# tpy001/VFMSeg

Hardware: AMD Instinct MI355X
Metric: train images/sec @512x512 DINOv2-L+LoRA (dg_lora_dinov2_ms_masked, 1024^2 sample = LR+HR 512^2 passes) (higher is better)
Workload: dtype bf16; 1 GPU; configs[1]: dg_lora_dinov2_ms_masked.py, synthetic 1024^2 19-class samples -> 2x512^2 passes, bs=2/GPU, full train step (fwd+bwd+allreduce+AdamW), LoRA dropout on; global_batch=2, parallelism=dp1

## Files before the change

include/vfmseg_hip.h:

```cpp
#ifndef VFMSEG_HIP_H
#define VFMSEG_HIP_H
#include <stdint.h>

#ifdef __cplusplus
extern "C" {
#endif

enum { VFM_F32 = 0, VFM_BF16 = 1, VFM_U8 = 2, VFM_I64 = 3,
       VFM_SPLIT3 = 4  };
enum { VFM_OK = 0, VFM_E_INVAL = -1, VFM_E_SHAPE = -2, VFM_E_ALIGN = -3, VFM_E_HIP = -4, VFM_E_UNSUPPORTED = -5 };
enum { VFM_EP_NONE = 0, VFM_EP_GELU = 1, VFM_EP_RELU = 2, VFM_EP_MUL_GELU_GRAD = 3, VFM_EP_MUL = 4,
       VFM_EP_QGELU = 5 , VFM_EP_MUL_QGELU_GRAD = 6,
       VFM_EP_GELU_DGELU = 7  };
enum { VFM_ACT_NONE = 0, VFM_ACT_GELU = 1, VFM_ACT_RELU = 2, VFM_ACT_QGELU = 3 };

const char* vfm_last_error(void);
int vfm_abi_version(void);
int vfm_half_kind(void);

int vfm_cast(const void* src, int src_dt, long ld_src, void* dst, int dst_dt, long ld_dst, long rows, long cols,
             const float* colscale, void* stream);
int vfm_split3(const float* src, long stride_r, long stride_c, void* dst, long ld_dst, long rows, long K, int pattern, void* stream);
int vfm_transpose(const void* src, int src_dt, long ld_src, void* dst, int dst_dt, long ld_dst, long rows, long cols,
                  long pad_rows, void* stream);
int vfm_strided_copy(const void* src, int src_dt, void* dst, int dst_dt, long n0, long n1, long n2, long n3, long s0,
                     long s1, long s2, long s3, long d0, long d1, long d2, long d3, int accumulate, void* stream);
typedef struct vfm_copy_job {
  const float* src; void* dst; long dst_dt; long accumulate;
  long n[4], s[4], d[4];
  long nsum, sum_stride;
} vfm_copy_job;
int vfm_strided_copy_batch(const vfm_copy_job* table_dev, int njobs, long max_elems, void* stream);
int vfm_axpby(const float* x, float a, float* y, float b, long n, void* stream);
int vfm_scale_by_device_scalar(float* y, const float* scalar, long n, void* stream);
int vfm_colsum(const void* x, int dt, long ld, long rows, long cols, float* out, int accumulate, float* ws, void* stream);
typedef struct vfm_lora_site {
  const float* A; const float* B;
  void* a; void* at; void* w; void* wt;
  long r, K, N, Kw, ld_a, ld_at, ld_w, ld_wt;
} vfm_lora_site;
int vfm_lora_pack(const vfm_lora_site* table_dev, int nsites, long max_elems, int dt, void* stream);
int vfm_slab_reduce(const float* slabs, int kch, long P, long Q, long rows_used, float alpha, float* dst, long sp, long sq,
                    int accumulate, void* stream);
int vfm_dropout_mask(void* out, int dt, long n, float p, uint64_t seed, uint64_t offset, void* stream);
int vfm_mul_mask(const void* src, int src_dt, long ld_src, const void* mask, int mask_dt, long mask_ld,
                 long rows_per_group, void* dst, int dst_dt, long ld_dst, long rows, long cols, void* stream);
int vfm_geglu_fwd(const void* h, int h_dt, long ld_h, void* out, int out_dt, long ld_out, long rows, long C, void* stream);
int vfm_geglu_bwd(const void* h, int h_dt, long ld_h, const void* dout, int do_dt, long ld_do, void* dh, int dh_dt,
                  long ld_dh, long rows, long C, void* stream);
int vfm_swiglu_fwd(const void* h, int h_dt, long ld_h, void* out, int out_dt, long ld_out, long rows, long C, void* stream);
int vfm_swiglu_bwd(const void* h, int h_dt, long ld_h, const void* dout, int do_dt, long ld_do, void* dh, int dh_dt,
                   long ld_dh, long rows, long C, void* stream);
int vfm_rope(void* x, int dt, long ld, long rows, int np, int ncols, int d, const float* cos_t, const float* sin_t,
             int inverse, void* stream);
int vfm_act_grad_mul(const void* dy, int dy_dt, long ld_dy, const void* pre, int pre_dt, long ld_pre, void* out, int out_dt,
                     long ld_out, long rows, long cols, int act, void* stream);
int vfm_mask_token_fwd(const float* x, const uint8_t* keep, const float* token, float* out, long rows, long C, void* stream);
int vfm_mask_token_bwd(const float* dout, const uint8_t* keep, float* dx, float* dtoken, float* ws ,
                       long rows, long C, void* stream);

int vfm_layernorm_fwd(const float* x, long ld_x, const float* w, const float* b, float eps, void* y, int y_dt, long ld_y,
                      float* stats, long rows, long C, void* stream);
int vfm_layernorm_fwd_split3(const float* x, long ld_x, const float* w, const float* b, float eps, float* y, long ld_y, void* y3, long ld3,
                             long plane, float* stats, long rows, long C, void* stream);
int vfm_layernorm_dropout_fwd(const float* x, long ld_x, const float* w, const float* b, float eps, void* y, long ld_y,
                              float* stats, void* y_drop, long ld_yd, void* mask, long ld_mask, float p, uint64_t seed,
                              uint64_t offset, long rows, long C, void* stream);
int vfm_layernorm_bwd_scaled(const void* dy, int dy_dt, long ld_dy, const float* x, long ld_x, const float* w,
                             const float* stats, float* dx, long ld_dx, int accumulate_dx, void* t_out, long ld_t,
                             const float* t_scale, long rows, long C, void* stream);
int vfm_layernorm_bwd(const void* dy, int dy_dt, long ld_dy, const float* x, long ld_x, const float* w,
                      const float* stats, float* dx, long ld_dx, int accumulate_dx, float* dw, float* db, float* ws,
                      long rows, long C, void* stream);
int vfm_groupnorm_fwd(const float* x, const float* w, const float* b, float eps, int G, int act, void* y, int y_dt,
                      float* stats, float* ws, long B, long P, long C, void* stream);
int vfm_groupnorm_bwd(const void* dy, int dy_dt, const float* x, const float* w, const float* b, const float* stats,
                      int G, int act, float* dx, float* dw, float* db, float* ws, long B, long P, long C, void* stream);
int vfm_groupnorm_tile_ok(long P, long C, int G);
int vfm_groupnorm_tile_fwd(const float* x, const float* w, const float* b, float eps, int G, int act, void* y, int y_dt,
                           float* stats, long B, long P, long C, void* stream);
int vfm_groupnorm_tile_bwd(const void* dy, int dy_dt, const float* x, const float* w, const float* b, const float* stats,
                           int G, int act, float* dx, float* dw, float* db, float* ws, long B, long P, long C, void* stream);
int vfm_bn_moments(const float* x, long rows, long C, float* sums, float* ws, void* stream);
int vfm_bn_finalize(const float* sums, float count, float* mean_var, float* running_mean, float* running_var,
                    float momentum, long C, void* stream);
int vfm_bn_apply(const float* x, const float* mean_var, const float* w, const float* b, float eps, int act, void* y,
                 int y_dt, long rows, long C, void* stream);
int vfm_bn_bwd_reduce(const void* dy, int dy_dt, const float* x, const float* mean_var, const float* w, const float* b,
                      float eps, int act, float* sums_dy, float* ws, long rows, long C, void* stream);
int vfm_bn_bwd_apply(const void* dy, int dy_dt, const float* x, const float* mean_var, const float* w, const float* b,
                     float eps, int act, const float* sums_dy, float total_rows, float* dx, long rows, long C,
                     void* stream);

typedef struct vfm_gemm_desc {
  const void* A; const void* B; void* C;
  int in_dt; int c_dt;
  long M, N, K;
  long sa_m, sa_k, sb_n, sb_k, ldc;
  float alpha;
  const float* bias; long bias_mod;
  const float* colscale;
  const void* residual; int r_dt; long ldr;
  int ep_mode; const void* aux; int aux_dt; long ld_aux;
  void* C2; int c2_dt; long ldc2;
  long batch, stride_a, stride_b, stride_c;
  long c_plane;
  long kb_rows;
} vfm_gemm_desc;
int vfm_gemm(const vfm_gemm_desc* d, void* stream);
int vfm_tune(const char* key, int value);

typedef struct vfm_attn_desc {
  const void* q; const void* k; const void* v; void* o;
  int dt; long ldq, ldk, ldv, ldo;
  int B, H, d;
  int nq_main, nq_extra, nk_main, nk_extra;
  float scale;
  float* lse;
  const void* dout; long ld_do;
  void* dq; void* dk; void* dv; long ld_dq, ld_dk, ld_dv;
  float* delta;
} vfm_attn_desc;
int vfm_attn_fwd(const vfm_attn_desc* d, void* stream);
int vfm_attn_bwd(const vfm_attn_desc* d, void* stream);
int vfm_attn_fwd_x3(const vfm_attn_desc* d, long lo_off, void* stream);
int vfm_attn_fwd_x3_split(const vfm_attn_desc* d, long lo_off, void* o3, long ld3, long plane, void* stream);
int vfm_attn_bwd_x3(const vfm_attn_desc* d, const void* q3, const void* k3, const void* v3, long ld3, long lo_off, const void* do3,
                    long ld_do3, long lo_off_do3, void* stream);

int vfm_sam_relpos_table(const float* rel_pos, int L, int d, int S, float* out, void* stream);
int vfm_sam_attn_prep(const void* qkv, int dt, long ld, const float* bias, const float* rh, const float* rw, void* q_aug,
                      void* k_aug, void* v_win, int nimg, int G, int S, int H, int d, int Dq, int NP,
                      int rows_per_batch , float scale, void* stream);
int vfm_softmax_rows(const float* scores, long ld_s, void* out, int out_dt, long ld_o, long rows, int n, int npad, void* stream);
int vfm_sam_attn_merge(const void* o_win, int dt, void* out, long ld, int nimg, int G, int S, int H, int d, int NP, void* stream);
int vfm_sam_attn_bwd_prep(const void* dao, long ld_dao, const void* qkv, long ld_qkv, const float* bias, int dt, void* dow,
                          void* dowT, void* vp, void* qsT, int nimg, int G, int S, int H, int d, int dp, int NP, float scale,
                          void* stream);
int vfm_softmax_rows_batched(const float* scores, long ld_s, void* out, int out_dt, long ld_o, long rows, int n, int npad,
                             int rows_per_batch, int valid_rows, void* stream);
int vfm_softmax_rows_bwd(const void* p, const float* dp, long ld_dp, void* ds, int dt, long ld_p, long rows, int n, int npad,
                         int rows_per_batch, int valid_rows, void* stream);
int vfm_sam_attn_bwd_merge(const void* dqa, const void* dkT, const void* dvT, int dt, const float* rh, const float* rw, void* dqkv,
                           long ld, int nimg, int G, int S, int H, int d, int dp, int NP, int Dq, float scale, void* stream);

int vfm_rein_mix_fwd(const float* x, long ld_x, const void* t, const void* vt, void* u, long ld_u, void* p, long ld_p, void* x16,
                     long ld_x16, long rows, int D, int m, float c, void* stream);
int vfm_rein_mix_bwd(const void* du, long ld_du, const void* p, long ld_p, const void* v, const void* tt, void* ds, long ld_ds,
                     float* dx, long ld_dx, long rows, int D, int m, float c, void* stream);

int vfm_sam_attn_flash_fwd(const void* qkv, long ld, const float* bias, const void* tbl_h, const void* tbl_w, void* out, long ldo,
                           int nimg, int G, int S, int H, int d, float scale, void* stream);
int vfm_sam_attn_flash_fwd_train(const void* qkv, long ld, const float* bias, const void* tbl_h, const void* tbl_w, void* out, long ldo,
                                 int nimg, int G, int S, int H, int d, float scale, float* lse, void* qext, void* stream);
long vfm_sam_attn_flash_stat_rows(int nimg, int G, int S, int H);
int vfm_sam_attn_flash_bwd(const void* qkv, long ld, const float* bias, const void* tbl_h, const void* tbl_w, const void* out,
                           const void* dout, long ldo, const float* lse, const void* qext, float* dsum, void* dqkv, long ldg,
                           int nimg, int G, int S, int H, int d, float scale, void* stream);

int vfm_patchify(const float* img, long stride_b, long stride_c, long stride_y, int y0, int x0, int h, int w, int P,
                 void* out, int out_dt, long ld_out, int B, void* stream);
int vfm_assemble_tokens(const float* patch_tok, const float* cls, const float* pos, float* x, int B, int np, int C,
                        void* stream);

int vfm_resize_bilinear(const void* in, int in_dt, int in_nchw, int B, int Hi, int Wi, int C, long in_ld_c, void* out,
                        int out_dt, int out_mode, long out_ld_c, int Hv, int Wv, int y0, int x0, int hc, int wc,
                        float scale_y, float scale_x, void* stream);
int vfm_resize_bicubic(const float* in, int Hi, int Wi, int C, float* out, int Ho, int Wo, double scale_y, double scale_x,
                       void* stream);
int vfm_label_resize(const int64_t* in, int B, int Hi, int Wi, int64_t* out, int Hv, int Wv, int y0, int x0, int hc,
                     int wc, void* stream);
int vfm_unblock(const float* x, float* y, int B, int H, int W, int C, int levels, int inverse, void* stream);
int vfm_upsample_ce(const float* logits_low, const int64_t* label, int B, int h, int w, int C, int H, int W,
                    int ignore_index, float* loss_parts, int32_t* counts, float* dlogits, void* stream);
int vfm_upsample_ce_w(const float* logits_low, const int64_t* label, const float* weight, int B, int h, int w, int C, int H, int W,
                      int ignore_index, float* loss_parts, int32_t* counts, float* dlogits, void* stream);
int vfm_pseudo_label(const float* logits_low, int B, int h, int w, int C, int H, int W, float thr, int64_t* pseudo_label,
                     float* pseudo_prob, int32_t* count, void* stream);
int vfm_class_presence(const int64_t* label, int B, long n, uint32_t* bits, void* stream);
int vfm_class_mix(const float* src_img, const float* tgt_img, const int64_t* src_label, const int64_t* pseudo_label,
                  const uint32_t* chosen, const int32_t* count, long total, int ignore_top, int ignore_bottom, int B, int H, int W,
                  float* mixed_img, int64_t* mixed_label, float* mix_weight, uint8_t* mask, void* stream);
int vfm_ce_finish(const float* loss_parts, long n, float scale, int32_t* counts, float eps, float* loss, float* acc, void* stream);
int vfm_hrda_fuse_fwd(const float* lr, const float* a, const float* hr, int B, int h, int w, int C, int ha, int wa, int hc, int wc,
                      int Y0, int X0, int my0, int my1, int mx0, int mx1, float* fused, float* att_out, float* lr_scaled_out,
                      void* stream);
int vfm_hrda_fuse_bwd(const float* d_fused, const float* lr, const float* a, const float* hr, const float* att, int B, int h, int w,
                      int C, int ha, int wa, int hc, int wc, int Y0, int X0, int my0, int my1, int mx0, int mx1, float* d_lr,
                      float* d_a, float* d_hr, float* d_att_ws, void* stream);
int vfm_reduce_sum(const float* x, long n, float scale, float* out, void* stream);

int vfm_preprocess_u8(const uint8_t* img, int H, int W, float* out, int Hp, int Wp, const float* mean3, const float* std3,
                      int bgr_to_rgb, float pad_val, void* stream);
int vfm_conf_gate(const float* logits, int B, int C, int H, int W, int y0, int x0, int hc, int wc, float thr,
                  int32_t* count, void* stream);
int vfm_slide_accumulate(const float* crop, int crop_nchw, int B, int h, int w, int C, float* preds, float* count,
                         int H, int W, int y0, int x0, int hc, int wc, void* stream);
typedef struct vfm_slide_win {
  const float* crop;
  int nchw, h, w;
  int y0, x0, hc, wc;
} vfm_slide_win;
int vfm_slide_gather(const vfm_slide_win* wins, int nwin, int B, int C, float* preds, int H, int W, void* stream);
int vfm_conf_gate_windows(const float* logits, int B, int C, int H, int W, const int* boxes, int nwin, float thr, int32_t* counts,
                          void* stream);
int vfm_slide_finalize(float* preds, const float* count, uint8_t* argmax, int B, int C, int H, int W, void* stream);

int vfm_confusion_hist(const uint8_t* pred, const void* label, int label_dt, long n, int num_classes, int ignore_index,
                       int64_t* hist, void* stream);

int vfm_adamw(float* p, float* g, float* m, float* v, long n, const long* seg_start, const float* seg_lr_mult,
              const float* seg_wd, int n_seg, float lr, float beta1, float beta2, float eps, int step, float grad_scale,
              int zero_grad, int vec4, void* stream);
int vfm_adamw_guarded(float* p, float* g, float* m, float* v, long n, const long* seg_start, const float* seg_lr_mult,
                      const float* seg_wd, int n_seg, float lr, float beta1, float beta2, float eps, int step, float grad_scale,
                      int zero_grad, int vec4, const int* skip, const float* amp_state, void* stream);
int vfm_amp_update(const int* flag, float* amp_state, float growth, float backoff, int interval, int dynamic, void* stream);

enum { VFM_OP_GEMM = 0, VFM_OP_LN_FWD = 1, VFM_OP_LN_DROPOUT_FWD = 2, VFM_OP_LN_BWD_SCALED = 3, VFM_OP_ATTN_FWD = 4, VFM_OP_ATTN_BWD = 5,
       VFM_OP_CAST = 6, VFM_OP_STRIDED_COPY = 7 };
enum { VFM_PROF_NONE = 0, VFM_PROF_GEMM = 1, VFM_PROF_GEMM_TN = 2, VFM_PROF_ATTN_FWD = 3, VFM_PROF_ATTN_BWD = 4 };
typedef struct vfm_plan_op {
  int kind;
  int prof_kind;
  double flops;
  union {
// ... 21 lines not shown
```

vfmseg_amd/csrc/elementwise.hip:

```cpp
#include "common.h"

thread_local char g_vfm_err[512] = {0};

extern "C" const char* vfm_last_error(void) { return g_vfm_err; }
extern "C" int vfm_abi_version(void) { return 6; }
extern "C" int vfm_half_kind(void) { return VFM_HALF_KIND; }

template <typename TI, typename TO>
__global__ void k_cast(const TI* __restrict__ src, long ld_src, TO* __restrict__ dst, long ld_dst, long rows, long cols,
                       const float* __restrict__ colscale) {
  const long cols4 = cols >> 2;
  const long total = rows * cols4;
  for (long i = blockIdx.x * (long)blockDim.x + threadIdx.x; i < total; i += (long)gridDim.x * blockDim.x) {
    const long r = i / cols4, c = (i - r * cols4) << 2;
    float v[4];
#pragma unroll
    for (int j = 0; j < 4; ++j) v[j] = ld_f32(src + r * ld_src + c + j);
    if (colscale) {
#pragma unroll
      for (int j = 0; j < 4; ++j) v[j] *= colscale[c + j];
    }
#pragma unroll
    for (int j = 0; j < 4; ++j) st_f32(dst + r * ld_dst + c + j, v[j]);
  }
  const long tail0 = cols4 << 2;
  const long ntail = cols - tail0;
  if (ntail) {
    for (long i = blockIdx.x * (long)blockDim.x + threadIdx.x; i < rows * ntail; i += (long)gridDim.x * blockDim.x) {
      const long r = i / ntail, c = tail0 + (i - r * ntail);
      float v = ld_f32(src + r * ld_src + c);
      if (colscale) v *= colscale[c];
      st_f32(dst + r * ld_dst + c, v);
    }
  }
}

extern "C" int vfm_cast(const void* src, int src_dt, long ld_src, void* dst, int dst_dt, long ld_dst, long rows, long cols,
                        const float* colscale, void* stream) {
  VFM_CHECK(rows >= 0 && cols >= 0 && ld_src >= cols && ld_dst >= cols, VFM_E_SHAPE, "vfm_cast: bad shape");
  if (rows == 0 || cols == 0) return VFM_OK;
  hipStream_t s = (hipStream_t)stream;
  const long total = rows * ((cols + 3) / 4);
  const int grid = (int)((total + 255) / 256 > 4096 ? 4096 : (total + 255) / 256);
#define L(TI, TO) hipLaunchKernelGGL((k_cast<TI, TO>), dim3(grid), dim3(256), 0, s, (const TI*)src, ld_src, (TO*)dst, ld_dst, rows, cols, colscale)
  if (src_dt == VFM_F32 && dst_dt == VFM_F32) L(float, float);
  else if (src_dt == VFM_F32 && dst_dt == VFM_BF16) L(float, bf16_t);
  else if (src_dt == VFM_BF16 && dst_dt == VFM_F32) L(bf16_t, float);
  else if (src_dt == VFM_BF16 && dst_dt == VFM_BF16) L(bf16_t, bf16_t);
  else VFM_FAIL(VFM_E_INVAL, "vfm_cast: dtype");
#undef L
  VFM_LAUNCH_CHECK();
  return VFM_OK;
}

__global__ void k_split3(const float* __restrict__ src, long sr, long sc, bf16_t* __restrict__ dst, long ld_dst, long rows, long K, long Kp,
                         int pattern) {
  const long per_row = Kp / 4;
  const long total = rows * per_row;
  for (long i = (long)blockIdx.x * blockDim.x + threadIdx.x; i < total; i += (long)gridDim.x * blockDim.x) {
    const long r = i / per_row, c = (i % per_row) * 4;
    float v[4];
    if (sc == 1 && c + 3 < K && ((reinterpret_cast<uintptr_t>(src + r * sr + c) & 15) == 0)) {
      const float4 f = *reinterpret_cast<const float4*>(src + r * sr + c);
      v[0] = f.x, v[1] = f.y, v[2] = f.z, v[3] = f.w;
    } else {
#pragma unroll
      for (int e = 0; e < 4; ++e) v[e] = (c + e < K) ? src[r * sr + (c + e) * sc] : 0.f;
    }
    ushort4 hi, lo;
    bf16_t* ph = &hi.x;
    bf16_t* pl = &lo.x;
#pragma unroll
    for (int e = 0; e < 4; ++e) {
      ph[e] = f32_to_bf16(v[e]);
      pl[e] = f32_to_bf16(v[e] - bf16_to_f32(ph[e]));
    }
    bf16_t* d = dst + r * ld_dst + c;
    *reinterpret_cast<ushort4*>(d) = hi;
    *reinterpret_cast<ushort4*>(d + Kp) = pattern == 0 ? hi : lo;
    *reinterpret_cast<ushort4*>(d + 2 * Kp) = pattern == 0 ? lo : hi;
  }
}

extern "C" int vfm_split3(const float* src, long stride_r, long stride_c, void* dst, long ld_dst, long rows, long K, int pattern, void* stream) {
  const long Kp = (K + 63) / 64 * 64;
  VFM_CHECK(rows >= 0 && K > 0 && ld_dst >= 3 * Kp && ld_dst % 4 == 0 && ((uintptr_t)dst % 8) == 0 && (pattern == 0 || pattern == 1), VFM_E_SHAPE,
            "vfm_split3: dst must hold rows x 3 ceil64(K) bf16 (ld %% 4 == 0, 8-byte aligned)");
  if (rows == 0) return VFM_OK;
  const long total = rows * (Kp / 4);
  const int grid = (int)((total + 255) / 256 > 8192 ? 8192 : (total + 255) / 256);
  hipLaunchKernelGGL(k_split3, dim3(grid), dim3(256), 0, (hipStream_t)stream, src, stride_r, stride_c, (bf16_t*)dst, ld_dst, rows, K, Kp, pattern);
  VFM_LAUNCH_CHECK();
  return VFM_OK;
}

template <typename TI, typename TO>
__global__ void k_transpose(const TI* __restrict__ src, long ld_src, TO* __restrict__ dst, long ld_dst, long rows, long cols,
                            long pad_rows) {
  __shared__ float tile[64][65];
  const long r0 = (long)blockIdx.y * 64, c0 = (long)blockIdx.x * 64;
  const int tx = threadIdx.x & 63, ty = threadIdx.x >> 6;
  for (int i = ty; i < 64; i += 4) {
    const long r = r0 + i, c = c0 + tx;
    tile[i][tx] = (r < rows && c < cols) ? ld_f32(src + r * ld_src + c) : 0.f;
  }
  __syncthreads();
  for (int i = ty; i < 64; i += 4) {
    const long c = c0 + i, r = r0 + tx;
    if (c < cols && r < pad_rows) st_f32(dst + c * ld_dst + r, tile[tx][i]);
  }
}

extern "C" int vfm_transpose(const void* src, int src_dt, long ld_src, void* dst, int dst_dt, long ld_dst, long rows, long cols,
                             long pad_rows, void* stream) {
  VFM_CHECK(pad_rows >= rows && ld_dst >= pad_rows && ld_src >= cols, VFM_E_SHAPE, "vfm_transpose: bad shape");
  if (cols == 0 || pad_rows == 0) return VFM_OK;
  hipStream_t s = (hipStream_t)stream;
  dim3 grid(cdiv(cols, 64), cdiv(pad_rows, 64));
#define L(TI, TO) hipLaunchKernelGGL((k_transpose<TI, TO>), grid, dim3(256), 0, s, (const TI*)src, ld_src, (TO*)dst, ld_dst, rows, cols, pad_rows)
  if (src_dt == VFM_F32 && dst_dt == VFM_F32) L(float, float);
  else if (src_dt == VFM_F32 && dst_dt == VFM_BF16) L(float, bf16_t);
  else if (src_dt == VFM_BF16 && dst_dt == VFM_F32) L(bf16_t, float);
  else if (src_dt == VFM_BF16 && dst_dt == VFM_BF16) L(bf16_t, bf16_t);
  else VFM_FAIL(VFM_E_INVAL, "vfm_transpose: dtype");
#undef L
  VFM_LAUNCH_CHECK();
  return VFM_OK;
}

template <typename TI, typename TO>
__global__ void k_strided_copy(const TI* __restrict__ src, TO* __restrict__ dst, long n0, long n1, long n2, long n3, long s0,
                               long s1, long s2, long s3, long d0, long d1, long d2, long d3, int accumulate) {
  const long total = n0 * n1 * n2 * n3;
  for (long i = blockIdx.x * (long)blockDim.x + threadIdx.x; i < total; i += (long)gridDim.x * blockDim.x) {
    long t = i;
    const long i3 = t % n3; t /= n3;
    const long i2 = t % n2; t /= n2;
    const long i1 = t % n1; t /= n1;
    const float v = ld_f32(src + t * s0 + i1 * s1 + i2 * s2 + i3 * s3);
    TO* q = dst + t * d0 + i1 * d1 + i2 * d2 + i3 * d3;
    st_f32(q, accumulate ? ld_f32(q) + v : v);
  }
}

extern "C" int vfm_strided_copy(const void* src, int src_dt, void* dst, int dst_dt, long n0, long n1, long n2, long n3,
                                long s0, long s1, long s2, long s3, long d0, long d1, long d2, long d3, int accumulate,
                                void* stream) {
  const long total = n0 * n1 * n2 * n3;
  if (total == 0) return VFM_OK;
  hipStream_t s = (hipStream_t)stream;
  const int grid = (int)((total + 255) / 256 > 4096 ? 4096 : (total + 255) / 256);
#define L(TI, TO) hipLaunchKernelGGL((k_strided_copy<TI, TO>), dim3(grid), dim3(256), 0, s, (const TI*)src, (TO*)dst, n0, n1, n2, n3, s0, s1, s2, s3, d0, d1, d2, d3, accumulate)
  if (src_dt == VFM_F32 && dst_dt == VFM_F32) L(float, float);
  else if (src_dt == VFM_F32 && dst_dt == VFM_BF16) L(float, bf16_t);
  else if (src_dt == VFM_BF16 && dst_dt == VFM_F32) L(bf16_t, float);
  else if (src_dt == VFM_BF16 && dst_dt == VFM_BF16) L(bf16_t, bf16_t);
  else VFM_FAIL(VFM_E_INVAL, "vfm_strided_copy: dtype");
#undef L
  VFM_LAUNCH_CHECK();
  return VFM_OK;
}

__global__ void k_axpby(const float* __restrict__ x, float a, float* __restrict__ y, float b, long n) {
  for (long i = blockIdx.x * (long)blockDim.x + threadIdx.x; i < n; i += (long)gridDim.x * blockDim.x)
    y[i] = (b == 0.f) ? a * x[i] : a * x[i] + b * y[i];
}
extern "C" int vfm_axpby(const float* x, float a, float* y, float b, long n, void* stream) {
  if (n == 0) return VFM_OK;
  const int grid = (int)((n + 255) / 256 > 4096 ? 4096 : (n + 255) / 256);
  hipLaunchKernelGGL(k_axpby, dim3(grid), dim3(256), 0, (hipStream_t)stream, x, a, y, b, n);
  VFM_LAUNCH_CHECK();
  return VFM_OK;
}
__global__ void k_scale_dev(float* __restrict__ y, const float* __restrict__ sc, long n) {
  const float s = *sc;
  for (long i = blockIdx.x * (long)blockDim.x + threadIdx.x; i < n; i += (long)gridDim.x * blockDim.x) y[i] *= s;
}
extern "C" int vfm_scale_by_device_scalar(float* y, const float* scalar, long n, void* stream) {
  if (n == 0) return VFM_OK;
  const int grid = (int)((n + 255) / 256 > 4096 ? 4096 : (n + 255) / 256);
  hipLaunchKernelGGL(k_scale_dev, dim3(grid), dim3(256), 0, (hipStream_t)stream, y, scalar, n);
  VFM_LAUNCH_CHECK();
  return VFM_OK;
}

template <typename T>
__global__ void k_colsum1(const T* __restrict__ x, long ld, long rows, long cols, float* __restrict__ ws, int CT) {
  __shared__ float sh[256];
  const int rl = 256 / CT;
  const int tx = threadIdx.x % CT, ty = threadIdx.x / CT;
  const long c = (long)blockIdx.x * CT + tx;
  float acc = 0.f;
  if (c < cols)
    for (long r = (long)blockIdx.y * rl + ty; r < rows; r += (long)gridDim.y * rl) acc += ld_f32(x + r * ld + c);
  sh[threadIdx.x] = acc;
  __syncthreads();
  if (ty == 0 && c < cols) {
    float a = 0.f;
    for (int k = 0; k < rl; ++k) a += sh[k * CT + tx];
    ws[(long)blockIdx.y * cols + c] = a;
  }
}
__global__ void __launch_bounds__(256) k_colsum2(const float* __restrict__ ws, long cols, int parts, float* __restrict__ out, int accumulate) {
  __shared__ float sh[4][64];
  const int tx = threadIdx.x & 63, g = threadIdx.x >> 6;
  const long c = blockIdx.x * 64L + tx;
  float a = 0.f;
  if (c < cols) {
    int p = g;
    for (; p + 12 < parts; p += 16) {
      const float v0 = ws[(long)p * cols + c], v1 = ws[(long)(p + 4) * cols + c], v2 = ws[(long)(p + 8) * cols + c], v3 = ws[(long)(p + 12) * cols + c];
      a += (v0 + v1) + (v2 + v3);
    }
    for (; p < parts; p += 4) a += ws[(long)p * cols + c];
  }
  sh[g][tx] = a;
  __syncthreads();
  if (g == 0 && c < cols) {
    const float t = (sh[0][tx] + sh[1][tx]) + (sh[2][tx] + sh[3][tx]);
    out[c] = accumulate ? out[c] + t : t;
  }
}
extern "C" int vfm_colsum(const void* x, int dt, long ld, long rows, long cols, float* out, int accumulate, float* ws,
                          void* stream) {
  VFM_CHECK(ld >= cols && ws, VFM_E_SHAPE, "vfm_colsum: bad args");
  if (cols == 0) return VFM_OK;
  hipStream_t s = (hipStream_t)stream;
  int CT = 64;
  while (CT > 8 && CT / 2 >= cols) CT /= 2;
  const int rl = 256 / CT;
  long parts = (rows + rl * 8 - 1) / (rl * 8);
  if (parts > 64) parts = 64;
  if (parts < 1) parts = 1;
  dim3 grid(cdiv(cols, CT), (unsigned)parts);
  if (dt == VFM_F32) hipLaunchKernelGGL(k_colsum1<float>, grid, dim3(256), 0, s, (const float*)x, ld, rows, cols, ws, CT);
  else if (dt == VFM_BF16) hipLaunchKernelGGL(k_colsum1<bf16_t>, grid, dim3(256), 0, s, (const bf16_t*)x, ld, rows, cols, ws, CT);
  else VFM_FAIL(VFM_E_INVAL, "vfm_colsum: dtype");
  hipLaunchKernelGGL(k_colsum2, dim3(cdiv(cols, 64)), dim3(256), 0, s, ws, cols, (int)parts, out, accumulate);
  VFM_LAUNCH_CHECK();
  return VFM_OK;
}

__global__ void k_slab_reduce(const float* __restrict__ slabs, int kch, long P, long Q, long rows_used, float alpha,
                              float* __restrict__ dst, long sp, long sq, int accumulate) {
  const long total = rows_used * Q;
  for (long i = blockIdx.x * (long)blockDim.x + threadIdx.x; i < total; i += (long)gridDim.x * blockDim.x) {
    const long p = i / Q, q = i - p * Q;
    float a = 0.f;
    for (int k = 0; k < kch; ++k) a += slabs[((long)k * P + p) * Q + q];
    a *= alpha;
    float* d = dst + p * sp + q * sq;
    *d = accumulate ? *d + a : a;
  }
}
extern "C" int vfm_slab_reduce(const float* slabs, int kch, long P, long Q, long rows_used, float alpha, float* dst, long sp,
                               long sq, int accumulate, void* stream) {
  VFM_CHECK(kch >= 1 && rows_used >= 0 && rows_used <= P, VFM_E_SHAPE, "vfm_slab_reduce: bad shape");
  const long total = rows_used * Q;
  if (total == 0) return VFM_OK;
  const int grid = (int)((total + 255) / 256 > 4096 ? 4096 : (total + 255) / 256);
  hipLaunchKernelGGL(k_slab_reduce, dim3(grid), dim3(256), 0, (hipStream_t)stream, slabs, kch, P, Q, rows_used, alpha, dst, sp, sq,
                     accumulate);
  VFM_LAUNCH_CHECK();
  return VFM_OK;
}

__global__ void __launch_bounds__(256) k_strided_copy_batch(const vfm_copy_job* __restrict__ tab) {
  const vfm_copy_job t = tab[blockIdx.y];
  const unsigned n1 = (unsigned)t.n[1], n2 = (unsigned)t.n[2], n3 = (unsigned)t.n[3];
  const unsigned total = (unsigned)t.n[0] * n1 * n2 * n3;
  for (unsigned i = blockIdx.x * 256u + threadIdx.x; i < total; i += gridDim.x * 256u) {
    unsigned r = i;
    const unsigned i3 = r % n3; r /= n3;
    const unsigned i2 = r % n2; r /= n2;
    const unsigned i1 = r % n1; r /= n1;
    const float* sp = t.src + ((long)r * t.s[0] + (long)i1 * t.s[1] + (long)i2 * t.s[2] + (long)i3 * t.s[3]);
    float v = sp[0];
    for (long c = 1; c < t.nsum; ++c) v += sp[c * t.sum_stride];
    const long o = (long)r * t.d[0] + (long)i1 * t.d[1] + (long)i2 * t.d[2] + (long)i3 * t.d[3];
    if (t.accumulate) ((float*)t.dst)[o] += v;
    else st_any(t.dst, o, (int)t.dst_dt, v);
  }
}
extern "C" int vfm_strided_copy_batch(const vfm_copy_job* table_dev, int njobs, long max_elems, void* stream) {
  VFM_CHECK(table_dev && njobs >= 0, VFM_E_INVAL, "vfm_strided_copy_batch: bad args");
  if (njobs == 0 || max_elems <= 0) return VFM_OK;
  VFM_CHECK(max_elems < (1l << 31), VFM_E_SHAPE, "vfm_strided_copy_batch: jobs are limited to 2^31 elements");
  int gx = (int)((max_elems + 2047) / 2048);
  if (gx > 2048) gx = 2048;
  if (gx < 1) gx = 1;
  hipLaunchKernelGGL(k_strided_copy_batch, dim3(gx, njobs), dim3(256), 0, (hipStream_t)stream, table_dev);
  VFM_LAUNCH_CHECK();
  return VFM_OK;
}

__global__ void k_lora_pack(const vfm_lora_site* __restrict__ tab, int dt) {
  const vfm_lora_site t = tab[blockIdx.y];
  const long na = t.r * t.K, nb = t.N * t.r;
  for (long i = blockIdx.x * (long)blockDim.x + threadIdx.x; i < na + nb; i += (long)gridDim.x * blockDim.x) {
    if (i < na) {
      const long rr = i / t.K, k = i - rr * t.K;
      const float v = t.A[i];
      st_any(t.a, rr * t.ld_a + k, dt, v);
      st_any(t.at, k * t.ld_at + rr, dt, v);
    } else {
      const long j = i - na;
      const long n = j / t.r, rr = j - n * t.r;
      const float v = t.B[j];
      st_any(t.w, n * t.ld_w + t.Kw + rr, dt, v);
      if (t.wt) st_any(t.wt, (t.Kw + rr) * t.ld_wt + n, dt, v);
    }
  }
}
extern "C" int vfm_lora_pack(const vfm_lora_site* table_dev, int nsites, long max_elems, int dt, void* stream) {
  VFM_CHECK(table_dev && nsites >= 0 && (dt == VFM_F32 || dt == VFM_BF16), VFM_E_INVAL, "vfm_lora_pack: bad args");
  if (nsites == 0) return VFM_OK;
  int gx = (int)((max_elems + 255) / 256);
  if (gx > 256) gx = 256;
  if (gx < 1) gx = 1;
  hipLaunchKernelGGL(k_lora_pack, dim3(gx, nsites), dim3(256), 0, (hipStream_t)stream, table_dev, dt);
  VFM_LAUNCH_CHECK();
  return VFM_OK;
}

struct F8 { float v[8]; };
__device__ __forceinline__ F8 ld8_bf16(const bf16_t* p) {
  const uint4 u = *reinterpret_cast<const uint4*>(p);
  F8 r;
  r.v[0] = h16_lo(u.x), r.v[1] = h16_hi(u.x);
  r.v[2] = h16_lo(u.y), r.v[3] = h16_hi(u.y);
  r.v[4] = h16_lo(u.z), r.v[5] = h16_hi(u.z);
  r.v[6] = h16_lo(u.w), r.v[7] = h16_hi(u.w);
  return r;
}
__device__ __forceinline__ void st8_bf16(bf16_t* p, const F8& r) {
  uint4 u;
  u.x = (uint32_t)f32_to_bf16(r.v[0]) | ((uint32_t)f32_to_bf16(r.v[1]) << 16);
  u.y = (uint32_t)f32_to_bf16(r.v[2]) | ((uint32_t)f32_to_bf16(r.v[3]) << 16);
  u.z = (uint32_t)f32_to_bf16(r.v[4]) | ((uint32_t)f32_to_bf16(r.v[5]) << 16);
  u.w = (uint32_t)f32_to_bf16(r.v[6]) | ((uint32_t)f32_to_bf16(r.v[7]) << 16);
  *reinterpret_cast<uint4*>(p) = u;
}
__device__ __forceinline__ F8 ld8_f32(const float* p) {
  const float4 a = *reinterpret_cast<const float4*>(p), b = *reinterpret_cast<const float4*>(p + 4);
  F8 r;
  r.v[0] = a.x, r.v[1] = a.y, r.v[2] = a.z, r.v[3] = a.w, r.v[4] = b.x, r.v[5] = b.y, r.v[6] = b.z, r.v[7] = b.w;
  return r;
}
__device__ __forceinline__ void st8_f32(float* p, const F8& r) {
  *reinterpret_cast<float4*>(p) = make_float4(r.v[0], r.v[1], r.v[2], r.v[3]);
  *reinterpret_cast<float4*>(p + 4) = make_float4(r.v[4], r.v[5], r.v[6], r.v[7]);
}
static inline bool al16(const void* p) { return ((uintptr_t)p & 15) == 0; }
static inline int grid8(long total8) { return (int)((total8 + 255) / 256 > 16384 ? 16384 : (total8 + 255) / 256); }

__global__ void k_dropout_mask_bf16x8(bf16_t* __restrict__ out, long n8, float p, float keep_scale, uint64_t seed, uint64_t offset) {
  for (long i = blockIdx.x * (long)blockDim.x + threadIdx.x; i < n8; i += (long)gridDim.x * blockDim.x) {
    F8 r;
#pragma unroll
    for (int e = 0; e < 8; ++e) {
      const float u = (hash_u32(seed, offset + (uint64_t)(i * 8 + e)) >> 8) * (1.0f / 16777216.0f);
      r.v[e] = u >= p ? keep_scale : 0.f;
    }
    st8_bf16(out + i * 8, r);
  }
}
__global__ void k_mul_mask_bf16x8(const bf16_t* __restrict__ src, long ld_src, const bf16_t* __restrict__ mask, long mask_ld, long rpg,
                                  bf16_t* __restrict__ dst, long ld_dst, long rows, int cols8) {
  const long total = rows * cols8;
  for (long i = blockIdx.x * (long)blockDim.x + threadIdx.x; i < total; i += (long)gridDim.x * blockDim.x) {
    const long r = i / cols8;
    const int c = (int)(i - r * cols8) * 8;
    F8 a = ld8_bf16(src + r * ld_src + c);
    const F8 m = ld8_bf16(mask + (r / rpg) * mask_ld + c);
#pragma unroll
    for (int e = 0; e < 8; ++e) a.v[e] *= m.v[e];
    st8_bf16(dst + r * ld_dst + c, a);
  }
}
__global__ void k_act_grad_mul_bf16x8(const bf16_t* __restrict__ dy, long ld_dy, const bf16_t* __restrict__ pre, long ld_pre,
                                      bf16_t* __restrict__ out, long ld_out, long rows, int cols8, int act) {
  const long total = rows * cols8;
  for (long i = blockIdx.x * (long)blockDim.x + threadIdx.x; i < total; i += (long)gridDim.x * blockDim.x) {
    const long r = i / cols8;
    const int c = (int)(i - r * cols8) * 8;
    F8 d = ld8_bf16(dy + r * ld_dy + c);
    const F8 p = ld8_bf16(pre + r * ld_pre + c);
#pragma unroll
    for (int e = 0; e < 8; ++e) {
      const float x = p.v[e];
      const float g = act == VFM_ACT_GELU ? gelu_grad_f(x) : (act == VFM_ACT_RELU ? (x > 0.f ? 1.f : 0.f) : (act == VFM_ACT_QGELU ? qgelu_grad_f(x) : 1.f));
      d.v[e] *= g;
    }
    st8_bf16(out + r * ld_out + c, d);
  }
// ... 57 lines not shown
}

__global__ void k_mul_mask(const void* __restrict__ src, int src_dt, long ld_src, const void* __restrict__ mask, int mask_dt,
                           long mask_ld, long rpg, void* __restrict__ dst, int dst_dt, long ld_dst, long rows, long cols) {
  const long total = rows * cols;
  for (long i = blockIdx.x * (long)blockDim.x + threadIdx.x; i < total; i += (long)gridDim.x * blockDim.x) {
    const long r = i / cols, c = i - r * cols;
    const float m = ld_any(mask, (r / rpg) * mask_ld + c, mask_dt);
    st_any(dst, r * ld_dst + c, dst_dt, ld_any(src, r * ld_src + c, src_dt) * m);
  }
}
template <typename TS, typename TM, typename TD>
__global__ void k_mul_mask_x8(const TS* __restrict__ src, long ld_src, const TM* __restrict__ mask, long mask_ld, long rpg, TD* __restrict__ dst,
                              long ld_dst, long rows, int cols8) {
  const long total = rows * cols8;
  for (long i = blockIdx.x * (long)blockDim.x + threadIdx.x; i < total; i += (long)gridDim.x * blockDim.x) {
    const long r = i / cols8;
    const int c = (int)(i - r * cols8) * 8;
    F8 a, m;
    if constexpr (sizeof(TS) == 2) a = ld8_bf16(src + r * ld_src + c); else a = ld8_f32(src + r * ld_src + c);
    if constexpr (sizeof(TM) == 2) m = ld8_bf16(mask + (r / rpg) * mask_ld + c); else m = ld8_f32(mask + (r / rpg) * mask_ld + c);
#pragma unroll
    for (int e = 0; e < 8; ++e) a.v[e] *= m.v[e];
    if constexpr (sizeof(TD) == 2) st8_bf16(dst + r * ld_dst + c, a); else st8_f32(dst + r * ld_dst + c, a);
  }
}
template <typename TS, typename TM, typename TD>
static void launch_mul_mask_x8(const void* src, long ld_src, const void* mask, long mask_ld, long rpg, void* dst, long ld_dst, long rows, long cols,
                               hipStream_t s) {
  hipLaunchKernelGGL((k_mul_mask_x8<TS, TM, TD>), dim3(grid8(rows * cols / 8)), dim3(256), 0, s, (const TS*)src, ld_src, (const TM*)mask, mask_ld, rpg,
                     (TD*)dst, ld_dst, rows, (int)(cols / 8));
}
extern "C" int vfm_mul_mask(const void* src, int src_dt, long ld_src, const void* mask, int mask_dt, long mask_ld,
                            long rows_per_group, void* dst, int dst_dt, long ld_dst, long rows, long cols, void* stream) {
  VFM_CHECK(rows_per_group >= 1, VFM_E_INVAL, "vfm_mul_mask: rows_per_group");
  const long total = rows * cols;
  if (total == 0) return VFM_OK;
  auto h16 = [](int dt) { return dt == VFM_BF16; };
  auto okdt = [](int dt) { return dt == VFM_BF16 || dt == VFM_F32; };
  if (okdt(src_dt) && okdt(mask_dt) && okdt(dst_dt) && !(h16(src_dt) && h16(mask_dt) && h16(dst_dt)) && cols % 8 == 0 && ld_src % 8 == 0 &&
      mask_ld % 8 == 0 && ld_dst % 8 == 0 && al16(src) && al16(mask) && al16(dst)) {
    hipStream_t s = (hipStream_t)stream;
    const int key = (h16(src_dt) ? 4 : 0) | (h16(mask_dt) ? 2 : 0) | (h16(dst_dt) ? 1 : 0);
#define MM(TS, TM, TD) launch_mul_mask_x8<TS, TM, TD>(src, ld_src, mask, mask_ld, rows_per_group, dst, ld_dst, rows, cols, s)
    switch (key) {
      case 0: MM(float, float, float); break;
      case 1: MM(float, float, bf16_t); break;
      case 2: MM(float, bf16_t, float); break;
      case 3: MM(float, bf16_t, bf16_t); break;
      case 4: MM(bf16_t, float, float); break;
      case 5: MM(bf16_t, float, bf16_t); break;
      default: MM(bf16_t, bf16_t, float); break;
    }
#undef MM
    VFM_LAUNCH_CHECK();
    return VFM_OK;
  }
  if (src_dt == VFM_BF16 && mask_dt == VFM_BF16 && dst_dt == VFM_BF16 && cols % 8 == 0 && ld_src % 8 == 0 && mask_ld % 8 == 0 && ld_dst % 8 == 0 &&
      al16(src) && al16(mask) && al16(dst)) {
    hipLaunchKernelGGL(k_mul_mask_bf16x8, dim3(grid8(total / 8)), dim3(256), 0, (hipStream_t)stream, (const bf16_t*)src, ld_src, (const bf16_t*)mask,
                       mask_ld, rows_per_group, (bf16_t*)dst, ld_dst, rows, (int)(cols / 8));
    VFM_LAUNCH_CHECK();
    return VFM_OK;
  }
  const int grid = (int)((total + 255) / 256 > 8192 ? 8192 : (total + 255) / 256);
  hipLaunchKernelGGL(k_mul_mask, dim3(grid), dim3(256), 0, (hipStream_t)stream, src, src_dt, ld_src, mask, mask_dt, mask_ld,
                     rows_per_group, dst, dst_dt, ld_dst, rows, cols);
  VFM_LAUNCH_CHECK();
  return VFM_OK;
}

__global__ void k_geglu_fwd(const void* __restrict__ h, int h_dt, long ld_h, void* __restrict__ out, int out_dt, long ld_out,
                            long rows, long C) {
  const long total = rows * C;
  for (long i = blockIdx.x * (long)blockDim.x + threadIdx.x; i < total; i += (long)gridDim.x * blockDim.x) {
    const long r = i / C, c = i - r * C;
    const float a = ld_any(h, r * ld_h + c, h_dt), g = ld_any(h, r * ld_h + C + c, h_dt);
    st_any(out, r * ld_out + c, out_dt, a * gelu_f(g));
  }
}
__global__ void k_geglu_bwd(const void* __restrict__ h, int h_dt, long ld_h, const void* __restrict__ dout, int do_dt,
                            long ld_do, void* __restrict__ dh, int dh_dt, long ld_dh, long rows, long C) {
  const long total = rows * C;
  for (long i = blockIdx.x * (long)blockDim.x + threadIdx.x; i < total; i += (long)gridDim.x * blockDim.x) {
    const long r = i / C, c = i - r * C;
    const float a = ld_any(h, r * ld_h + c, h_dt), g = ld_any(h, r * ld_h + C + c, h_dt);
    const float d = ld_any(dout, r * ld_do + c, do_dt);
    st_any(dh, r * ld_dh + c, dh_dt, d * gelu_f(g));
    st_any(dh, r * ld_dh + C + c, dh_dt, d * a * gelu_grad_f(g));
  }
}
__global__ void k_geglu_fwd_x8(const bf16_t* __restrict__ h, long ld_h, bf16_t* __restrict__ out, long ld_out, long rows, long C, int c8) {
  const long total = rows * c8;
  for (long i = blockIdx.x * (long)blockDim.x + threadIdx.x; i < total; i += (long)gridDim.x * blockDim.x) {
    const long r = i / c8;
    const int c = (int)(i - r * c8) * 8;
    F8 a = ld8_bf16(h + r * ld_h + c);
    const F8 g = ld8_bf16(h + r * ld_h + C + c);
#pragma unroll
    for (int e = 0; e < 8; ++e) a.v[e] *= gelu_f(g.v[e]);
    st8_bf16(out + r * ld_out + c, a);
  }
}
__global__ void k_geglu_bwd_x8(const bf16_t* __restrict__ h, long ld_h, const bf16_t* __restrict__ dout, long ld_do, bf16_t* __restrict__ dh,
                               long ld_dh, long rows, long C, int c8) {
  const long total = rows * c8;
  for (long i = blockIdx.x * (long)blockDim.x + threadIdx.x; i < total; i += (long)gridDim.x * blockDim.x) {
    const long r = i / c8;
    const int c = (int)(i - r * c8) * 8;
    const F8 a = ld8_bf16(h + r * ld_h + c), g = ld8_bf16(h + r * ld_h + C + c), d = ld8_bf16(dout + r * ld_do + c);
    F8 da, dg;
#pragma unroll
    for (int e = 0; e < 8; ++e) {
      da.v[e] = d.v[e] * gelu_f(g.v[e]);
      dg.v[e] = d.v[e] * a.v[e] * gelu_grad_f(g.v[e]);
    }
    st8_bf16(dh + r * ld_dh + c, da);
    st8_bf16(dh + r * ld_dh + C + c, dg);
  }
}
extern "C" int vfm_geglu_fwd(const void* h, int h_dt, long ld_h, void* out, int out_dt, long ld_out, long rows, long C,
                             void* stream) {
  const long total = rows * C;
  if (total == 0) return VFM_OK;
  if (h_dt == VFM_BF16 && out_dt == VFM_BF16 && C % 8 == 0 && ld_h % 8 == 0 && ld_out % 8 == 0 && al16(h) && al16(out)) {
    hipLaunchKernelGGL(k_geglu_fwd_x8, dim3(grid8(total / 8)), dim3(256), 0, (hipStream_t)stream, (const bf16_t*)h, ld_h, (bf16_t*)out, ld_out, rows, C,
                       (int)(C / 8));
    VFM_LAUNCH_CHECK();
    return VFM_OK;
  }
  const int grid = (int)((total + 255) / 256 > 8192 ? 8192 : (total + 255) / 256);
  hipLaunchKernelGGL(k_geglu_fwd, dim3(grid), dim3(256), 0, (hipStream_t)stream, h, h_dt, ld_h, out, out_dt, ld_out, rows, C);
  VFM_LAUNCH_CHECK();
  return VFM_OK;
}
extern "C" int vfm_geglu_bwd(const void* h, int h_dt, long ld_h, const void* dout, int do_dt, long ld_do, void* dh, int dh_dt,
                             long ld_dh, long rows, long C, void* stream) {
  const long total = rows * C;
  if (total == 0) return VFM_OK;
  if (h_dt == VFM_BF16 && do_dt == VFM_BF16 && dh_dt == VFM_BF16 && C % 8 == 0 && ld_h % 8 == 0 && ld_do % 8 == 0 && ld_dh % 8 == 0 && al16(h) &&
      al16(dout) && al16(dh)) {
    hipLaunchKernelGGL(k_geglu_bwd_x8, dim3(grid8(total / 8)), dim3(256), 0, (hipStream_t)stream, (const bf16_t*)h, ld_h, (const bf16_t*)dout, ld_do,
                       (bf16_t*)dh, ld_dh, rows, C, (int)(C / 8));
    VFM_LAUNCH_CHECK();
    return VFM_OK;
  }
  const int grid = (int)((total + 255) / 256 > 8192 ? 8192 : (total + 255) / 256);
  hipLaunchKernelGGL(k_geglu_bwd, dim3(grid), dim3(256), 0, (hipStream_t)stream, h, h_dt, ld_h, dout, do_dt, ld_do, dh, dh_dt,
                     ld_dh, rows, C);
  VFM_LAUNCH_CHECK();
  return VFM_OK;
}

__global__ void k_swiglu_fwd(const void* __restrict__ h, int h_dt, long ld_h, void* __restrict__ out, int out_dt, long ld_out,
                             long rows, long C) {
  const long total = rows * C;
  for (long i = blockIdx.x * (long)blockDim.x + threadIdx.x; i < total; i += (long)gridDim.x * blockDim.x) {
    const long r = i / C, c = i - r * C;
    const float a = ld_any(h, r * ld_h + c, h_dt), g = ld_any(h, r * ld_h + C + c, h_dt);
    st_any(out, r * ld_out + c, out_dt, a / (1.f + __expf(-a)) * g);
  }
}
__global__ void k_swiglu_bwd(const void* __restrict__ h, int h_dt, long ld_h, const void* __restrict__ dout, int do_dt,
                             long ld_do, void* __restrict__ dh, int dh_dt, long ld_dh, long rows, long C) {
  const long total = rows * C;
  for (long i = blockIdx.x * (long)blockDim.x + threadIdx.x; i < total; i += (long)gridDim.x * blockDim.x) {
    const long r = i / C, c = i - r * C;
    const float a = ld_any(h, r * ld_h + c, h_dt), g = ld_any(h, r * ld_h + C + c, h_dt);
    const float d = ld_any(dout, r * ld_do + c, do_dt);
    const float sg = 1.f / (1.f + __expf(-a));
    st_any(dh, r * ld_dh + c, dh_dt, d * g * sg * (1.f + a * (1.f - sg)));
    st_any(dh, r * ld_dh + C + c, dh_dt, d * a * sg);
  }
}
extern "C" int vfm_swiglu_fwd(const void* h, int h_dt, long ld_h, void* out, int out_dt, long ld_out, long rows, long C,
                              void* stream) {
  const long total = rows * C;
  if (total == 0) return VFM_OK;
  if (h_dt == VFM_BF16 && (out_dt == VFM_BF16 || out_dt == VFM_F32) && C % 8 == 0 && ld_h % 8 == 0 && ld_out % 8 == 0 && al16(h) && al16(out)) {
    if (out_dt == VFM_BF16)
      hipLaunchKernelGGL(k_swiglu_fwd_x8<true>, dim3(grid8(total / 8)), dim3(256), 0, (hipStream_t)stream, (const bf16_t*)h, ld_h, out, ld_out, rows, C, (int)(C / 8));
    else
      hipLaunchKernelGGL(k_swiglu_fwd_x8<false>, dim3(grid8(total / 8)), dim3(256), 0, (hipStream_t)stream, (const bf16_t*)h, ld_h, out, ld_out, rows, C, (int)(C / 8));
    VFM_LAUNCH_CHECK();
    return VFM_OK;
  }
  const int grid = (int)((total + 255) / 256 > 8192 ? 8192 : (total + 255) / 256);
  hipLaunchKernelGGL(k_swiglu_fwd, dim3(grid), dim3(256), 0, (hipStream_t)stream, h, h_dt, ld_h, out, out_dt, ld_out, rows, C);
  VFM_LAUNCH_CHECK();
  return VFM_OK;
}
extern "C" int vfm_swiglu_bwd(const void* h, int h_dt, long ld_h, const void* dout, int do_dt, long ld_do, void* dh, int dh_dt,
                              long ld_dh, long rows, long C, void* stream) {
  const long total = rows * C;
  if (total == 0) return VFM_OK;
  if (h_dt == VFM_BF16 && dh_dt == VFM_BF16 && (do_dt == VFM_BF16 || do_dt == VFM_F32) && C % 8 == 0 && ld_h % 8 == 0 && ld_do % 8 == 0 &&
      ld_dh % 8 == 0 && al16(h) && al16(dout) && al16(dh)) {
    if (do_dt == VFM_BF16)
      hipLaunchKernelGGL(k_swiglu_bwd_x8<true>, dim3(grid8(total / 8)), dim3(256), 0, (hipStream_t)stream, (const bf16_t*)h, ld_h, dout, ld_do, (bf16_t*)dh, ld_dh, rows, C, (int)(C / 8));
    else
      hipLaunchKernelGGL(k_swiglu_bwd_x8<false>, dim3(grid8(total / 8)), dim3(256), 0, (hipStream_t)stream, (const bf16_t*)h, ld_h, dout, ld_do, (bf16_t*)dh, ld_dh, rows, C, (int)(C / 8));
    VFM_LAUNCH_CHECK();
    return VFM_OK;
  }
  const int grid = (int)((total + 255) / 256 > 8192 ? 8192 : (total + 255) / 256);
  hipLaunchKernelGGL(k_swiglu_bwd, dim3(grid), dim3(256), 0, (hipStream_t)stream, h, h_dt, ld_h, dout, do_dt, ld_do, dh, dh_dt,
                     ld_dh, rows, C);
  VFM_LAUNCH_CHECK();
  return VFM_OK;
}

__device__ __forceinline__ void rope_pair(float x0, float x1, float c_0, float c_1, float s_0, float s_1, int inverse, float& y0, float& y1) {
  if (!inverse) {
    y0 = fmaf(x0, c_0, -(x1 * s_0));
    y1 = fmaf(x1, c_1, x0 * s_1);
  } else {
    y0 = fmaf(x0, c_0, x1 * s_1);
    y1 = fmaf(x1, c_1, -(x0 * s_0));
  }
}
__global__ void k_rope(void* __restrict__ x, int dt, long ld, long rows, int np, int ncols, int d, const float* __restrict__ cs,
                       const float* __restrict__ sn, int inverse) {
  const long half = ncols / 2;
  const long total = rows * half;
  for (long i = blockIdx.x * (long)blockDim.x + threadIdx.x; i < total; i += (long)gridDim.x * blockDim.x) {
    const long r = i / half;
    const int c0 = (int)(i - r * half) * 2;
    const int t = (int)(r % np), dc = c0 % d;
    const float x0 = ld_any(x, r * ld + c0, dt), x1 = ld_any(x, r * ld + c0 + 1, dt);
    const float c_0 = cs[(long)t * d + dc], c_1 = cs[(long)t * d + dc + 1];
    const float s_0 = sn[(long)t * d + dc], s_1 = sn[(long)t * d + dc + 1];
    float y0, y1;
    rope_pair(x0, x1, c_0, c_1, s_0, s_1, inverse, y0, y1);
    st_any(x, r * ld + c0, dt, y0);
    st_any(x, r * ld + c0 + 1, dt, y1);
  }
}
__global__ void k_rope_bf16x8(bf16_t* __restrict__ x, long ld, long rows, int np, int c8n, int d, const float* __restrict__ cs,
                              const float* __restrict__ sn, int inverse) {
  const long total = rows * c8n;
  for (long i = blockIdx.x * (long)blockDim.x + threadIdx.x; i < total; i += (long)gridDim.x * blockDim.x) {
    const long r = i / c8n;
    const int c0 = (int)(i - r * c8n) * 8;
    const int t = (int)(r % np), dc = c0 % d;
    F8 v = ld8_bf16(x + r * ld + c0);
    const F8 c = ld8_f32(cs + (long)t * d + dc), sv = ld8_f32(sn + (long)t * d + dc);
#pragma unroll
    for (int e = 0; e < 8; e += 2) rope_pair(v.v[e], v.v[e + 1], c.v[e], c.v[e + 1], sv.v[e], sv.v[e + 1], inverse, v.v[e], v.v[e + 1]);
    st8_bf16(x + r * ld + c0, v);
  }
}
extern "C" int vfm_rope(void* x, int dt, long ld, long rows, int np, int ncols, int d, const float* cos_t, const float* sin_t,
                        int inverse, void* stream) {
  VFM_CHECK(d % 2 == 0 && ncols % d == 0 && np > 0, VFM_E_SHAPE, "vfm_rope: shape");
  const long total = rows * (ncols / 2);
  if (total == 0) return VFM_OK;
  if (dt == VFM_BF16 && d % 8 == 0 && ld % 8 == 0 && al16(x) && al16(cos_t) && al16(sin_t)) {
    hipLaunchKernelGGL(k_rope_bf16x8, dim3(grid8(rows * (ncols / 8))), dim3(256), 0, (hipStream_t)stream, (bf16_t*)x, ld, rows, np, ncols / 8, d, cos_t,
                       sin_t, inverse);
    VFM_LAUNCH_CHECK();
    return VFM_OK;
  }
  const int grid = (int)((total + 255) / 256 > 8192 ? 8192 : (total + 255) / 256);
  hipLaunchKernelGGL(k_rope, dim3(grid), dim3(256), 0, (hipStream_t)stream, x, dt, ld, rows, np, ncols, d, cos_t, sin_t, inverse);
  VFM_LAUNCH_CHECK();
  return VFM_OK;
}

__global__ void k_act_grad_mul(const void* __restrict__ dy, int dy_dt, long ld_dy, const void* __restrict__ pre, int pre_dt,
                               long ld_pre, void* __restrict__ out, int out_dt, long ld_out, long rows, long cols, int act) {
  const long total = rows * cols;
  for (long i = blockIdx.x * (long)blockDim.x + threadIdx.x; i < total; i += (long)gridDim.x * blockDim.x) {
    const long r = i / cols, c = i - r * cols;
    const float p = ld_any(pre, r * ld_pre + c, pre_dt);
    const float g = act == VFM_ACT_GELU ? gelu_grad_f(p) : (act == VFM_ACT_RELU ? (p > 0.f ? 1.f : 0.f) : (act == VFM_ACT_QGELU ? qgelu_grad_f(p) : 1.f));
    st_any(out, r * ld_out + c, out_dt, ld_any(dy, r * ld_dy + c, dy_dt) * g);
  }
}
extern "C" int vfm_act_grad_mul(const void* dy, int dy_dt, long ld_dy, const void* pre, int pre_dt, long ld_pre, void* out,
                                int out_dt, long ld_out, long rows, long cols, int act, void* stream) {
  const long total = rows * cols;
  if (total == 0) return VFM_OK;
  if (dy_dt == VFM_BF16 && pre_dt == VFM_BF16 && out_dt == VFM_BF16 && cols % 8 == 0 && ld_dy % 8 == 0 && ld_pre % 8 == 0 && ld_out % 8 == 0 &&
      al16(dy) && al16(pre) && al16(out)) {
    hipLaunchKernelGGL(k_act_grad_mul_bf16x8, dim3(grid8(total / 8)), dim3(256), 0, (hipStream_t)stream, (const bf16_t*)dy, ld_dy, (const bf16_t*)pre,
                       ld_pre, (bf16_t*)out, ld_out, rows, (int)(cols / 8), act);
    VFM_LAUNCH_CHECK();
    return VFM_OK;
  }
  const int grid = (int)((total + 255) / 256 > 8192 ? 8192 : (total + 255) / 256);
  hipLaunchKernelGGL(k_act_grad_mul, dim3(grid), dim3(256), 0, (hipStream_t)stream, dy, dy_dt, ld_dy, pre, pre_dt, ld_pre, out,
                     out_dt, ld_out, rows, cols, act);
  VFM_LAUNCH_CHECK();
  return VFM_OK;
}

__global__ void k_mask_token_fwd(const float* __restrict__ x, const uint8_t* __restrict__ keep, const float* __restrict__ tok,
                                 float* __restrict__ out, long rows, long C) {
  const long total = rows * C;
  for (long i = blockIdx.x * (long)blockDim.x + threadIdx.x; i < total; i += (long)gridDim.x * blockDim.x) {
    const long r = i / C, c = i - r * C;
    out[i] = keep[r] ? x[i] : tok[c];
  }
}
__global__ void k_mask_token_bwd(const float* __restrict__ dout, const uint8_t* __restrict__ keep, float* __restrict__ dx,
                                 float* __restrict__ ws, long rows, long C, long rows_per_chunk) {
// ... 74 lines not shown
```

vfmseg_amd/csrc/norm.hip:

```cpp
#include "common.h"

__device__ __forceinline__ float act_f(float v, int act) {
  return act == VFM_ACT_GELU ? gelu_f(v) : (act == VFM_ACT_RELU ? fmaxf(v, 0.f) : v);
}
__device__ __forceinline__ float act_grad_f(float v, int act) {
  return act == VFM_ACT_GELU ? gelu_grad_f(v) : (act == VFM_ACT_RELU ? (v > 0.f ? 1.f : 0.f) : 1.f);
}

template <typename TO, int MAXPL>
__global__ void k_ln_fwd(const float* __restrict__ x, long ld_x, const float* __restrict__ w, const float* __restrict__ b,
                         float eps, TO* __restrict__ y, long ld_y, float* __restrict__ stats, long rows, int C) {
  const int lane = threadIdx.x & 63;
  const long row = (long)blockIdx.x * (blockDim.x >> 6) + (threadIdx.x >> 6);
  if (row >= rows) return;
  const float* xr = x + row * ld_x;
  float v[MAXPL];
  float s = 0.f;
#pragma unroll
  for (int i = 0; i < MAXPL; ++i) {
    const int c = i * 64 + lane;
    v[i] = c < C ? xr[c] : 0.f;
    s += v[i];
  }
  const float mean = wave_sum(s) / C;
// ... 466 lines not shown
#pragma unroll
  for (int i = 0; i < MAXP4; ++i) {
    const int c = (i * 64 + lane) * 4;
    if (c < C) {
      float o[4];
#pragma unroll
      for (int e = 0; e < 4; ++e) o[e] = rstd * (g[i][e] - s1 - xh[i][e] * s2);
      if (c + 4 <= C) {
        float4* pp = reinterpret_cast<float4*>(dx + row * ld_dx + c);
        if (accumulate_dx) {
          const float4 old = *pp;
          o[0] += old.x, o[1] += old.y, o[2] += old.z, o[3] += old.w;
        }
        *pp = make_float4(o[0], o[1], o[2], o[3]);
      } else {
#pragma unroll
        for (int e = 0; e < 4; ++e)
          if (c + e < C) dx[row * ld_dx + c + e] = accumulate_dx ? dx[row * ld_dx + c + e] + o[e] : o[e];
      }
    }
  }
}

static int ln_bwd_impl(const void* dy, int dy_dt, long ld_dy, const float* x, long ld_x, const float* w, const float* stats,
                       float* dx, long ld_dx, int accumulate_dx, float* dw, float* db, float* ws, long rows, long C, void* t_out,
                       long ld_t, const float* t_scale, void* stream);
extern "C" int vfm_layernorm_bwd(const void* dy, int dy_dt, long ld_dy, const float* x, long ld_x, const float* w,
                                 const float* stats, float* dx, long ld_dx, int accumulate_dx, float* dw, float* db,
                                 float* ws, long rows, long C, void* stream) {
  return ln_bwd_impl(dy, dy_dt, ld_dy, x, ld_x, w, stats, dx, ld_dx, accumulate_dx, dw, db, ws, rows, C, nullptr, 0, nullptr, stream);
}
extern "C" int vfm_layernorm_bwd_scaled(const void* dy, int dy_dt, long ld_dy, const float* x, long ld_x, const float* w,
                                        const float* stats, float* dx, long ld_dx, int accumulate_dx, void* t_out, long ld_t,
                                        const float* t_scale, long rows, long C, void* stream) {
  VFM_CHECK(t_out && t_scale && ld_t % 4 == 0 && (uintptr_t)t_out % 8 == 0 && (uintptr_t)t_scale % 16 == 0, VFM_E_INVAL,
            "vfm_layernorm_bwd_scaled: t_out / t_scale");
  return ln_bwd_impl(dy, dy_dt, ld_dy, x, ld_x, w, stats, dx, ld_dx, accumulate_dx, nullptr, nullptr, nullptr, rows, C, t_out, ld_t,
                     t_scale, stream);
}
template <typename TD, int MAXP2>
__global__ void k_ln_bwd_v2(const TD* __restrict__ dy, long ld_dy, const float* __restrict__ x, long ld_x, const float* __restrict__ w,
                            const float* __restrict__ stats, float* __restrict__ dx, long ld_dx, int accumulate_dx, long rows, int C) {
  const int lane = threadIdx.x & 63;
  const long row = (long)blockIdx.x * (blockDim.x >> 6) + (threadIdx.x >> 6);
  if (row >= rows) return;
  const float mean = stats[row * 2], rstd = stats[row * 2 + 1];
  float2 g[MAXP2], xh[MAXP2];
  float s1 = 0.f, s2 = 0.f;
#pragma unroll
  for (int i = 0; i < MAXP2; ++i) {
    const int c = (i * 64 + lane) * 2;
    g[i] = xh[i] = make_float2(0.f, 0.f);
    if (c < C) {
      float2 d;
      if constexpr (sizeof(TD) == 2) {
        const ushort2 pp = *reinterpret_cast<const ushort2*>(dy + row * ld_dy + c);
        d = make_float2(bf16_to_f32(pp.x), bf16_to_f32(pp.y));
      } else {
        d = *reinterpret_cast<const float2*>(dy + row * ld_dy + c);
      }
      const float2 xv = *reinterpret_cast<const float2*>(x + row * ld_x + c);
      const float2 ww = *reinterpret_cast<const float2*>(w + c);
      xh[i] = make_float2((xv.x - mean) * rstd, (xv.y - mean) * rstd);
      g[i] = make_float2(d.x * ww.x, d.y * ww.y);
      s1 += g[i].x + g[i].y;
      s2 += g[i].x * xh[i].x + g[i].y * xh[i].y;
    }
  }
  s1 = wave_sum(s1) / C;
  s2 = wave_sum(s2) / C;
#pragma unroll
  for (int i = 0; i < MAXP2; ++i) {
    const int c = (i * 64 + lane) * 2;
    if (c < C) {
      float2 o = make_float2(rstd * (g[i].x - s1 - xh[i].x * s2), rstd * (g[i].y - s1 - xh[i].y * s2));
      float2* pp = reinterpret_cast<float2*>(dx + row * ld_dx + c);
      if (accumulate_dx) {
        const float2 old = *pp;
        o.x += old.x, o.y += old.y;
      }
      *pp = o;
    }
  }
}

static int ln_bwd_impl(const void* dy, int dy_dt, long ld_dy, const float* x, long ld_x, const float* w, const float* stats,
                       float* dx, long ld_dx, int accumulate_dx, float* dw, float* db, float* ws, long rows, long C, void* t_out,
                       long ld_t, const float* t_scale, void* stream) {
  VFM_CHECK(C > 0 && (C <= 1024 || (C <= 3072 && !(dw || db))), VFM_E_SHAPE, "vfm_layernorm_bwd: C=%ld unsupported", C);
  VFM_CHECK(!(dw || db) || ws, VFM_E_INVAL, "vfm_layernorm_bwd: ws required for dw/db");
  if (rows == 0) return VFM_OK;
  hipStream_t s = (hipStream_t)stream;
  const bool need_w = (dw || db);
  const int nv = (int)(C / 256);
  const bool v4 = !need_w && (C % 256 == 0) && (nv == 1 || nv == 2 || nv == 4 || nv == 5) && (ld_x % 4 == 0) && (ld_dx % 4 == 0) &&
                  (ld_dy % 4 == 0) && ((uintptr_t)x % 16 == 0) && ((uintptr_t)dx % 16 == 0) && ((uintptr_t)dy % 8 == 0) &&
                  ((uintptr_t)w % 16 == 0);
  if (v4) {
    dim3 grid(cdiv(rows, 4)), blk(256);
#define LV(TD, NV) hipLaunchKernelGGL((k_ln_bwd_v4<TD, NV>), grid, blk, 0, s, (const TD*)dy, ld_dy, x, ld_x, w, stats, dx, ld_dx, accumulate_dx, rows, (int)C, (bf16_t*)t_out, ld_t, t_scale)
    if (dy_dt == VFM_BF16) { if (nv == 1) LV(bf16_t, 1); else if (nv == 2) LV(bf16_t, 2); else if (nv == 4) LV(bf16_t, 4); else LV(bf16_t, 5); }
    else if (dy_dt == VFM_F32) { if (nv == 1) LV(float, 1); else if (nv == 2) LV(float, 2); else if (nv == 4) LV(float, 4); else LV(float, 5); }
    else VFM_FAIL(VFM_E_INVAL, "vfm_layernorm_bwd: dtype");
#undef LV
    VFM_LAUNCH_CHECK();
    return VFM_OK;
  }
  VFM_CHECK(!t_out, VFM_E_UNSUPPORTED, "vfm_layernorm_bwd_scaled: needs the vectorised path (C %% 256 == 0, aligned operands, no dw/db)");
  {
    const long cp = (C + 3) / 4 * 4;
    if (!need_w && C > 1024 && C <= 2816 && ld_x % 4 == 0 && ld_dx % 4 == 0 && ld_dy % 4 == 0 && ld_x >= cp && ld_dx >= cp && ld_dy >= cp &&
        (uintptr_t)x % 16 == 0 && (uintptr_t)dx % 16 == 0 && (uintptr_t)dy % 16 == 0 && (uintptr_t)w % 16 == 0) {
      dim3 grid(cdiv(rows, 4)), blk(256);
      if (dy_dt == VFM_BF16)
        hipLaunchKernelGGL((k_ln_bwd_v4t<bf16_t, 11>), grid, blk, 0, s, (const bf16_t*)dy, ld_dy, x, ld_x, w, stats, dx, ld_dx, accumulate_dx, rows, (int)C);
      else if (dy_dt == VFM_F32)
        hipLaunchKernelGGL((k_ln_bwd_v4t<float, 11>), grid, blk, 0, s, (const float*)dy, ld_dy, x, ld_x, w, stats, dx, ld_dx, accumulate_dx, rows, (int)C);
      else VFM_FAIL(VFM_E_INVAL, "vfm_layernorm_bwd: dtype");
      VFM_LAUNCH_CHECK();
      return VFM_OK;
    }
  }
  if (!need_w && C > 1024 && C % 2 == 0 && ld_x % 2 == 0 && ld_dx % 2 == 0 && ld_dy % 2 == 0 && (uintptr_t)x % 8 == 0 &&
      (uintptr_t)dx % 8 == 0 && (uintptr_t)dy % 8 == 0 && (uintptr_t)w % 8 == 0) {
    dim3 grid(cdiv(rows, 4)), blk(256);
    if (dy_dt == VFM_BF16)
      hipLaunchKernelGGL((k_ln_bwd_v2<bf16_t, 24>), grid, blk, 0, s, (const bf16_t*)dy, ld_dy, x, ld_x, w, stats, dx, ld_dx, accumulate_dx, rows, (int)C);
    else if (dy_dt == VFM_F32)
      hipLaunchKernelGGL((k_ln_bwd_v2<float, 24>), grid, blk, 0, s, (const float*)dy, ld_dy, x, ld_x, w, stats, dx, ld_dx, accumulate_dx, rows, (int)C);
    else VFM_FAIL(VFM_E_INVAL, "vfm_layernorm_bwd: dtype");
    VFM_LAUNCH_CHECK();
    return VFM_OK;
  }
  const int parts = need_w ? 128 : cdiv(rows, 4);
  const size_t shm = need_w ? (size_t)4 * 2 * C * sizeof(float) : 0;
  float* wsp = need_w ? ws : nullptr;
#define L(TD, PL, NW) hipLaunchKernelGGL((k_ln_bwd<TD, PL, NW>), dim3(parts), dim3(256), shm, s, (const TD*)dy, ld_dy, x, ld_x, w, stats, dx, ld_dx, accumulate_dx, wsp, rows, (int)C)
  const int pl = (int)((C + 63) / 64);
  if (need_w) {
    if (dy_dt == VFM_BF16) { if (pl <= 4) L(bf16_t, 4, true); else L(bf16_t, 16, true); }
    else if (dy_dt == VFM_F32) { if (pl <= 4) L(float, 4, true); else L(float, 16, true); }
    else VFM_FAIL(VFM_E_INVAL, "vfm_layernorm_bwd: dtype");
  } else {
    if (dy_dt == VFM_BF16) { if (pl <= 4) L(bf16_t, 4, false); else if (pl <= 16) L(bf16_t, 16, false); else L(bf16_t, 48, false); }
    else if (dy_dt == VFM_F32) { if (pl <= 4) L(float, 4, false); else if (pl <= 16) L(float, 16, false); else L(float, 48, false); }
    else VFM_FAIL(VFM_E_INVAL, "vfm_layernorm_bwd: dtype");
  }
#undef L
  if (need_w) hipLaunchKernelGGL(k_ln_bwd_fin, dim3(cdiv(C, 64)), dim3(256), 0, s, ws, parts, (int)C, dw, db);
  VFM_LAUNCH_CHECK();
  return VFM_OK;
}

template <int MODE, typename TD>
__global__ void k_chan_moments(const float* __restrict__ x, const TD* __restrict__ dy, const float* __restrict__ w,
                               const float* __restrict__ bb, const float* __restrict__ stats, int G, float eps, int act,
                               float* __restrict__ ws, long P, int C, int rows_per_chunk) {
  __shared__ float sh[2][4][64];
  const int tx = threadIdx.x & 63, ty = threadIdx.x >> 6;
  const int c = blockIdx.x * 64 + tx;
  const long b = blockIdx.z;
  const long r0 = (long)blockIdx.y * rows_per_chunk;
  long r1 = r0 + rows_per_chunk;
  if (r1 > P) r1 = P;
  float a1 = 0.f, a2 = 0.f;
  if (c < C) {
    float mean = 0.f, rstd = 1.f, wc = 1.f, bc = 0.f;
    if (MODE == 1) {
      if (G > 0) {
        const int g = c / (C / G);
        mean = stats[(b * G + g) * 2];
        rstd = stats[(b * G + g) * 2 + 1];
      } else {
        mean = stats[c];
        rstd = rsqrtf(stats[C + c] + eps);
      }
      wc = w[c];
      bc = bb[c];
    }
    const float* xp = x + (b * P) * C + c;
    for (long r = r0 + ty; r < r1; r += 4) {
      const float xv = xp[r * C];
      if (MODE == 0) {
        a1 += xv;
        a2 += xv * xv;
      } else {
        const float xh = (xv - mean) * rstd;
        float d = ld_f32(dy + (b * P + r) * C + c);
        if (act != VFM_ACT_NONE) d *= act_grad_f(xh * wc + bc, act);
        a1 += d;
        a2 += d * xh;
      }
    }
  }
  sh[0][ty][tx] = a1;
  sh[1][ty][tx] = a2;
  __syncthreads();
  if (ty == 0 && c < C) {
    const long slot = b * gridDim.y + blockIdx.y;
    ws[(slot * 2 + 0) * C + c] = sh[0][0][tx] + sh[0][1][tx] + sh[0][2][tx] + sh[0][3][tx];
    ws[(slot * 2 + 1) * C + c] = sh[1][0][tx] + sh[1][1][tx] + sh[1][2][tx] + sh[1][3][tx];
  }
}

static inline int pick_chunks(long P) {
  int n = (int)((P + 63) / 64);
  if (n > 64) n = 64;
  if (n < 1) n = 1;
  return n;
}

__device__ __forceinline__ double wave_sum_f64(double v) {
#pragma unroll
  for (int o = 32; o > 0; o >>= 1) v += __shfl_xor(v, o, 64);
  return v;
}
__global__ void k_gn_fin_fwd(const float* __restrict__ ws, int nchunk, int C, int G, long P, float eps,
                             float* __restrict__ stats, int BG) {
  const int i = blockIdx.x * (blockDim.x >> 6) + (threadIdx.x >> 6), lane = threadIdx.x & 63;
  if (i >= BG) return;
  const int b = i / G, g = i - b * G, cg = C / G;
  double s = 0.0, q = 0.0;
  for (int e = lane; e < nchunk * cg; e += 64) {
    const int k = e / cg, j = e - k * cg;
    const long slot = (long)b * nchunk + k;
    s += ws[(slot * 2 + 0) * C + g * cg + j];
    q += ws[(slot * 2 + 1) * C + g * cg + j];
  }
  s = wave_sum_f64(s), q = wave_sum_f64(q);
  if (lane) return;
  const double n = (double)P * cg;
  const double mean = s / n;
  double var = q / n - mean * mean;
  if (var < 0) var = 0;
  stats[i * 2] = (float)mean;
  stats[i * 2 + 1] = (float)(1.0 / sqrt(var + (double)eps));
}
template <typename TO>
__global__ void k_gn_apply(const float* __restrict__ x, const float* __restrict__ w, const float* __restrict__ b,
                           const float* __restrict__ stats, int G, int act, TO* __restrict__ y, long B, long P, int C) {
  const long total = B * P * C;
  const int cg = C / G;
  for (long i = blockIdx.x * (long)blockDim.x + threadIdx.x; i < total; i += (long)gridDim.x * blockDim.x) {
    const int c = (int)(i % C);
    const long bi = i / ((long)P * C);
    const int g = c / cg;
    const float mean = stats[(bi * G + g) * 2], rstd = stats[(bi * G + g) * 2 + 1];
    st_f32(y + i, act_f((x[i] - mean) * rstd * w[c] + b[c], act));
  }
}
extern "C" int vfm_groupnorm_fwd(const float* x, const float* w, const float* b, float eps, int G, int act, void* y, int y_dt,
                                 float* stats, float* ws_in, long B, long P, long C, void* stream) {
  VFM_CHECK(G > 0 && C % G == 0 && ws_in, VFM_E_SHAPE, "vfm_groupnorm_fwd: C %% G / ws");
  if (B * P * C == 0) return VFM_OK;
  hipStream_t s = (hipStream_t)stream;
  const int nchunk = pick_chunks(P);
  const int rpc = (int)((P + nchunk - 1) / nchunk);
  float* ws = ws_in + B * G * 2;
  hipLaunchKernelGGL((k_chan_moments<0, float>), dim3(cdiv(C, 64), nchunk, (unsigned)B), dim3(256), 0, s, x, (const float*)nullptr,
                     (const float*)nullptr, (const float*)nullptr, (const float*)nullptr, 0, 0.f, 0, ws, P, (int)C, rpc);
  hipLaunchKernelGGL(k_gn_fin_fwd, dim3(cdiv(B * G, 4)), dim3(256), 0, s, ws, nchunk, (int)C, G, P, eps, stats, (int)(B * G));
  const long total = B * P * C;
  const int grid = (int)((total + 255) / 256 > 8192 ? 8192 : (total + 255) / 256);
  if (y_dt == VFM_BF16) hipLaunchKernelGGL(k_gn_apply<bf16_t>, dim3(grid), dim3(256), 0, s, x, w, b, stats, G, act, (bf16_t*)y, B, P, (int)C);
  else if (y_dt == VFM_F32) hipLaunchKernelGGL(k_gn_apply<float>, dim3(grid), dim3(256), 0, s, x, w, b, stats, G, act, (float*)y, B, P, (int)C);
  else VFM_FAIL(VFM_E_INVAL, "vfm_groupnorm_fwd: dtype");
  VFM_LAUNCH_CHECK();
  return VFM_OK;
}

__global__ void k_gn_fin_bwd(const float* __restrict__ ws, int nchunk, int C, int G, const float* __restrict__ w,
                             float* __restrict__ gs, int BG) {
  const int i = blockIdx.x * (blockDim.x >> 6) + (threadIdx.x >> 6), lane = threadIdx.x & 63;
  if (i >= BG) return;
  const int b = i / G, g = i - b * G, cg = C / G;
  double s1 = 0.0, s2 = 0.0;
  for (int e = lane; e < nchunk * cg; e += 64) {
    const int k = e / cg, j = e - k * cg;
    const long slot = (long)b * nchunk + k;
    const int c = g * cg + j;
    s1 += (double)w[c] * ws[(slot * 2 + 0) * C + c];
    s2 += (double)w[c] * ws[(slot * 2 + 1) * C + c];
  }
  s1 = wave_sum_f64(s1), s2 = wave_sum_f64(s2);
  if (lane) return;
  gs[i * 2] = (float)s1;
  gs[i * 2 + 1] = (float)s2;
}
__global__ void k_chan_fin_wb(const float* __restrict__ ws, int slots, int C, float* __restrict__ dw, float* __restrict__ db) {
  __shared__ float sh[2][4][64];
  const int tx = threadIdx.x & 63, ty = threadIdx.x >> 6;
  const int c = blockIdx.x * 64 + tx;
  float a = 0.f, b = 0.f;
  if (c < C) {
#pragma unroll 8
    for (int k = ty; k < slots; k += 4) {
      b += ws[((long)k * 2 + 0) * C + c];
      a += ws[((long)k * 2 + 1) * C + c];
    }
  }
  sh[0][ty][tx] = a, sh[1][ty][tx] = b;
  __syncthreads();
  if (ty == 0 && c < C) {
    if (dw) dw[c] += (sh[0][0][tx] + sh[0][1][tx]) + (sh[0][2][tx] + sh[0][3][tx]);
    if (db) db[c] += (sh[1][0][tx] + sh[1][1][tx]) + (sh[1][2][tx] + sh[1][3][tx]);
  }
// ... 330 lines not shown
```

vfmseg_amd/functional.py:

```python
import os

import torch

from .precision import is_half
from . import ops
from .precision import compute_dtype

_seed_state = {"seed": 0x5EED, "offset": 0}


def manual_seed(seed):
    _seed_state["seed"], _seed_state["offset"] = int(seed), 0


def _next_rng(n):
    off = _seed_state["offset"]
    _seed_state["offset"] += int(n)
    return _seed_state["seed"], off


def draw_seed(seed, n):
    if seed is None:
        return _next_rng(n)
    return int(seed), 0
# ... 201 lines not shown
            assert act is None
            mask = torch.empty(M, N, dtype=cd, device=x.device)
            seed, off = _next_rng(M * N)
            ops.dropout_mask(mask, drop_p, seed, off)
            ep, aux = ops.EP_MUL, mask
        bias_full = None
        if bias is not None:
            bias_full = bias.detach()
        ops.gemm(x, wp, y, bias=bias_full, bias_mod=(N // bias_tile if bias_tile > 1 else 0), residual=residual, ep_mode=ep,
                 aux=aux, c2=pre)
        ctx.save_for_backward(x, wp, pre if pre is not None else (y if act == "relu" else None), mask, *weights)
        ctx.opts, ctx.dims, ctx.has_res, ctx.has_bias = opts, dims, residual is not None, bias is not None
        ctx.bias_param = bias
        ctx.res_dtype = residual.dtype if residual is not None else None
        return y

    @staticmethod
    def backward(ctx, dy):
        x, wp, pre, mask, *weights = ctx.saved_tensors
        opts, dims = ctx.opts, ctx.dims
        layouts, act, bias_tile = opts["layouts"], opts.get("act"), opts.get("bias_tile", 1)
        cd = x.dtype
        M, Kp = x.shape
        N = wp.shape[0]
        dy = dy.contiguous()
        d_res = None
        if ctx.has_res and ctx.needs_input_grad[1]:
            d_res = dy if dy.dtype == ctx.res_dtype else _cast_new(dy, ctx.res_dtype)
        npad = _pad64(N) if is_half(cd) else N
        if mask is None and act is None and dy.dtype == cd and npad == N and dy.data_ptr() % 16 == 0:
            g = gv = dy
        else:
            g = torch.zeros(M, npad, dtype=cd, device=dy.device) if npad > N else torch.empty(M, N, dtype=cd, device=dy.device)
            gv = g[:, :N]
        if g is dy:
            pass
        elif mask is not None:
            ops.mul_mask(dy, mask, gv)
        elif act == "gelu":
            _mul_act_grad(dy, pre, gv, "gelu")
        elif act == "relu":
            _mul_act_grad(dy, pre, gv, "relu")
        else:
            ops.cast(dy, gv)
        dx = None
        if ctx.needs_input_grad[0]:
            dx = torch.empty(M, Kp, dtype=cd, device=dy.device)
            if is_half(cd):
                ops.gemm(g, wp, dx, trans_b=True, kb_rows=N)
            else:
                ops.gemm(gv, wp, dx, trans_b=True)
        side = None
        if is_half(cd) and dy.is_cuda and all(direct_grad_target(p_) is not None for p_ in
                                              ([ctx.bias_param] if (ctx.has_bias and ctx.needs_input_grad[2]) else []) +
                                              [w for i, w in enumerate(weights) if ctx.needs_input_grad[4 + i]]):
            side = wgrad_stream()
        if side is not None:
            side.wait_stream(torch.cuda.current_stream())
            g.record_stream(side), x.record_stream(side)
            if not _WG["used"]:
                torch.autograd.Variable._execution_engine.queue_callback(join_wgrad_stream)
            _WG["used"] = True
            with torch.cuda.stream(side):
                dbias, dws = LinearFn._param_grads(ctx, g, gv, x, weights, dims, layouts, bias_tile, cd, M, N, Kp, npad)
        else:
            dbias, dws = LinearFn._param_grads(ctx, g, gv, x, weights, dims, layouts, bias_tile, cd, M, N, Kp, npad)
        return (dx, d_res, dbias, None) + tuple(dws)


def _param_grads_impl(ctx, g, gv, x, weights, dims, layouts, bias_tile, cd, M, N, Kp, npad):
        dy = g
        dbias = None
        if ctx.has_bias and ctx.needs_input_grad[2]:
            btgt = direct_grad_target(ctx.bias_param) if ctx.bias_param is not None else None
            if bias_tile > 1:
                full = torch.empty(N, dtype=torch.float32, device=dy.device)
                ops.colsum(gv, full)
                if btgt is not None:
                    ops.colsum(full.view(bias_tile, N // bias_tile), btgt.view(-1), accumulate=True)
                else:
                    dbias = torch.empty(N // bias_tile, dtype=torch.float32, device=dy.device)
                    ops.colsum(full.view(bias_tile, N // bias_tile), dbias)
            elif btgt is not None:
                ops.colsum(gv, btgt.view(-1), accumulate=True)
            else:
                dbias = torch.empty(N, dtype=torch.float32, device=dy.device)
                ops.colsum(gv, dbias)
        dws = [None] * len(weights)
        if any(ctx.needs_input_grad[4:]):
            gw = torch.empty(npad if is_half(cd) else N, Kp, dtype=torch.float32, device=dy.device)
            if is_half(cd):
                mp = _pad64(M)
                tiles = ((N + 127) // 128) * ((Kp + 127) // 128)
                kch = 1
                while tiles * kch < 256 and (mp // (kch * 2)) % 64 == 0 and mp // (kch * 2) >= 256:
                    kch *= 2
                if kch > 1:
                    slabs = torch.empty(kch, npad, Kp, dtype=torch.float32, device=dy.device)
                    ops.gemm_splitk_tn(g, x, slabs, kch)
                    tgt = direct_grad_target(weights[0]) if len(weights) == 1 and ctx.needs_input_grad[4] else None
                    if tgt is not None and layouts[0] in ("linear", "conv1x1") and Kp == dims[0][1]:
                        ops.slab_reduce(slabs, N, tgt, Kp, 1, accumulate=True)
                        return dbias, dws
                    ops.colsum(slabs.view(kch, npad * Kp), gw.view(npad * Kp))
                else:
                    ops.gemm_splitk_tn(g, x, gw.view(1, npad, Kp), 1)
            else:
                ops.gemm(gv, x, gw, trans_a=True, trans_b=True)
            r0 = 0
            for i, (w, l, d) in enumerate(zip(weights, layouts, dims)):
                if ctx.needs_input_grad[4 + i]:
                    dws[i] = _unpack_grad(gw[r0:r0 + d[0]], l, w)
                r0 += d[0]
        return dbias, dws

LinearFn._param_grads = staticmethod(_param_grads_impl)


def _cast_new(t, dtype):
    out = torch.empty(t.shape, dtype=dtype, device=t.device)
    ops.cast(t.view(-1, t.shape[-1]), out.view(-1, t.shape[-1]))
    return out


def _mul_act_grad(dy, pre, out, kind):
    M, N = dy.shape
    if kind == "gelu":
        ops.act_grad_mul(dy, pre, out, ops.ACT_GELU)
    else:
        ops.act_grad_mul(dy, pre, out, ops.ACT_RELU)


def linear(x, weights, layouts, bias=None, residual=None, act=None, out_dtype=None, drop_p=0.0, bias_tile=1):
    if not isinstance(weights, (list, tuple)):
        weights, layouts = [weights], [layouts]
    opts = dict(layouts=list(layouts), act=act, out_dtype=out_dtype or x.dtype, drop_p=drop_p, bias_tile=bias_tile)
    return LinearFn.apply(x, residual, bias, opts, *weights)


def _norm_grad_slots(w, b, C, device):
    tw, tb = direct_grad_target(w), direct_grad_target(b)
    dw = tw.view(-1) if tw is not None else torch.zeros(C, dtype=torch.float32, device=device)
    db = tb.view(-1) if tb is not None else torch.zeros(C, dtype=torch.float32, device=device)
    return dw, db, (None if tw is not None else dw), (None if tb is not None else db)


class GroupNormActFn(torch.autograd.Function):
    @staticmethod
    def forward(ctx, x, w, b, B, P, groups, eps, act, out_dtype):
        x = x.contiguous()
        C = x.shape[1]
        y = torch.empty(B * P, C, dtype=out_dtype, device=x.device)
        stats = torch.empty(B, groups, 2, dtype=torch.float32, device=x.device)
        ops.groupnorm_fwd(x, w.detach(), b.detach(), eps, groups, act, y, stats, B, P)
        ctx.save_for_backward(x, w, b, stats)
        ctx.cfg = (B, P, groups, act)
        return y

    @staticmethod
    def backward(ctx, dy):
        x, w, b, stats = ctx.saved_tensors
        B, P, groups, act = ctx.cfg
        C = x.shape[1]
        dx = torch.empty_like(x)
        dw, db, ret_w, ret_b = _norm_grad_slots(w, b, C, x.device)
        ops.groupnorm_bwd(dy.contiguous(), x, w.detach(), b.detach(), stats, groups, act, dx, dw, db, B, P)
        return dx, ret_w, ret_b, None, None, None, None, None, None


def group_norm_act(x, w, b, B, P, groups=32, eps=1e-5, act=ops.ACT_NONE, out_dtype=None):
    return GroupNormActFn.apply(x, w, b, B, P, groups, eps, act, out_dtype or compute_dtype())


GN_TILE_BWD_MIN_BLOCKS = 64
GN_TILE_SLAB = 32


def gn_tile_selected(P, C, groups, B=None, backward=False):
    v = os.environ.get("VFMSEG_GN_TILE", "")
    if v == "0" or not ops.groupnorm_tile_ok(P, C, groups):
        return False
    if v == "1" or not backward:
        return True
    return B is None or B * (C // GN_TILE_SLAB) >= GN_TILE_BWD_MIN_BLOCKS


class NormParamPack:

    def __init__(self):
        self.key = self.buf = self.table = self.stamp = None
        self.gkey = self.gbuf = self.gtable = None

    def get(self, ws, bs):
        key = tuple(p.data_ptr() for p in ws + bs)
        if key != self.key:
            C, n = ws[0].numel(), len(ws)
            self.buf = torch.empty(2, n * C, dtype=torch.float32, device=ws[0].device)
            jobs = [(p.detach().view(-1), self.buf[j][i * C:(i + 1) * C], (C,), (1,), (1,))
                    for j, ps in enumerate((ws, bs)) for i, p in enumerate(ps)]
            self.table, self.key, self.stamp = ops.CopyBatch(jobs), key, None
        stamp = _PackCache._stamp(ws + bs)
        if stamp != self.stamp:
            self.table.run()
            self.stamp = stamp
        return self.buf[0], self.buf[1]

    def grad_buffer(self, C, device):
        if self.gbuf is None or self.gbuf.shape[1] != C or self.gbuf.device != device:
            self.gbuf, self.gkey = torch.empty(2, C, dtype=torch.float32, device=device), None
        return self.gbuf.zero_()

    def scatter(self, params, n):
        c = self.gbuf.shape[1] // n
        parts = [self.gbuf[j, i * c:(i + 1) * c] for j in range(2) for i in range(n)]
        tgts = [direct_grad_target(p) for p in params]
        if any(t is None for t in tgts):
            for part, t in zip(parts, tgts):
                if t is not None:
                    ops.axpby(part, 1.0, t.view(-1), 1.0)
            return tuple(None if t is not None else part.clone() for part, t in zip(parts, tgts))
        key = tuple(t.data_ptr() for t in tgts)
        if key != self.gkey:
            self.gtable = ops.CopyBatch([(part, t.view(-1), (c,), (1,), (1,), True) for part, t in zip(parts, tgts)])
            self.gkey = key
        self.gtable.run()
        return (None,) * len(params)


class GroupNormCatFn(torch.autograd.Function):

    @staticmethod
    def forward(ctx, x, B, P, groups, eps, act, out_dtype, pack, n, *wb):
        x = x.contiguous()
        C = x.shape[1]
        ws, bs = wb[:n], wb[n:]
        if n == 1:
            w, b = ws[0].detach(), bs[0].detach()
        else:
            w, b = pack.get(ws, bs)
        tile = gn_tile_selected(P, C, n * groups, B)
        y = torch.empty(B * P, C, dtype=out_dtype, device=x.device)
        stats = torch.empty(B, n * groups, 2, dtype=torch.float32, device=x.device)
        (ops.groupnorm_tile_fwd if tile else ops.groupnorm_fwd)(x, w, b, eps, n * groups, act, y, stats, B, P)
        ctx.save_for_backward(x, w, b, stats, *wb)
        ctx.cfg = (B, P, n * groups, act, n, gn_tile_selected(P, C, n * groups, B, backward=True))
        ctx.pack = pack
        return y

    @staticmethod
    def backward(ctx, dy):
        x, w, b, stats, *wb = ctx.saved_tensors
        B, P, G, act, n, tile = ctx.cfg
        C = x.shape[1]
        bwd = ops.groupnorm_tile_bwd if tile else ops.groupnorm_bwd
        if n == 1:
            dw, db, ret_w, ret_b = _norm_grad_slots(wb[0], wb[1], C, x.device)
            dx = bwd(dy.contiguous(), x, w, b, stats, G, act, torch.empty_like(x), dw, db, B, P)
            return (dx,) + (None,) * 8 + (ret_w, ret_b)
        pack = ctx.pack
        dwb = pack.grad_buffer(C, x.device)
        dx = bwd(dy.contiguous(), x, w, b, stats, G, act, torch.empty_like(x), dwb[0], dwb[1], B, P)
        return (dx,) + (None,) * 8 + pack.scatter(wb, n)


def group_norm_cat_act(x, ws, bs, B, P, groups, eps, act, out_dtype=None, pack=None):
    ws, bs = list(ws), list(bs)
    return GroupNormCatFn.apply(x, B, P, groups, eps, act, out_dtype or compute_dtype(), pack, len(ws), *ws, *bs)


class BranchLinearFn(torch.autograd.Function):

    @staticmethod
    def _views(x, n):
        M, K = x.shape[0], x.shape[1] // n
        return x.as_strided((n, M, K), (K, x.stride(0), 1), x.storage_offset())

    @staticmethod
    def forward(ctx, x, n, *weights):
        cd = x.dtype
        M, K = x.shape[0], x.shape[1] // n
        N = weights[0].shape[0]
        assert x.stride(1) == 1 and all(w.shape[0] == N and w[0].numel() == K for w in weights)
        if is_half(cd) and (N % 64 or K % 64):
            raise NotImplementedError(f"branch_linear: 16-bit operands need in / out channels in multiples of 64 (got {K} / {N})")
        wp = PACKS.get(weights, ["conv1x1"] * n, [(N, K)] * n, K, K, cd)
        y = torch.empty(M, n * N, dtype=torch.float32, device=x.device)
        ops.gemm(BranchLinearFn._views(x, n), wp.view(n, N, K), BranchLinearFn._views(y, n))
        ctx.save_for_backward(x, wp, *weights)
        ctx.n = n
        return y

    @staticmethod
    def backward(ctx, dy):
        x, wp, *weights = ctx.saved_tensors
        n, cd = ctx.n, x.dtype
        M, K = x.shape[0], x.shape[1] // n
        N = wp.shape[0] // n
        dy = dy.contiguous()
        g = dy if dy.dtype == cd else _cast_new(dy, cd)
        g3, x3 = BranchLinearFn._views(g, n), BranchLinearFn._views(x, n)
        dx = None
        if ctx.needs_input_grad[0]:
            dx = torch.empty(M, n * K, dtype=cd, device=x.device)
            ops.gemm(g3, wp.view(n, N, K), BranchLinearFn._views(dx, n), trans_b=True)
        dws = [None] * n
        if any(ctx.needs_input_grad[2:]):
            gw = torch.empty(n, N, K, dtype=torch.float32, device=x.device)
            if is_half(cd):
                ops.gemm_tn_batched(g3, x3, gw, M)
            else:
                ops.gemm(g3, x3, gw, trans_a=True, trans_b=True)
            for i, w_ in enumerate(weights):
                if ctx.needs_input_grad[2 + i]:
                    tgt = direct_grad_target(w_)
                    if tgt is not None:
                        ops.axpby(gw[i].view(-1), 1.0, tgt.view(-1), 1.0)
                    else:
                        dws[i] = gw[i].view(w_.shape)
        return (dx, None) + tuple(dws)


def branch_linear(x, weights):
    return BranchLinearFn.apply(x, len(weights), *weights)


class LayerNormFn(torch.autograd.Function):
    @staticmethod
    def forward(ctx, x, w, b, eps, out_dtype):
        x = x.contiguous()
        M, C = x.shape
        y = torch.empty(M, C, dtype=out_dtype, device=x.device)
        stats = torch.empty(M, 2, dtype=torch.float32, device=x.device)
        ops.layernorm_fwd(x, w.detach(), b.detach(), eps, y, stats)
        ctx.save_for_backward(x, w, b, stats)
        return y

    @staticmethod
    def backward(ctx, dy):
        x, w, b, stats = ctx.saved_tensors
        C = x.shape[1]
        dx = torch.empty_like(x)
        dw, db, ret_w, ret_b = _norm_grad_slots(w, b, C, x.device)
        ops.layernorm_bwd(dy.contiguous(), x, w.detach(), stats, dx, False, dw, db)
        return dx, ret_w, ret_b, None, None


def layer_norm(x, w, b, eps=1e-5, out_dtype=None):
    return LayerNormFn.apply(x, w, b, eps, out_dtype or compute_dtype())


class BatchNormActFn(torch.autograd.Function):

    @staticmethod
    def forward(ctx, x, w, b, running_mean, running_var, momentum, eps, act, out_dtype, sync, world):
        x = x.contiguous()
        rows, C = x.shape
        sums = torch.empty(2, C, dtype=torch.float32, device=x.device)
        ops.bn_moments(x, sums)
        total = rows * world
        if sync is not None:
            sync(sums)
        mv = torch.empty(2, C, dtype=torch.float32, device=x.device)
        ops.bn_finalize(sums, total, mv, running_mean, running_var, momentum)
        y = torch.empty(rows, C, dtype=out_dtype, device=x.device)
        ops.bn_apply(x, mv, w.detach(), b.detach(), eps, act, y)
        ctx.save_for_backward(x, w, b, mv)
        ctx.cfg = (eps, act, sync, total)
        return y

    @staticmethod
    def backward(ctx, dy):
        x, w, b, mv = ctx.saved_tensors
        eps, act, sync, total = ctx.cfg
        rows, C = x.shape
        dy = dy.contiguous()
        sd = torch.empty(2, C, dtype=torch.float32, device=x.device)
        ops.bn_bwd_reduce(dy, x, mv, w.detach(), b.detach(), eps, act, sd)
        tw, tb = direct_grad_target(w), direct_grad_target(b)
        if tw is not None and tb is not None:
            ops.axpby(sd[1], 1.0, tw.view(-1), 1.0)
            ops.axpby(sd[0], 1.0, tb.view(-1), 1.0)
            dw = db = None
        else:
            db, dw = sd[0].clone(), sd[1].clone()
        if sync is not None:
            sync(sd)
        dx = torch.empty_like(x)
        ops.bn_bwd_apply(dy, x, mv, w.detach(), b.detach(), eps, act, sd, total, dx)
        return dx, dw, db, None, None, None, None, None, None, None, None


def batch_norm_act_train(x, w, b, running_mean, running_var, momentum=0.1, eps=1e-5, act=ops.ACT_NONE, out_dtype=None,
                         sync=None, world=1):
    return BatchNormActFn.apply(x, w, b, running_mean, running_var, momentum, eps, act, out_dtype or compute_dtype(), sync, world)


def batch_norm_act_eval(x, w, b, running_mean, running_var, eps=1e-5, act=ops.ACT_NONE, out_dtype=None):
    mv = torch.stack([running_mean.detach().float(), running_var.detach().float()]).contiguous()
    y = torch.empty(x.shape, dtype=out_dtype or compute_dtype(), device=x.device)
    ops.bn_apply(x.contiguous(), mv, w.detach(), b.detach(), eps, act, y)
    return y


class SelfAttnFn(torch.autograd.Function):

    @staticmethod
    def forward(ctx, qkv, B, N, H, d):
        inner = H * d
        o = torch.empty(B * N, inner, dtype=qkv.dtype, device=qkv.device)
        lse = torch.empty(B, H, N, dtype=torch.float32, device=qkv.device)
        ops.attn_fwd(qkv[:, :inner], qkv[:, inner:2 * inner], qkv[:, 2 * inner:], o, lse, B, H, d, N, 0, N, 0, d ** -0.5,
                     keep_split=ctx.needs_input_grad[0])
        ctx.save_for_backward(qkv, o, lse)
        ctx.cfg = (B, N, H, d)
        return o

    @staticmethod
    def backward(ctx, do):
        qkv, o, lse = ctx.saved_tensors
        B, N, H, d = ctx.cfg
        inner = H * d
        dqkv = torch.empty_like(qkv)
        ops.attn_bwd(qkv[:, :inner], qkv[:, inner:2 * inner], qkv[:, 2 * inner:], o, lse, do.contiguous(), dqkv[:, :inner],
                     dqkv[:, inner:2 * inner], dqkv[:, 2 * inner:], B, H, d, N, 0, N, 0, d ** -0.5)
        return dqkv, None, None, None, None


class CrossAttnFn(torch.autograd.Function):

    @staticmethod
    def forward(ctx, q, kv, B, Nq, Nk, H, d):
        inner = H * d
        o = torch.empty(B * Nq, inner, dtype=q.dtype, device=q.device)
        lse = torch.empty(B, H, Nq, dtype=torch.float32, device=q.device)
        ops.attn_fwd(q, kv[:, :inner], kv[:, inner:], o, lse, B, H, d, Nq, 0, Nk, 0, d ** -0.5)
        ctx.save_for_backward(q, kv, o, lse)
        ctx.cfg = (B, Nq, Nk, H, d)
        return o

    @staticmethod
    def backward(ctx, do):
        q, kv, o, lse = ctx.saved_tensors
        B, Nq, Nk, H, d = ctx.cfg
        inner = H * d
        dq, dkv = torch.empty_like(q), torch.empty_like(kv)
        ops.attn_bwd(q, kv[:, :inner], kv[:, inner:], o, lse, do.contiguous(), dq, dkv[:, :inner], dkv[:, inner:], B, H, d, Nq,
                     0, Nk, 0, d ** -0.5)
        return dq, dkv, None, None, None, None, None


class GegluFn(torch.autograd.Function):
    @staticmethod
    def forward(ctx, h):
        M, c2 = h.shape
        out = torch.empty(M, c2 // 2, dtype=h.dtype, device=h.device)
        ops.geglu_fwd(h, out)
        ctx.save_for_backward(h)
        return out

    @staticmethod
    def backward(ctx, dout):
        (h,) = ctx.saved_tensors
        dh = torch.empty_like(h)
        ops.geglu_bwd(h, dout.contiguous(), dh)
        return dh


class DropoutFn(torch.autograd.Function):

    @staticmethod
    def forward(ctx, x, p, rows_per_group):
        M, C = x.shape
        g = (M + rows_per_group - 1) // rows_per_group
        mask = torch.empty(g, C, dtype=torch.float32, device=x.device)
        seed, off = _next_rng(g * C)
        ops.dropout_mask(mask, p, seed, off)
        y = torch.empty_like(x)
        ops.mul_mask(x, mask, y, rows_per_group)
        ctx.save_for_backward(mask)
        ctx.rpg = rows_per_group
        return y

    @staticmethod
    def backward(ctx, dy):
        (mask,) = ctx.saved_tensors
        dx = torch.empty_like(dy)
        ops.mul_mask(dy.contiguous(), mask, dx, ctx.rpg)
        return dx, None, None


def dropout(x, p, training, rows_per_group=1):
    if not training or p <= 0:
        return x
    return DropoutFn.apply(x, p, rows_per_group)


class MaskTokenFn(torch.autograd.Function):
    @staticmethod
    def forward(ctx, x, keep_u8, token):
        out = torch.empty_like(x)
        ops.mask_token_fwd(x.contiguous(), keep_u8, token.detach().reshape(-1).contiguous(), out)
        ctx.save_for_backward(keep_u8)
        ctx.tshape = token.shape
        return out

    @staticmethod
    def backward(ctx, dout):
        (keep,) = ctx.saved_tensors
        dx = torch.empty_like(dout)
        dt = torch.empty(dout.shape[1], dtype=torch.float32, device=dout.device)
        ops.mask_token_bwd(dout.contiguous(), keep, dx, dt)
        return dx, None, dt.view(ctx.tshape)


class UnblockFn(torch.autograd.Function):

    @staticmethod
    def forward(ctx, x, B, H, W, levels):
        C = x.shape[-1]
        y = torch.empty(B, H, W, C, dtype=torch.float32, device=x.device)
        ops.unblock(x.contiguous(), y, B, H, W, C, levels, False)
        ctx.cfg = (B, H, W, C, levels, x.shape)
        return y

    @staticmethod
    def backward(ctx, dy):
        B, H, W, C, levels, shp = ctx.cfg
        dx = torch.empty(shp, dtype=torch.float32, device=dy.device)
        ops.unblock(dy.contiguous(), dx, B, H, W, C, levels, True)
        return dx, None, None, None, None


class UpsampleCEFn(torch.autograd.Function):

    @staticmethod
    def forward(ctx, logits_low, label, ignore_index, loss_weight):
        loss, acc, dl = ops.upsample_ce_loss_acc(logits_low.contiguous(), label, ignore_index, need_grad=True)
        ctx.save_for_backward(dl)
        ctx.lw = loss_weight
        ctx.mark_non_differentiable(acc)
        if loss_weight != 1.0:
            ops.axpby(loss, loss_weight, loss, 0.0)
        return loss.view(()), acc

    @staticmethod
    def backward(ctx, dloss, _):
        (dl,) = ctx.saved_tensors
        g = dl.clone() if False else dl
        ops.scale_by_device_scalar(g, dloss.contiguous().view(1))
        if ctx.lw != 1.0:
            ops.axpby(g, ctx.lw, g, 0.0)
        return g, None, None, None


class UpsampleCEWeightedFn(torch.autograd.Function):

    @staticmethod
    def forward(ctx, logits_low, label, weight, ignore_index, loss_weight):
        loss, acc, dl = ops.upsample_ce_w_loss_acc(logits_low.contiguous(), label, weight, ignore_index, need_grad=True)
        ctx.save_for_backward(dl)
        ctx.lw = loss_weight
        ctx.mark_non_differentiable(acc)
        if loss_weight != 1.0:
            ops.axpby(loss, loss_weight, loss, 0.0)
        return loss.view(()), acc

    @staticmethod
    def backward(ctx, dloss, _):
        (g,) = ctx.saved_tensors
        ops.scale_by_device_scalar(g, dloss.contiguous().view(1))
        if ctx.lw != 1.0:
            ops.axpby(g, ctx.lw, g, 0.0)
        return g, None, None, None, None


class UpsampleCEAllFn(torch.autograd.Function):

    @staticmethod
    def forward(ctx, logits_low, label, ignore_index, loss_weight):
        loss, counts, dl = ops.upsample_ce(logits_low.contiguous(), label, ignore_index, need_grad=True)
        ctx.save_for_backward(dl)
        ctx.lw = loss_weight
        acc = counts[:1].to(torch.float32)
        ops.axpby(acc, 100.0 / label.numel(), acc, 0.0)
        ctx.mark_non_differentiable(acc)
        if loss_weight != 1.0:
            ops.axpby(loss, loss_weight, loss, 0.0)
        return loss.view(()), acc

    @staticmethod
    def backward(ctx, dloss, _):
        (g,) = ctx.saved_tensors
        ops.scale_by_device_scalar(g, dloss.contiguous().view(1))
        if ctx.lw != 1.0:
            ops.axpby(g, ctx.lw, g, 0.0)
        return g, None, None, None


class HrdaFuseFn(torch.autograd.Function):

    @staticmethod
    def forward(ctx, lr, a, hr, offset, mask_box):
        lr, a, hr = lr.contiguous(), a.contiguous(), hr.contiguous()
        B, h, w, C = lr.shape
        fused = torch.empty(B, 2 * h, 2 * w, C, dtype=torch.float32, device=lr.device)
        att = torch.empty_like(lr)
        lrs = torch.empty_like(lr)
        ops.hrda_fuse_fwd(lr, a, hr, offset, mask_box, fused, att, lrs)
        ctx.save_for_backward(lr, a, hr, att)
        ctx.geo = (tuple(offset), None if mask_box is None else tuple(mask_box))
        ctx.mark_non_differentiable(lrs)
        return fused, lrs

    @staticmethod
    def backward(ctx, d_fused, _):
        lr, a, hr, att = ctx.saved_tensors
        offset, mask_box = ctx.geo
        d_lr, d_a, d_hr = torch.empty_like(lr), torch.empty_like(a), torch.empty_like(hr)
        ops.hrda_fuse_bwd(d_fused.contiguous(), lr, a, hr, att, offset, mask_box, d_lr, d_a, d_hr)
        return d_lr, d_a, d_hr, None, None
```

vfmseg_amd/heads.py:

```python
import torch
import torch.nn as nn

from . import functional as Fh
from . import ops
from .precision import compute_dtype, is_half
from .registry import MODELS


class FeatPack:

    def __init__(self, xcat, B, hp, wp):
        self.xcat, self.B, self.hp, self.wp = xcat, B, hp, wp

    def taps_nchw(self):
        n = 4
        c = self.xcat.shape[1] // n
        v = self.xcat.view(self.B, self.hp, self.wp, n, c)
        return tuple(v[:, :, :, i].permute(0, 3, 1, 2) for i in range(n))


def as_featpack(inputs, in_index=(0, 1, 2, 3)):
    if isinstance(inputs, FeatPack):
        return inputs
    feats = [inputs[i] for i in in_index]
# ... 117 lines not shown

        class _ConvModule(nn.Module):
            def __init__(s):
                super().__init__()
                s.conv = nn.Conv2d(c * n, c, 1, bias=False)
                s.gn = nn.GroupNorm(self.norm_cfg.get("num_groups", 32), c)

        self.fusion_conv = _ConvModule()
        self.output_upscaling = nn.Sequential(
            nn.ConvTranspose2d(c, c // 2, kernel_size=2, stride=2),
            nn.BatchNorm2d(c // 2),
            nn.GELU(),
            nn.ConvTranspose2d(c // 2, c // 4, kernel_size=2, stride=2),
            nn.GELU(),
        )
        self.bn_sync = None
        self.bn_world = 1

    @_fp32_on_fp32_taps
    def forward_tokens(self, fp):
        cd = compute_dtype()
        B, P = fp.B, fp.hp * fp.wp
        fc, up = self.fusion_conv, self.output_upscaling
        y = Fh.linear(fp.xcat, fc.conv.weight, "conv1x1", out_dtype=torch.float32)
        y = Fh.group_norm_act(y, fc.gn.weight, fc.gn.bias, B, P, fc.gn.num_groups, fc.gn.eps, ops.ACT_RELU, cd)
        y = Fh.linear(y, up[0].weight, "convT2x2", bias=up[0].bias, bias_tile=4, out_dtype=torch.float32)
        y = y.view(4 * B * P, -1)
        bn = up[1]
        if self.training:
            y = Fh.batch_norm_act_train(y, bn.weight, bn.bias, bn.running_mean, bn.running_var, bn.momentum, bn.eps,
                                        ops.ACT_GELU, cd, self.bn_sync, self.bn_world)
            with torch.no_grad():
                bn.num_batches_tracked += 1
        else:
            y = Fh.batch_norm_act_eval(y, bn.weight, bn.bias, bn.running_mean, bn.running_var, bn.eps, ops.ACT_GELU, cd)
        y = Fh.linear(y, up[3].weight, "convT2x2", bias=up[3].bias, bias_tile=4, act="gelu", out_dtype=cd)
        y = y.view(16 * B * P, -1)
        y = Fh.dropout(y, self.dropout_ratio, self.training, rows_per_group=16 * P)
        lg = Fh.linear(y, self.conv_seg.weight, "conv1x1", bias=self.conv_seg.bias, out_dtype=torch.float32)
        return Fh.UnblockFn.apply(lg.view(B, 16 * P, -1), B, 4 * fp.hp, 4 * fp.wp, 2)

    def forward(self, inputs):
        return self.forward_tokens(as_featpack(inputs, self.in_index)).permute(0, 3, 1, 2)

    def loss(self, inputs, seg_label, return_logits=False):
        lg = self.forward_tokens(as_featpack(inputs, self.in_index))
        return self._loss_from_lowres(lg, seg_label, return_logits)

    def predict(self, inputs, batch_img_metas, test_cfg=None):
        return self.predict_by_feat(self.forward_tokens(as_featpack(inputs, self.in_index)), batch_img_metas)


@MODELS.register_module()
class SegformerHead(BaseDecodeHead):

    def __init__(self, interpolate_mode="bilinear", **kwargs):
        super().__init__(input_transform="multiple_select", **kwargs)
        if interpolate_mode != "bilinear":
            raise NotImplementedError(f"SegformerHead: interpolate_mode={interpolate_mode!r}: the taps of the reference configs share one size, "
                                      "only the (identity) bilinear resize is on the HIP path")
        if (self.norm_cfg or {}).get("type") != "GN":
            raise NotImplementedError("SegformerHead: only norm_cfg=dict(type='GN') (the reference configs) is on the HIP path")
        if (self.act_cfg or {}).get("type") != "ReLU":
            raise NotImplementedError("SegformerHead: only act_cfg=dict(type='ReLU') is on the HIP path")
        n = len(self.in_channels)
        assert n == len(self.in_index)
        if any(c != self.in_channels[0] for c in self.in_channels):
            raise NotImplementedError("SegformerHead: taps of differing width are not on the HIP path (one batched embedding GEMM)")
        ch, groups = self.channels, self.norm_cfg.get("num_groups", 32)

        class _ConvModule(nn.Module):
            def __init__(s, cin):
                super().__init__()
                s.conv = nn.Conv2d(cin, ch, 1, bias=False)
                s.gn = nn.GroupNorm(groups, ch)

        self.convs = nn.ModuleList([_ConvModule(c) for c in self.in_channels])
        self.fusion_conv = _ConvModule(ch * n)
        self._gn_pack = Fh.NormParamPack()

    @_fp32_on_fp32_taps
    def forward_tokens(self, fp):
        cd = compute_dtype()
        B, P = fp.B, fp.hp * fp.wp
        n, fc = len(self.convs), self.fusion_conv
        if fp.xcat.shape[1] != sum(self.in_channels):
            raise NotImplementedError("SegformerHead: the feature pack does not hold one tap per in_channels entry")
        gn0 = self.convs[0].gn
        y = Fh.branch_linear(fp.xcat, [m.conv.weight for m in self.convs])
        y = Fh.group_norm_cat_act(y, [m.gn.weight for m in self.convs], [m.gn.bias for m in self.convs], B, P, gn0.num_groups, gn0.eps,
                                  ops.ACT_RELU, cd, pack=self._gn_pack)
        y = Fh.linear(y, fc.conv.weight, "conv1x1", out_dtype=torch.float32)
        y = Fh.group_norm_cat_act(y, [fc.gn.weight], [fc.gn.bias], B, P, fc.gn.num_groups, fc.gn.eps, ops.ACT_RELU, cd)
        y = Fh.dropout(y, self.dropout_ratio, self.training, rows_per_group=P)
        lg = Fh.linear(y, self.conv_seg.weight, "conv1x1", bias=self.conv_seg.bias, out_dtype=torch.float32)
        return lg.view(B, fp.hp, fp.wp, -1)

    def _pack(self, inputs):
        if not isinstance(inputs, FeatPack):
            feats = [inputs[i] for i in self.in_index]
            if any(f.shape[2:] != feats[0].shape[2:] for f in feats):
                raise NotImplementedError("SegformerHead: taps of differing size (resize_feat / multi-resolution necks) are not on the HIP path")
        return as_featpack(inputs, self.in_index)

    def forward(self, inputs):
        return self.forward_tokens(self._pack(inputs)).permute(0, 3, 1, 2)

    def loss(self, inputs, seg_label, return_logits=False):
        return self._loss_from_lowres(self.forward_tokens(self._pack(inputs)), seg_label, return_logits)

    def predict(self, inputs, batch_img_metas, test_cfg=None):
        return self.predict_by_feat(self.forward_tokens(self._pack(inputs)), batch_img_metas)


class _CrossAttention(nn.Module):
    def __init__(self, query_dim, context_dim=None, heads=8, dim_head=64, dropout=0.0):
        super().__init__()
        inner = heads * dim_head
        context_dim = context_dim or query_dim
        self.heads, self.dim_head, self.p = heads, dim_head, dropout
        self.to_q = nn.Linear(query_dim, inner, bias=False)
        self.to_k = nn.Linear(context_dim, inner, bias=False)
        self.to_v = nn.Linear(context_dim, inner, bias=False)
        self.to_out = nn.Sequential(nn.Linear(inner, query_dim), nn.Dropout(dropout))


class _GEGLU(nn.Module):
    def __init__(self, dim_in, dim_out):
        super().__init__()
        self.proj = nn.Linear(dim_in, dim_out * 2)


class _FeedForward(nn.Module):
    def __init__(self, dim, mult=4, dropout=0.0):
        super().__init__()
        self.p = dropout
        self.net = nn.Sequential(_GEGLU(dim, dim * mult), nn.Dropout(dropout), nn.Linear(dim * mult, dim))


class BasicTransformerBlock(nn.Module):

    def __init__(self, query_dim, n_heads, d_head, dropout=0.0, context_dim=None):
        super().__init__()
        self.attn1 = _CrossAttention(query_dim, None, n_heads, d_head, dropout)
        self.ff = _FeedForward(query_dim, dropout=dropout)
        self.attn2 = _CrossAttention(query_dim, context_dim, n_heads, d_head, dropout)
        self.norm1, self.norm2, self.norm3 = nn.LayerNorm(query_dim), nn.LayerNorm(query_dim), nn.LayerNorm(query_dim)

    def run(self, x, ctx, B, N, Nk, training):
        cd = compute_dtype()
        a1, a2, ff = self.attn1, self.attn2, self.ff
        H, d = a1.heads, a1.dim_head
        lin = ["linear"]
        h = Fh.layer_norm(x, self.norm1.weight, self.norm1.bias, self.norm1.eps, cd)
        qkv = Fh.linear(h, [a1.to_q.weight, a1.to_k.weight, a1.to_v.weight], lin * 3, out_dtype=cd)
        o = Fh.SelfAttnFn.apply(qkv, B, N, H, d)
        x = Fh.linear(o, a1.to_out[0].weight, "linear", bias=a1.to_out[0].bias, residual=x, out_dtype=torch.float32,
                      drop_p=a1.p if training else 0.0)
        h = Fh.layer_norm(x, self.norm2.weight, self.norm2.bias, self.norm2.eps, cd)
        q = Fh.linear(h, a2.to_q.weight, "linear", out_dtype=cd)
        kv = Fh.linear(ctx, [a2.to_k.weight, a2.to_v.weight], lin * 2, out_dtype=cd)
        o = Fh.CrossAttnFn.apply(q, kv, B, N, Nk, H, d)
        x = Fh.linear(o, a2.to_out[0].weight, "linear", bias=a2.to_out[0].bias, residual=x, out_dtype=torch.float32,
                      drop_p=a2.p if training else 0.0)
        h = Fh.layer_norm(x, self.norm3.weight, self.norm3.bias, self.norm3.eps, cd)
        g = Fh.GegluFn.apply(Fh.linear(h, ff.net[0].proj.weight, "linear", bias=ff.net[0].proj.bias, out_dtype=cd))
        g = Fh.dropout(g, ff.p, training)
        return Fh.linear(g, ff.net[2].weight, "linear", bias=ff.net[2].bias, residual=x, out_dtype=torch.float32)


@MODELS.register_module()
class TransformerDecoder(nn.Module):

    def __init__(self, query_dim, img_feat_dim, n_heads, d_head, depth=1, dropout=0.0):
        super().__init__()
        self.in_channels = query_dim
        self.norm = nn.GroupNorm(32, query_dim, eps=1e-6)
        self.transformer_blocks = nn.ModuleList(
            [BasicTransformerBlock(query_dim, n_heads, d_head, dropout, img_feat_dim) for _ in range(depth)])

    def run_tokens(self, query_f32, ctx_cd, B, P, Pk):
        x = Fh.group_norm_act(query_f32, self.norm.weight, self.norm.bias, B, P, 32, self.norm.eps, ops.ACT_NONE, torch.float32)
        for blk in self.transformer_blocks:
            x = blk.run(x, ctx_cd, B, P, Pk, self.training)
        return x


@MODELS.register_module()
class MaskTransformerDecoder(TransformerDecoder):

    def __init__(self, mask_ratio, **kwargs):
        super().__init__(**kwargs)
        self.mask_ratio = mask_ratio
        self.mask_token = nn.Parameter(torch.randn(1, self.in_channels, 1, 1))
        self.mask_enable = True
        self.fixed_keep = None

    def draw_keep(self, B, P, device):
        if self.fixed_keep is not None:
            return self.fixed_keep.reshape(B * P).to(device=device, dtype=torch.uint8).contiguous()
        m = torch.empty(B * P, dtype=torch.float32, device=device)
        seed, off = Fh._next_rng(B * P)
        ops.dropout_mask(m, self.mask_ratio, seed, off)
        return (m > 0).to(torch.uint8)

    def run_tokens(self, query_f32, ctx_cd, B, P, Pk):
        if self.mask_enable:
            query_f32 = Fh.MaskTokenFn.apply(query_f32, self.draw_keep(B, P, query_f32.device), self.mask_token)
        return super().run_tokens(query_f32, ctx_cd, B, P, Pk)


class CastFn(torch.autograd.Function):
    @staticmethod
    def forward(ctx, x, dtype):
        ctx.src = x.dtype
        if x.dtype == dtype:
            return x
        out = torch.empty(x.shape, dtype=dtype, device=x.device)
        ops.cast(x, out)
        return out

    @staticmethod
    def backward(ctx, dy):
        if dy.dtype == ctx.src:
            return dy, None
        out = torch.empty(dy.shape, dtype=ctx.src, device=dy.device)
        ops.cast(dy.contiguous(), out)
        return out, None


@MODELS.register_module()
class VFMHead(BaseDecodeHead):
    def __init__(self, transformer, interpolate_mode="bilinear", **kwargs):
        super().__init__(input_transform="multiple_select", **kwargs)
        n = len(self.in_channels)
        assert n == len(self.in_index) == 4
        transformer = dict(transformer)
        transformer["img_feat_dim"] = self.channels
        self.query_dim = transformer["query_dim"]
        ch = self.channels
        self.fuse_conv = nn.Sequential(nn.Conv2d(self.in_channels[0] * n, ch, 1), nn.GroupNorm(32, ch), nn.GELU())
        self.seg_logits_embed = nn.Sequential(
            nn.Conv2d(19, ch // 4, kernel_size=2, stride=2), nn.GroupNorm(32, ch // 4), nn.GELU(),
            nn.Conv2d(ch // 4, ch // 2, kernel_size=2, stride=2), nn.GroupNorm(32, ch // 2), nn.GELU(),
            nn.Conv2d(ch // 2, ch, kernel_size=1), nn.GroupNorm(32, ch),
        )
        self.transformer_decoder = MODELS.build(transformer)

    @staticmethod
    def ctx_windows_ok(seg, boxes, hp, wp):
        H, W = seg.shape[2:]
        ok = True
        for (y1, y2, x1, x2) in boxes:
            hc, wc = y2 - y1, x2 - x1
            ok = ok and hc % (4 * hp) == 0 and wc % (4 * wp) == 0 and hc // (4 * hp) == wc // (4 * wp)
            if ok:
                s_ = hc // (4 * hp)
                ok = y1 % s_ == 0 and x1 % s_ == 0 and H % s_ == 0 and W % s_ == 0
        return ok and len(boxes) > 0

    @_fp32_on_fp32_taps
    def forward_tokens(self, fp, ctx_nchw, ctx_windows=None):
        cd = compute_dtype()
        B, hp, wp = fp.B, fp.hp, fp.wp
        P = hp * wp
        emb, fc = self.seg_logits_embed, self.fuse_conv
        if ctx_windows is not None:
            seg, boxes = ctx_windows
            seg = seg.detach()
            assert seg.is_contiguous() and seg.dtype == torch.float32 and len(boxes) * seg.shape[0] == B
            Bimg, Cc, H, W = seg.shape
            dev = seg.device
        else:
            ctx_nchw = ctx_nchw.detach().contiguous()
            Cc, Hc, Wc = ctx_nchw.shape[1:]
            dev = ctx_nchw.device
        kpad = 128 if 4 * Cc <= 128 else (4 * Cc + 63) // 64 * 64
        a1 = torch.zeros(B * 4 * P, kpad, dtype=cd, device=dev)
        if ctx_windows is not None:
            for j, (y1, y2, x1, x2) in enumerate(boxes):
                s_ = (y2 - y1) // (4 * hp)
                ops.resize_bilinear(seg, True, Bimg, H, W, Cc, a1[j * Bimg * 4 * P:(j + 1) * Bimg * 4 * P], 2, (H // s_, W // s_),
                                    window=(y1 // s_, x1 // s_, 4 * hp, 4 * wp), out_ld=kpad)
        else:
            ops.resize_bilinear(ctx_nchw, True, B, Hc, Wc, Cc, a1, 2, (4 * hp, 4 * wp), out_ld=kpad)
        e = Fh.linear(a1, emb[0].weight, "conv2x2s2", bias=emb[0].bias, out_dtype=torch.float32)
        e = Fh.group_norm_act(e, emb[1].weight, emb[1].bias, B, 4 * P, 32, emb[1].eps, ops.ACT_GELU, cd)
        e = Fh.linear(e.view(B * P, -1), emb[3].weight, "conv2x2s2", bias=emb[3].bias, out_dtype=torch.float32)
        e = Fh.group_norm_act(e, emb[4].weight, emb[4].bias, B, P, 32, emb[4].eps, ops.ACT_GELU, cd)
        e = Fh.linear(e, emb[6].weight, "conv1x1", bias=emb[6].bias, out_dtype=torch.float32)
        e = Fh.group_norm_act(e, emb[7].weight, emb[7].bias, B, P, 32, emb[7].eps, ops.ACT_NONE, cd)
        f = Fh.linear(fp.xcat, fc[0].weight, "conv1x1", bias=fc[0].bias, out_dtype=torch.float32)
        f = Fh.group_norm_act(f, fc[1].weight, fc[1].bias, B, P, 32, fc[1].eps, ops.ACT_GELU, torch.float32)
        x = self.transformer_decoder.run_tokens(f, e, B, P, P)
        x = CastFn.apply(x, cd)
        x = Fh.dropout(x, self.dropout_ratio, self.training, rows_per_group=P)
        lg = Fh.linear(x, self.conv_seg.weight, "conv1x1", bias=self.conv_seg.bias, out_dtype=torch.float32)
        return lg.view(B, hp, wp, -1)

    def forward(self, inputs, seg_logits, query=None):
        return self.forward_tokens(as_featpack(inputs, self.in_index), seg_logits).permute(0, 3, 1, 2)

    def loss(self, inputs, seg_logits_embed, seg_label, query=None, return_logits=False):
        lg = self.forward_tokens(as_featpack(inputs, self.in_index), seg_logits_embed)
        return self._loss_from_lowres(lg, seg_label, return_logits)


@MODELS.register_module()
class AttentionHead(BaseDecodeHead):

    def __init__(self, interpolate_mode="bilinear", **kwargs):
        super().__init__(input_transform="multiple_select", **kwargs)
        n = len(self.in_channels)
        assert n == len(self.in_index) == 4
        if (self.norm_cfg or {}).get("type") != "GN":
            raise NotImplementedError("AttentionHead: only norm_cfg=dict(type='GN') (the reference config) is on the HIP path")
        cin, ch, groups = self.in_channels[0] * n, self.channels, self.norm_cfg.get("num_groups", 32)

        class _ConvModule(nn.Module):
            def __init__(s):
# ... 153 lines not shown
```

vfmseg_amd/lib.py:

```python
import ctypes as C
import os

import torch

_HERE = os.path.dirname(os.path.abspath(__file__))
LIB_PATH = os.path.join(_HERE, "csrc", "libvfmseg_hip.so")
LIB_PATH_F16 = os.path.join(_HERE, "csrc", "libvfmseg_hip_f16.so")

F32, BF16, U8, I64, SPLIT3 = 0, 1, 2, 3, 4
ABI_VERSION = 6
EP_NONE, EP_GELU, EP_RELU, EP_MUL_GELU_GRAD, EP_MUL, EP_QGELU, EP_MUL_QGELU_GRAD, EP_GELU_DGELU = 0, 1, 2, 3, 4, 5, 6, 7
ACT_NONE, ACT_GELU, ACT_RELU, ACT_QGELU = 0, 1, 2, 3

vp, ci, cl, cf, u64 = C.c_void_p, C.c_int, C.c_long, C.c_float, C.c_uint64


class GemmDesc(C.Structure):
    _fields_ = [
        ("A", vp), ("B", vp), ("C", vp),
        ("in_dt", ci), ("c_dt", ci),
        ("M", cl), ("N", cl), ("K", cl),
        ("sa_m", cl), ("sa_k", cl), ("sb_n", cl), ("sb_k", cl), ("ldc", cl),
        ("alpha", cf),
        ("bias", vp), ("bias_mod", cl),
        ("colscale", vp),
        ("residual", vp), ("r_dt", ci), ("ldr", cl),
        ("ep_mode", ci), ("aux", vp), ("aux_dt", ci), ("ld_aux", cl),
        ("C2", vp), ("c2_dt", ci), ("ldc2", cl),
        ("batch", cl), ("stride_a", cl), ("stride_b", cl), ("stride_c", cl),
        ("c_plane", cl),
        ("kb_rows", cl),
    ]


class AttnDesc(C.Structure):
    _fields_ = [
        ("q", vp), ("k", vp), ("v", vp), ("o", vp),
        ("dt", ci), ("ldq", cl), ("ldk", cl), ("ldv", cl), ("ldo", cl),
        ("B", ci), ("H", ci), ("d", ci),
        ("nq_main", ci), ("nq_extra", ci), ("nk_main", ci), ("nk_extra", ci),
        ("scale", cf),
        ("lse", vp),
        ("dout", vp), ("ld_do", cl),
        ("dq", vp), ("dk", vp), ("dv", vp), ("ld_dq", cl), ("ld_dk", cl), ("ld_dv", cl),
        ("delta", vp),
    ]


class _LnFwd(C.Structure):
    _fields_ = [("x", vp), ("ld_x", cl), ("w", vp), ("b", vp), ("eps", cf), ("y", vp), ("y_dt", ci), ("ld_y", cl), ("stats", vp),
                ("rows", cl), ("C", cl)]


class _LnDrop(C.Structure):
    _fields_ = [("x", vp), ("ld_x", cl), ("w", vp), ("b", vp), ("eps", cf), ("y", vp), ("ld_y", cl), ("stats", vp), ("y_drop", vp),
                ("ld_yd", cl), ("mask", vp), ("ld_mask", cl), ("p", cf), ("offset", u64), ("rows", cl), ("C", cl)]


class _LnBwd(C.Structure):
    _fields_ = [("dy", vp), ("dy_dt", ci), ("ld_dy", cl), ("x", vp), ("ld_x", cl), ("w", vp), ("stats", vp), ("dx", vp), ("ld_dx", cl),
                ("accumulate_dx", ci), ("t_out", vp), ("ld_t", cl), ("t_scale", vp), ("rows", cl), ("C", cl)]


class _CastOp(C.Structure):
    _fields_ = [("src", vp), ("src_dt", ci), ("ld_src", cl), ("dst", vp), ("dst_dt", ci), ("ld_dst", cl), ("rows", cl), ("cols", cl),
                ("colscale", vp)]


class _CopyOp(C.Structure):
    _fields_ = [("src", vp), ("src_dt", ci), ("dst", vp), ("dst_dt", ci), ("n", cl * 4), ("ss", cl * 4), ("ds", cl * 4), ("accumulate", ci)]


class _PlanU(C.Union):
    _fields_ = [("gemm", GemmDesc), ("attn", AttnDesc), ("ln_fwd", _LnFwd), ("ln_drop", _LnDrop), ("ln_bwd", _LnBwd), ("cast", _CastOp),
                ("copy", _CopyOp)]


class PlanOp(C.Structure):
    _fields_ = [("kind", ci), ("prof_kind", ci), ("flops", C.c_double), ("u", _PlanU)]


OP_GEMM, OP_LN_FWD, OP_LN_DROPOUT_FWD, OP_LN_BWD_SCALED, OP_ATTN_FWD, OP_ATTN_BWD, OP_CAST, OP_STRIDED_COPY = range(8)
PROF_NONE, PROF_GEMM, PROF_GEMM_TN, PROF_ATTN_FWD, PROF_ATTN_BWD = range(5)
PROF_NAMES = {PROF_GEMM: "gemm", PROF_GEMM_TN: "gemm_tn", PROF_ATTN_FWD: "attn_fwd", PROF_ATTN_BWD: "attn_bwd"}


class SlideWin(C.Structure):
    _fields_ = [("crop", vp), ("nchw", ci), ("h", ci), ("w", ci), ("y0", ci), ("x0", ci), ("hc", ci), ("wc", ci)]


SIGNATURES = {
    "vfm_cast": [vp, ci, cl, vp, ci, cl, cl, cl, vp, vp],
    "vfm_split3": [vp, cl, cl, vp, cl, cl, cl, ci, vp],
    "vfm_transpose": [vp, ci, cl, vp, ci, cl, cl, cl, cl, vp],
    "vfm_strided_copy": [vp, ci, vp, ci] + [cl] * 12 + [ci, vp],
    "vfm_strided_copy_batch": [vp, ci, cl, vp],
    "vfm_axpby": [vp, cf, vp, cf, cl, vp],
    "vfm_scale_by_device_scalar": [vp, vp, cl, vp],
    "vfm_colsum": [vp, ci, cl, cl, cl, vp, ci, vp, vp],
    "vfm_preprocess_u8": [vp, ci, ci, vp, ci, ci, C.POINTER(C.c_float), C.POINTER(C.c_float), ci, cf, vp],
    "vfm_lora_pack": [vp, ci, cl, ci, vp],
    "vfm_slab_reduce": [vp, ci, cl, cl, cl, cf, vp, cl, cl, ci, vp],
    "vfm_dropout_mask": [vp, ci, cl, cf, u64, u64, vp],
    "vfm_mul_mask": [vp, ci, cl, vp, ci, cl, cl, vp, ci, cl, cl, cl, vp],
    "vfm_geglu_fwd": [vp, ci, cl, vp, ci, cl, cl, cl, vp],
    "vfm_geglu_bwd": [vp, ci, cl, vp, ci, cl, vp, ci, cl, cl, cl, vp],
    "vfm_swiglu_fwd": [vp, ci, cl, vp, ci, cl, cl, cl, vp],
    "vfm_swiglu_bwd": [vp, ci, cl, vp, ci, cl, vp, ci, cl, cl, cl, vp],
    "vfm_rope": [vp, ci, cl, cl, ci, ci, ci, vp, vp, ci, vp],
    "vfm_act_grad_mul": [vp, ci, cl, vp, ci, cl, vp, ci, cl, cl, cl, ci, vp],
    "vfm_mask_token_fwd": [vp, vp, vp, vp, cl, cl, vp],
    "vfm_mask_token_bwd": [vp, vp, vp, vp, vp, cl, cl, vp],
    "vfm_layernorm_fwd": [vp, cl, vp, vp, cf, vp, ci, cl, vp, cl, cl, vp],
    "vfm_layernorm_fwd_split3": [vp, cl, vp, vp, cf, vp, cl, vp, cl, cl, vp, cl, cl, vp],
    "vfm_layernorm_dropout_fwd": [vp, cl, vp, vp, cf, vp, cl, vp, vp, cl, vp, cl, cf, u64, u64, cl, cl, vp],
    "vfm_layernorm_bwd_scaled": [vp, ci, cl, vp, cl, vp, vp, vp, cl, ci, vp, cl, vp, cl, cl, vp],
    "vfm_layernorm_bwd": [vp, ci, cl, vp, cl, vp, vp, vp, cl, ci, vp, vp, vp, cl, cl, vp],
    "vfm_groupnorm_fwd": [vp, vp, vp, cf, ci, ci, vp, ci, vp, vp, cl, cl, cl, vp],
    "vfm_groupnorm_bwd": [vp, ci, vp, vp, vp, vp, ci, ci, vp, vp, vp, vp, cl, cl, cl, vp],
    "vfm_groupnorm_tile_ok": [cl, cl, ci],
    "vfm_groupnorm_tile_fwd": [vp, vp, vp, cf, ci, ci, vp, ci, vp, cl, cl, cl, vp],
    "vfm_groupnorm_tile_bwd": [vp, ci, vp, vp, vp, vp, ci, ci, vp, vp, vp, vp, cl, cl, cl, vp],
    "vfm_bn_moments": [vp, cl, cl, vp, vp, vp],
    "vfm_bn_finalize": [vp, cf, vp, vp, vp, cf, cl, vp],
    "vfm_bn_apply": [vp, vp, vp, vp, cf, ci, vp, ci, cl, cl, vp],
    "vfm_bn_bwd_reduce": [vp, ci, vp, vp, vp, vp, cf, ci, vp, vp, cl, cl, vp],
    "vfm_bn_bwd_apply": [vp, ci, vp, vp, vp, vp, cf, ci, vp, cf, vp, cl, cl, vp],
    "vfm_gemm": [C.POINTER(GemmDesc), vp],
    "vfm_tune": [C.c_char_p, ci],
    "vfm_attn_fwd": [C.POINTER(AttnDesc), vp],
    "vfm_attn_fwd_x3": [C.POINTER(AttnDesc), cl, vp],
    "vfm_attn_fwd_x3_split": [C.POINTER(AttnDesc), cl, vp, cl, cl, vp],
    "vfm_attn_bwd": [C.POINTER(AttnDesc), vp],
    "vfm_attn_bwd_x3": [C.POINTER(AttnDesc), vp, vp, vp, cl, cl, vp, cl, cl, vp],
    "vfm_sam_relpos_table": [vp, ci, ci, ci, vp, vp],
    "vfm_sam_attn_prep": [vp, ci, cl, vp, vp, vp, vp, vp, vp, ci, ci, ci, ci, ci, ci, ci, ci, cf, vp],
    "vfm_softmax_rows": [vp, cl, vp, ci, cl, cl, ci, ci, vp],
    "vfm_sam_attn_merge": [vp, ci, vp, cl, ci, ci, ci, ci, ci, ci, vp],
    "vfm_sam_attn_bwd_prep": [vp, cl, vp, cl, vp, ci, vp, vp, vp, vp, ci, ci, ci, ci, ci, ci, ci, cf, vp],
    "vfm_softmax_rows_batched": [vp, cl, vp, ci, cl, cl, ci, ci, ci, ci, vp],
    "vfm_softmax_rows_bwd": [vp, vp, cl, vp, ci, cl, cl, ci, ci, ci, ci, vp],
    "vfm_rein_mix_fwd": [vp, cl, vp, vp, vp, cl, vp, cl, vp, cl, cl, ci, ci, cf, vp],
    "vfm_rein_mix_bwd": [vp, cl, vp, cl, vp, vp, vp, cl, vp, cl, cl, ci, ci, cf, vp],
    "vfm_sam_attn_bwd_merge": [vp, vp, vp, ci, vp, vp, vp, cl, ci, ci, ci, ci, ci, ci, ci, ci, cf, vp],
    "vfm_sam_attn_flash_fwd": [vp, cl, vp, vp, vp, vp, cl, ci, ci, ci, ci, ci, cf, vp],
    "vfm_sam_attn_flash_fwd_train": [vp, cl, vp, vp, vp, vp, cl, ci, ci, ci, ci, ci, cf, vp, vp, vp],
    "vfm_sam_attn_flash_bwd": [vp, cl, vp, vp, vp, vp, vp, cl, vp, vp, vp, vp, cl, ci, ci, ci, ci, ci, cf, vp],
    "vfm_patchify": [vp, cl, cl, cl, ci, ci, ci, ci, ci, vp, ci, cl, ci, vp],
    "vfm_assemble_tokens": [vp, vp, vp, vp, ci, ci, ci, vp],
    "vfm_resize_bilinear": [vp, ci, ci, ci, ci, ci, ci, cl, vp, ci, ci, cl, ci, ci, ci, ci, ci, ci, cf, cf, vp],
    "vfm_resize_bicubic": [vp, ci, ci, ci, vp, ci, ci, C.c_double, C.c_double, vp],
    "vfm_label_resize": [vp, ci, ci, ci, vp, ci, ci, ci, ci, ci, ci, vp],
    "vfm_unblock": [vp, vp, ci, ci, ci, ci, ci, ci, vp],
    "vfm_upsample_ce": [vp, vp, ci, ci, ci, ci, ci, ci, ci, vp, vp, vp, vp],
    "vfm_upsample_ce_w": [vp, vp, vp, ci, ci, ci, ci, ci, ci, ci, vp, vp, vp, vp],
    "vfm_pseudo_label": [vp, ci, ci, ci, ci, ci, ci, cf, vp, vp, vp, vp],
    "vfm_class_presence": [vp, ci, cl, vp, vp],
    "vfm_class_mix": [vp, vp, vp, vp, vp, vp, cl, ci, ci, ci, ci, ci, vp, vp, vp, vp, vp],
    "vfm_hrda_fuse_fwd": [vp, vp, vp] + [ci] * 14 + [vp, vp, vp, vp],
    "vfm_hrda_fuse_bwd": [vp, vp, vp, vp, vp] + [ci] * 14 + [vp, vp, vp, vp, vp],
    "vfm_reduce_sum": [vp, cl, cf, vp, vp],
    "vfm_ce_finish": [vp, cl, cf, vp, cf, vp, vp, vp],
    "vfm_conf_gate": [vp, ci, ci, ci, ci, ci, ci, ci, ci, cf, vp, vp],
    "vfm_slide_accumulate": [vp, ci, ci, ci, ci, ci, vp, vp, ci, ci, ci, ci, ci, ci, vp],
    "vfm_slide_finalize": [vp, vp, vp, ci, ci, ci, ci, vp],
    "vfm_slide_gather": [vp, ci, ci, ci, vp, ci, ci, vp],
    "vfm_conf_gate_windows": [vp, ci, ci, ci, ci, vp, ci, cf, vp, vp],
    "vfm_confusion_hist": [vp, vp, ci, cl, ci, ci, vp, vp],
    "vfm_adamw": [vp, vp, vp, vp, cl, vp, vp, vp, ci, cf, cf, cf, cf, ci, cf, ci, ci, vp],
    "vfm_adamw_guarded": [vp, vp, vp, vp, cl, vp, vp, vp, ci, cf, cf, cf, cf, ci, cf, ci, ci, vp, vp, vp],
    "vfm_amp_update": [vp, vp, cf, cf, ci, ci, vp],
    "vfm_run_plan": [C.POINTER(PlanOp), ci, u64, u64, vp],
    "vfm_prof_config": [ci],
    "vfm_prof_read": [C.POINTER(C.c_double), ci],
}

_lib = None
_libs = {}
_half = 0
HALF_DTYPES = (torch.bfloat16, torch.float16)


class HipLibraryMissing(RuntimeError):
    pass


def _open(kind):
    path = LIB_PATH_F16 if kind else LIB_PATH
    if not os.path.exists(path):
        raise HipLibraryMissing(
            f"{path} not found: build it with `python -m vfmseg_amd.csrc.build` (hipcc --offload-arch=gfx950)")
    lib = C.CDLL(path)
    lib.vfm_last_error.restype = C.c_char_p
    lib.vfm_abi_version.restype = ci
    lib.vfm_half_kind.restype = ci
    if lib.vfm_abi_version() < ABI_VERSION:
        raise HipLibraryMissing(f"{path} has ABI version {lib.vfm_abi_version()}, this binding needs {ABI_VERSION}: rebuild (python -m vfmseg_amd.csrc.build)")
    if lib.vfm_half_kind() != kind:
        raise HipLibraryMissing(f"{path} reports half kind {lib.vfm_half_kind()}, expected {kind}: stale build")
    for name, args in SIGNATURES.items():
        fn = getattr(lib, name)
        fn.argtypes = args
        fn.restype = ci
    return lib


def load():
    global _lib
    if _lib is not None:
        return _lib
    if _half not in _libs:
        _libs[_half] = _open(_half)
    _lib = _libs[_half]
    return _lib


def set_half(kind):
    global _half, _lib
    kind = {torch.bfloat16: 0, torch.float16: 1, "bf16": 0, "fp16": 1, "f16": 1}.get(kind, kind)
    assert kind in (0, 1)
    if kind != _half:
        _half, _lib = kind, None


def half_dtype():
    return torch.float16 if _half else torch.bfloat16


class HipError(RuntimeError):
    pass


def check(rc, name):
    if rc != 0:
        raise HipError(f"{name} failed ({rc}): {load().vfm_last_error().decode()}")


_raw_stream = getattr(torch._C, "_cuda_getCurrentRawStream", None)
_dev_index = None


def stream():
    global _dev_index
    if _raw_stream is not None:
        if _dev_index is None:
            _dev_index = torch.cuda.current_device()
        return _raw_stream(_dev_index)
    return torch.cuda.current_stream().cuda_stream


def set_device_index(i):
    global _dev_index
    _dev_index = i


def dt_of(t):
    if t.dtype == torch.float32:
        return F32
    if t.dtype == torch.bfloat16 or t.dtype == torch.float16:
        if (t.dtype == torch.float16) != bool(_half):
            raise TypeError(f"{t.dtype} tensor handed to the {'fp16' if _half else 'bf16'} library (precision mode and tensors disagree)")
        return BF16
    if t.dtype == torch.uint8 or t.dtype == torch.bool:
        return U8
    if t.dtype == torch.int64:
        return I64
    raise TypeError(f"unsupported dtype {t.dtype}")


def torch_dt(code):
# ... 10 lines not shown
```

vfmseg_amd/ops.py:

```python
import ctypes as C
import os

import torch

from .precision import is_half
from . import lib as L
from .lib import (ACT_GELU, ACT_NONE, ACT_QGELU, ACT_RELU, BF16, EP_GELU, EP_GELU_DGELU, EP_MUL, EP_MUL_GELU_GRAD,
                  EP_MUL_QGELU_GRAD, EP_NONE, EP_QGELU, EP_RELU, F32)

_ws_cache = {}

PROFILE = None
REGION = ["heads"]


class region:
    def __init__(self, name):
        self.name = name

    def __enter__(self):
        REGION.append(self.name)

    def __exit__(self, *a):
        REGION.pop()


def workspace(nfloats, device, tag="default"):
    key = (str(device), tag, L.stream())
    t = _ws_cache.get(key)
    if t is None or t.numel() < nfloats:
        t = torch.empty(max(int(nfloats), 1 << 16), dtype=torch.float32, device=device)
        _ws_cache[key] = t
    return t


def ld_pad(cols, dtype):
    esz = torch.empty(0, dtype=dtype).element_size()
    return (256 // esz) if (cols * esz) % 8192 == 0 else 0


def empty_ld(rows, cols, dtype, device, zero=False):
    pad = ld_pad(cols, dtype)
    make = torch.zeros if zero else torch.empty
    if pad == 0:
        return make(rows, cols, dtype=dtype, device=device)
    return make(rows, cols + pad, dtype=dtype, device=device)[:, :cols]


def _ld(t):
    assert t.dim() == 2 and t.stride(1) == 1, "expected a row-major 2-D view"
    return t.stride(0)


def cast(src, dst, colscale=None):
    lib = L.load()
    L.check(lib.vfm_cast(L.ptr(src), L.dt_of(src), _ld(src), L.ptr(dst), L.dt_of(dst), _ld(dst), src.shape[0], src.shape[1],
                         L.ptr(colscale), L.stream()), "vfm_cast")
    return dst


def transpose(src, dst, pad_rows=None):
    lib = L.load()
    rows, cols = src.shape
    pad_rows = rows if pad_rows is None else pad_rows
    L.check(lib.vfm_transpose(L.ptr(src), L.dt_of(src), _ld(src), L.ptr(dst), L.dt_of(dst), _ld(dst), rows, cols, pad_rows,
                              L.stream()), "vfm_transpose")
    return dst


def strided_copy(src, dst, shape, sstr, dstr, accumulate=False):
    lib = L.load()
    n = list(shape) + [1] * (4 - len(shape))
    s = list(sstr) + [0] * (4 - len(sstr))
    d = list(dstr) + [0] * (4 - len(dstr))
    k = 4 - len(shape)
    n = [1] * k + list(shape)
    s = [0] * k + list(sstr)
    d = [0] * k + list(dstr)
    L.check(lib.vfm_strided_copy(L.ptr(src), L.dt_of(src), L.ptr(dst), L.dt_of(dst), *n, *s, *d, int(accumulate), L.stream()),
            "vfm_strided_copy")
    return dst


class CopyBatch:

    def __init__(self, jobs):
        import struct
        buf = bytearray()
        self.keep, self.max_elems, self.n = [], 0, len(jobs)
        for job in jobs:
            src, dst, shape, sstr, dstr = job[:5]
            acc = int(bool(job[5])) if len(job) > 5 else 0
            nsum, sstride = (int(job[6]), int(job[7])) if len(job) > 7 else (1, 0)
            assert src.dtype == torch.float32 and src.is_cuda and dst.is_cuda and (not acc or dst.dtype == torch.float32)
            k = 4 - len(shape)
            n, s_, d_ = [1] * k + list(shape), [0] * k + list(sstr), [0] * k + list(dstr)
            buf += struct.pack("2Q16q", src.data_ptr(), dst.data_ptr(), L.dt_of(dst), acc, *n, *s_, *d_, nsum, sstride)
            self.keep += [src, dst]
            e = 1
            for v in shape:
                e *= v
            self.max_elems = max(self.max_elems, e)
        self.table = torch.frombuffer(buf, dtype=torch.uint8).clone().to(jobs[0][1].device) if jobs else None

    def run(self):
        if self.n:
            lib = L.load()
            L.check(lib.vfm_strided_copy_batch(L.ptr(self.table), self.n, self.max_elems, L.stream()), "vfm_strided_copy_batch")


def permute_copy(src, perm, dst):
    v = src.permute(*perm)
    strided_copy(src, dst, list(v.shape), list(v.stride()), list(torch.empty(v.shape, device="meta").stride()))
    return dst


def axpby(x, a, y, b):
    lib = L.load()
    assert x.is_contiguous() and y.is_contiguous() and x.dtype == y.dtype == torch.float32 and x.numel() == y.numel()
    L.check(lib.vfm_axpby(L.ptr(x), float(a), L.ptr(y), float(b), x.numel(), L.stream()), "vfm_axpby")
    return y


def scale_by_device_scalar(y, scalar):
    lib = L.load()
    assert y.is_contiguous() and y.dtype == torch.float32
    L.check(lib.vfm_scale_by_device_scalar(L.ptr(y), L.ptr(scalar), y.numel(), L.stream()), "vfm_scale_by_device_scalar")
    return y


def colsum(x, out, accumulate=False):
    lib = L.load()
    rows, cols = x.shape
    ws = workspace(64 * cols, x.device)
    L.check(lib.vfm_colsum(L.ptr(x), L.dt_of(x), _ld(x), rows, cols, L.ptr(out), int(accumulate), L.ptr(ws), L.stream()),
            "vfm_colsum")
    return out


def dropout_mask(out, p, seed, offset=0):
    lib = L.load()
    assert out.is_contiguous()
    L.check(lib.vfm_dropout_mask(L.ptr(out), L.dt_of(out), out.numel(), float(p), int(seed), int(offset), L.stream()),
            "vfm_dropout_mask")
    return out


def mul_mask(src, mask, dst, rows_per_group=1):
    lib = L.load()
    L.check(lib.vfm_mul_mask(L.ptr(src), L.dt_of(src), _ld(src), L.ptr(mask), L.dt_of(mask), _ld(mask), rows_per_group,
                             L.ptr(dst), L.dt_of(dst), _ld(dst), src.shape[0], src.shape[1], L.stream()), "vfm_mul_mask")
    return dst


def geglu_fwd(h, out):
    lib = L.load()
    rows, c2 = h.shape
    L.check(lib.vfm_geglu_fwd(L.ptr(h), L.dt_of(h), _ld(h), L.ptr(out), L.dt_of(out), _ld(out), rows, c2 // 2, L.stream()),
            "vfm_geglu_fwd")
    return out


def geglu_bwd(h, dout, dh):
    lib = L.load()
    rows, c2 = h.shape
    L.check(lib.vfm_geglu_bwd(L.ptr(h), L.dt_of(h), _ld(h), L.ptr(dout), L.dt_of(dout), _ld(dout), L.ptr(dh), L.dt_of(dh),
                              _ld(dh), rows, c2 // 2, L.stream()), "vfm_geglu_bwd")
    return dh


def swiglu_fwd(h, out, C_):
    lib = L.load()
    L.check(lib.vfm_swiglu_fwd(L.ptr(h), L.dt_of(h), _ld(h), L.ptr(out), L.dt_of(out), _ld(out), h.shape[0], C_, L.stream()),
            "vfm_swiglu_fwd")
    return out


def swiglu_bwd(h, dout, dh, C_):
    lib = L.load()
    L.check(lib.vfm_swiglu_bwd(L.ptr(h), L.dt_of(h), _ld(h), L.ptr(dout), L.dt_of(dout), _ld(dout), L.ptr(dh), L.dt_of(dh),
                               _ld(dh), h.shape[0], C_, L.stream()), "vfm_swiglu_bwd")
    return dh


def rope(x, rows, np_, ncols, d, cos_t, sin_t, inverse=False):
    lib = L.load()
    L.check(lib.vfm_rope(L.ptr(x), L.dt_of(x), _ld(x), rows, np_, ncols, d, L.ptr(cos_t), L.ptr(sin_t), int(inverse), L.stream()),
            "vfm_rope")
    return x


def act_grad_mul(dy, pre, out, act):
    lib = L.load()
    L.check(lib.vfm_act_grad_mul(L.ptr(dy), L.dt_of(dy), _ld(dy), L.ptr(pre), L.dt_of(pre), _ld(pre), L.ptr(out),
                                 L.dt_of(out), _ld(out), dy.shape[0], dy.shape[1], act, L.stream()), "vfm_act_grad_mul")
    return out


def mask_token_fwd(x, keep, token, out):
    lib = L.load()
    L.check(lib.vfm_mask_token_fwd(L.ptr(x), L.ptr(keep), L.ptr(token), L.ptr(out), x.shape[0], x.shape[1], L.stream()),
            "vfm_mask_token_fwd")
    return out


def mask_token_bwd(dout, keep, dx, dtoken):
    lib = L.load()
    ws = workspace(64 * dout.shape[1], dout.device)
    L.check(lib.vfm_mask_token_bwd(L.ptr(dout), L.ptr(keep), L.ptr(dx), L.ptr(dtoken), L.ptr(ws), dout.shape[0], dout.shape[1],
                                   L.stream()), "vfm_mask_token_bwd")


def _split_key(t):
    return (t.data_ptr(), tuple(t.shape), tuple(t.stride()), t._version)


def _register_split_out(t, t3):
    try:
        t._vfm_split3_out = (_split_key(t), t3)
    except AttributeError:
        pass


def layernorm_fwd(x, w, b, eps, y, stats=None, split_out=None):
    lib = L.load()
    rows, c = x.shape
    if split_out and _split3_on() and y.dtype == torch.float32 and c % 256 == 0 and c // 256 in (1, 2, 4, 5, 8) and y.shape[1] == c:
        kp = (c + 63) // 64 * 64
        y3 = torch.empty(rows, 3 * kp, dtype=L.half_dtype(), device=x.device)
        L.check(lib.vfm_layernorm_fwd_split3(L.ptr(x), _ld(x), L.ptr(w), L.ptr(b), float(eps), None if split_out == "only" else L.ptr(y), _ld(y),
                                             L.ptr(y3), y3.stride(0), kp, L.ptr(stats), rows, c, L.stream()), "vfm_layernorm_fwd_split3")
        _register_split_out(y, y3)
        return y
    L.check(lib.vfm_layernorm_fwd(L.ptr(x), _ld(x), L.ptr(w), L.ptr(b), float(eps), L.ptr(y), L.dt_of(y), _ld(y),
                                  L.ptr(stats), rows, c, L.stream()), "vfm_layernorm_fwd")
    return y


def layernorm_dropout_fwd(x, w, b, eps, y, stats, y_drop, mask, p, seed, offset=0):
    lib = L.load()
    rows, c = x.shape
    assert is_half(y.dtype) and is_half(y_drop.dtype) and is_half(mask.dtype)
    L.check(lib.vfm_layernorm_dropout_fwd(L.ptr(x), _ld(x), L.ptr(w), L.ptr(b), float(eps), L.ptr(y), _ld(y), L.ptr(stats),
                                          L.ptr(y_drop), _ld(y_drop), L.ptr(mask), _ld(mask), float(p), int(seed), int(offset),
                                          rows, c, L.stream()), "vfm_layernorm_dropout_fwd")
    return y


def layernorm_bwd_scaled(dy, x, w, stats, dx, t_out, t_scale, accumulate_dx=False):
    lib = L.load()
    rows, c = x.shape
    assert is_half(t_out.dtype) and t_scale.dtype == torch.float32
    L.check(lib.vfm_layernorm_bwd_scaled(L.ptr(dy), L.dt_of(dy), _ld(dy), L.ptr(x), _ld(x), L.ptr(w), L.ptr(stats), L.ptr(dx),
                                         _ld(dx), int(accumulate_dx), L.ptr(t_out), _ld(t_out), L.ptr(t_scale), rows, c,
                                         L.stream()), "vfm_layernorm_bwd_scaled")
    return dx


def layernorm_bwd(dy, x, w, stats, dx, accumulate_dx=False, dw=None, db=None):
    lib = L.load()
    rows, c = x.shape
    ws = workspace(2 * 128 * c, x.device) if (dw is not None or db is not None) else None
    L.check(lib.vfm_layernorm_bwd(L.ptr(dy), L.dt_of(dy), _ld(dy), L.ptr(x), _ld(x), L.ptr(w), L.ptr(stats), L.ptr(dx),
                                  _ld(dx), int(accumulate_dx), L.ptr(dw), L.ptr(db), L.ptr(ws), rows, c, L.stream()),
            "vfm_layernorm_bwd")
    return dx


def groupnorm_fwd(x, w, b, eps, groups, act, y, stats, B, P):
    lib = L.load()
    c = x.shape[1]
    ws = workspace(B * groups * 2 + B * 64 * 2 * c, x.device)
    L.check(lib.vfm_groupnorm_fwd(L.ptr(x), L.ptr(w), L.ptr(b), float(eps), groups, act, L.ptr(y), L.dt_of(y), L.ptr(stats),
                                  L.ptr(ws), B, P, c, L.stream()), "vfm_groupnorm_fwd")
    return y


def groupnorm_bwd(dy, x, w, b, stats, groups, act, dx, dw, db, B, P):
    lib = L.load()
    c = x.shape[1]
    ws = workspace(B * groups * 2 + B * 64 * 2 * c, x.device)
    L.check(lib.vfm_groupnorm_bwd(L.ptr(dy), L.dt_of(dy), L.ptr(x), L.ptr(w), L.ptr(b), L.ptr(stats), groups, act, L.ptr(dx),
                                  L.ptr(dw), L.ptr(db), L.ptr(ws), B, P, c, L.stream()), "vfm_groupnorm_bwd")
    return dx


def groupnorm_tile_ok(P, C, groups):
    return bool(L.load().vfm_groupnorm_tile_ok(int(P), int(C), int(groups)))


def groupnorm_tile_fwd(x, w, b, eps, groups, act, y, stats, B, P):
    lib = L.load()
    L.check(lib.vfm_groupnorm_tile_fwd(L.ptr(x), L.ptr(w), L.ptr(b), float(eps), groups, act, L.ptr(y), L.dt_of(y), L.ptr(stats),
                                       B, P, x.shape[1], L.stream()), "vfm_groupnorm_tile_fwd")
    return y


def groupnorm_tile_bwd(dy, x, w, b, stats, groups, act, dx, dw, db, B, P):
    lib = L.load()
    c = x.shape[1]
    ws = workspace(B * 2 * c, x.device)
    L.check(lib.vfm_groupnorm_tile_bwd(L.ptr(dy), L.dt_of(dy), L.ptr(x), L.ptr(w), L.ptr(b), L.ptr(stats), groups, act, L.ptr(dx),
                                       L.ptr(dw), L.ptr(db), L.ptr(ws), B, P, c, L.stream()), "vfm_groupnorm_tile_bwd")
    return dx


def bn_moments(x, sums):
    lib = L.load()
    rows, c = x.shape
    ws = workspace(64 * 2 * c, x.device)
    L.check(lib.vfm_bn_moments(L.ptr(x), rows, c, L.ptr(sums), L.ptr(ws), L.stream()), "vfm_bn_moments")
    return sums


def bn_finalize(sums, count, mean_var, running_mean=None, running_var=None, momentum=0.1):
    lib = L.load()
    L.check(lib.vfm_bn_finalize(L.ptr(sums), float(count), L.ptr(mean_var), L.ptr(running_mean), L.ptr(running_var),
                                float(momentum), sums.shape[1], L.stream()), "vfm_bn_finalize")
    return mean_var


def bn_apply(x, mean_var, w, b, eps, act, y):
    lib = L.load()
    rows, c = x.shape
    L.check(lib.vfm_bn_apply(L.ptr(x), L.ptr(mean_var), L.ptr(w), L.ptr(b), float(eps), act, L.ptr(y), L.dt_of(y), rows, c,
                             L.stream()), "vfm_bn_apply")
    return y


def bn_bwd_reduce(dy, x, mean_var, w, b, eps, act, sums_dy):
    lib = L.load()
    rows, c = x.shape
    ws = workspace(64 * 2 * c, x.device)
    L.check(lib.vfm_bn_bwd_reduce(L.ptr(dy), L.dt_of(dy), L.ptr(x), L.ptr(mean_var), L.ptr(w), L.ptr(b), float(eps), act,
                                  L.ptr(sums_dy), L.ptr(ws), rows, c, L.stream()), "vfm_bn_bwd_reduce")
    return sums_dy


def bn_bwd_apply(dy, x, mean_var, w, b, eps, act, sums_dy, total_rows, dx):
    lib = L.load()
    rows, c = x.shape
    L.check(lib.vfm_bn_bwd_apply(L.ptr(dy), L.dt_of(dy), L.ptr(x), L.ptr(mean_var), L.ptr(w), L.ptr(b), float(eps), act,
                                 L.ptr(sums_dy), float(total_rows), L.ptr(dx), rows, c, L.stream()), "vfm_bn_bwd_apply")
    return dx


def split3(x, pattern, trans=False, cache=False):
    if pattern == 0 and not trans:
        hit = getattr(x, "_vfm_split3_out", None)
        if hit is not None and hit[0] == _split_key(x):
            return hit[1]
    if cache:
        from .optim import PARAM_EPOCH
        key = (PARAM_EPOCH[0], x._version, x.data_ptr(), pattern, trans, tuple(x.shape), tuple(x.stride()))
        hit = getattr(x, "_vfm_split3", None)
        if hit is not None and hit[0] == key:
            return hit[1]
    rows, K = (x.shape[1], x.shape[0]) if trans else (x.shape[0], x.shape[1])
    sr, sc = (x.stride(1), x.stride(0)) if trans else (x.stride(0), x.stride(1))
    kp = (K + 63) // 64 * 64
    out = torch.empty(rows, 3 * kp, dtype=L.half_dtype(), device=x.device)
    L.check(L.load().vfm_split3(L.ptr(x), sr, sc, L.ptr(out), out.stride(0), rows, K, pattern, L.stream()), "vfm_split3")
    if cache:
        try:
            x._vfm_split3 = (key, out)
        except AttributeError:
            pass
    return out


def gemm(a, b, c, *, alpha=1.0, bias=None, bias_mod=0, colscale=None, residual=None, ep_mode=EP_NONE, aux=None, c2=None,
         trans_a=False, trans_b=False, kb_rows=0, c_split=None):
    if a.dtype == torch.float32 and b.dtype == torch.float32 and a.dim() == 2 and not kb_rows and _split3_on():
        a3 = split3(a, 0, trans=trans_a)
        b3 = split3(b, 1, trans=trans_b, cache=not b.requires_grad)
        c3 = None
        if (c_split == "only" and c.dtype == torch.float32 and c.dim() == 2 and c.shape[1] % 64 == 0 and residual is None and c2 is None
                and ep_mode in (EP_NONE, EP_GELU)):
            c3 = torch.empty(c.shape[0], 3 * c.shape[1], dtype=L.half_dtype(), device=c.device)
        gemm(a3, b3, c, alpha=alpha, bias=bias, bias_mod=bias_mod, colscale=colscale, residual=residual, ep_mode=ep_mode, aux=aux, c2=c2, c_split=c3)
        if c3 is not None:
            _register_split_out(c, c3)
        return c
    lib = L.load()
    d = gemm_desc(a, b, c, alpha=alpha, bias=bias, bias_mod=bias_mod, colscale=colscale, residual=residual, ep_mode=ep_mode, aux=aux, c2=c2,
                  trans_a=trans_a, trans_b=trans_b, kb_rows=kb_rows)
    if torch.is_tensor(c_split):
        d.C, d.c_dt, d.ldc, d.c_plane = L.ptr(c_split), L.SPLIT3, c_split.stride(0), c.shape[1]
    fin = PROFILE("gemm", 2.0 * d.M * d.N * d.K * d.batch, REGION[-1]) if (PROFILE is not None and is_half(a.dtype)) else None
    L.check(lib.vfm_gemm(C.byref(d), L.stream()), "vfm_gemm")
    if fin is not None:
        fin()
    return c


def gemm_desc(a, b, c, *, alpha=1.0, bias=None, bias_mod=0, colscale=None, residual=None, ep_mode=EP_NONE, aux=None, c2=None,
              trans_a=False, trans_b=False, kb_rows=0, d=None):
    d = L.GemmDesc() if d is None else d
    batched = a.dim() == 3
    a2 = a[0] if batched else a
    b2 = b[0] if batched else b
    c2d = c[0] if batched else c
    if trans_a:
        K, M = a2.shape
        d.sa_m, d.sa_k = a2.stride(1), a2.stride(0)
    else:
        M, K = a2.shape
        d.sa_m, d.sa_k = a2.stride(0), a2.stride(1)
    if trans_b:
        Kb, N = b2.shape
        d.sb_n, d.sb_k = b2.stride(1), b2.stride(0)
    else:
        N, Kb = b2.shape
        d.sb_n, d.sb_k = b2.stride(0), b2.stride(1)
    if kb_rows:
        assert trans_b and Kb == kb_rows and K >= Kb, "kb_rows: b holds the first kb_rows of the K (token) dimension"
        d.kb_rows = int(kb_rows)
    else:
# ... 788 lines not shown
```

Before: 130.1 images/s.

## Fuse dropout, GEGLU+dropout, LayerNorm backward and colsum reductions in heads

Adds fused kernels that generate the dropout mask and apply it in one pass, combine GEGLU with dropout in forward and backward, and fold the LayerNorm backward dw/db reduction plus a residual gradient add into one kernel. A last-block ticket pattern finishes the cross-block reduction inside the same launch. The aim is fewer launches and less memory traffic in the decoder head blocks. The cost is extra complexity, atomic ticket counters that must be zero-initialised, and possible small numeric differences from the new rounding order.

New measurement: 130.2 images/s (median of 3 runs). Within noise of the previous version (+0.1%).

```diff
diff --git a/include/vfmseg_hip.h b/include/vfmseg_hip.h
--- a/include/vfmseg_hip.h
+++ b/include/vfmseg_hip.h
@@ -34,6 +34,8 @@
 int vfm_axpby(const float* x, float a, float* y, float b, long n, void* stream);
 int vfm_scale_by_device_scalar(float* y, const float* scalar, long n, void* stream);
 int vfm_colsum(const void* x, int dt, long ld, long rows, long cols, float* out, int accumulate, float* ws, void* stream);
+int vfm_colsum_fused(const void* x, int dt, long ld, long rows, long cols, float* out, int accumulate, float* ws, unsigned* counters,
+                     long n_counters, void* stream);
 typedef struct vfm_lora_site {
   const float* A; const float* B;
   void* a; void* at; void* w; void* wt;
@@ -48,6 +50,12 @@
 int vfm_geglu_fwd(const void* h, int h_dt, long ld_h, void* out, int out_dt, long ld_out, long rows, long C, void* stream);
 int vfm_geglu_bwd(const void* h, int h_dt, long ld_h, const void* dout, int do_dt, long ld_do, void* dh, int dh_dt,
                   long ld_dh, long rows, long C, void* stream);
+int vfm_dropout_apply(const void* src, int src_dt, long ld_src, void* mask, int mask_dt, long mask_ld, long rows_per_group, void* dst,
+                      int dst_dt, long ld_dst, long rows, long cols, float p, uint64_t seed, uint64_t offset, void* stream);
+int vfm_geglu_dropout_fwd(const void* h, int h_dt, long ld_h, void* out, int out_dt, long ld_out, void* mask, int mask_dt, long mask_ld,
+                          long rows, long C, float p, uint64_t seed, uint64_t offset, void* stream);
+int vfm_geglu_dropout_bwd(const void* h, int h_dt, long ld_h, const void* dout, int do_dt, long ld_do, const void* mask, int mask_dt,
+                          long mask_ld, void* dh, int dh_dt, long ld_dh, long rows, long C, void* stream);
 int vfm_swiglu_fwd(const void* h, int h_dt, long ld_h, void* out, int out_dt, long ld_out, long rows, long C, void* stream);
 int vfm_swiglu_bwd(const void* h, int h_dt, long ld_h, const void* dout, int do_dt, long ld_do, void* dh, int dh_dt,
                    long ld_dh, long rows, long C, void* stream);
@@ -72,6 +80,10 @@
 int vfm_layernorm_bwd(const void* dy, int dy_dt, long ld_dy, const float* x, long ld_x, const float* w,
                       const float* stats, float* dx, long ld_dx, int accumulate_dx, float* dw, float* db, float* ws,
                       long rows, long C, void* stream);
+int vfm_layernorm_bwd_fused_ok(long C);
+int vfm_layernorm_bwd_fused(const void* dy, int dy_dt, long ld_dy, const float* x, long ld_x, const float* w, const float* stats,
+                            const float* dx_add, long ld_add, float* dx, long ld_dx, float* dw, float* db, float* ws,
+                            unsigned* counter, long rows, long C, void* stream);
 int vfm_groupnorm_fwd(const float* x, const float* w, const float* b, float eps, int G, int act, void* y, int y_dt,
                       float* stats, float* ws, long B, long P, long C, void* stream);
 int vfm_groupnorm_bwd(const void* dy, int dy_dt, const float* x, const float* w, const float* b, const float* stats,
diff --git a/vfmseg_amd/csrc/elementwise.hip b/vfmseg_amd/csrc/elementwise.hip
--- a/vfmseg_amd/csrc/elementwise.hip
+++ b/vfmseg_amd/csrc/elementwise.hip
@@ -3,7 +3,7 @@
 thread_local char g_vfm_err[512] = {0};
 
 extern "C" const char* vfm_last_error(void) { return g_vfm_err; }
-extern "C" int vfm_abi_version(void) { return 6; }
+extern "C" int vfm_abi_version(void) { return 7; }
 extern "C" int vfm_half_kind(void) { return VFM_HALF_KIND; }
 
 template <typename TI, typename TO>
@@ -241,6 +241,83 @@
   return VFM_OK;
 }
 
+template <typename T>
+__global__ void __launch_bounds__(256) k_colsum_tk(const T* __restrict__ x, long ld, long rows, long cols, float* __restrict__ ws,
+                                                   unsigned* __restrict__ counters, float* __restrict__ out, int accumulate, int CT) {
+  __shared__ float sh[257];
+  const int rl = 256 / CT;
+  const int tx = threadIdx.x % CT, ty = threadIdx.x / CT;
+  const long c = (long)blockIdx.x * CT + tx;
+  const int parts = gridDim.y;
+  float acc = 0.f;
+  if (c < cols)
+    for (long r = (long)blockIdx.y * rl + ty; r < rows; r += (long)gridDim.y * rl) acc += ld_f32(x + r * ld + c);
+  sh[threadIdx.x] = acc;
+  __syncthreads();
+  if (ty == 0 && c < cols) {
+    float a = 0.f;
+    for (int k = 0; k < rl; ++k) a += sh[k * CT + tx];
+    if (parts == 1) {
+      const float t = ((0.f + a) + 0.f) + (0.f + 0.f);
+      out[c] = accumulate ? out[c] + t : t;
+    } else {
+      __hip_atomic_store(&ws[(long)blockIdx.y * cols + c], a, __ATOMIC_RELAXED, __HIP_MEMORY_SCOPE_AGENT);
+    }
+  }
+  if (parts == 1) return;
+  asm volatile("s_waitcnt vmcnt(0)" ::: "memory");
+  __syncthreads();
+  if (threadIdx.x == 0) {
+    const unsigned t = __hip_atomic_fetch_add(&counters[blockIdx.x], 1u, __ATOMIC_RELAXED, __HIP_MEMORY_SCOPE_AGENT);
+    const bool last = t == (unsigned)(parts - 1);
+    if (last) {
+      __builtin_amdgcn_fence(__ATOMIC_ACQUIRE, "agent");
+      asm volatile("s_waitcnt vmcnt(0)" ::: "memory");
+      __hip_atomic_store(&counters[blockIdx.x], 0u, __ATOMIC_RELAXED, __HIP_MEMORY_SCOPE_AGENT);
+    }
+    sh[256] = last ? 1.f : 0.f;
+  }
+  __syncthreads();
+  if (sh[256] == 0.f) return;
+  const int lx = threadIdx.x & 63, g = threadIdx.x >> 6;
+  const long cc = (long)blockIdx.x * CT + lx;
+  const bool live = lx < CT && cc < cols;
+  float a = 0.f;
+  if (live) {
+    int p = g;
+    for (; p + 12 < parts; p += 16) {
+      const float v0 = ws[(long)p * cols + cc], v1 = ws[(long)(p + 4) * cols + cc], v2 = ws[(long)(p + 8) * cols + cc], v3 = ws[(long)(p + 12) * cols + cc];
+      a += (v0 + v1) + (v2 + v3);
+    }
+    for (; p < parts; p += 4) a += ws[(long)p * cols + cc];
+  }
+  sh[g * 64 + lx] = a;
+  __syncthreads();
+  if (g == 0 && live) {
+    const float t = (sh[lx] + sh[64 + lx]) + (sh[128 + lx] + sh[192 + lx]);
+    out[cc] = accumulate ? out[cc] + t : t;
+  }
+}
+extern "C" int vfm_colsum_fused(const void* x, int dt, long ld, long rows, long cols, float* out, int accumulate, float* ws,
+                                unsigned* counters, long n_counters, void* stream) {
+  VFM_CHECK(ld >= cols && ws && counters, VFM_E_SHAPE, "vfm_colsum_fused: bad args");
+  if (cols == 0) return VFM_OK;
+  hipStream_t s = (hipStream_t)stream;
+  int CT = 64;
+  while (CT > 8 && CT / 2 >= cols) CT /= 2;
+  const int rl = 256 / CT;
+  long parts = (rows + rl * 8 - 1) / (rl * 8);
+  if (parts > 64) parts = 64;
+  if (parts < 1) parts = 1;
+  dim3 grid(cdiv(cols, CT), (unsigned)parts);
+  VFM_CHECK(parts == 1 || (long)grid.x <= n_counters, VFM_E_SHAPE, "vfm_colsum_fused: %u column strips, %ld counters", grid.x, n_counters);
+  if (dt == VFM_F32) hipLaunchKernelGGL(k_colsum_tk<float>, grid, dim3(256), 0, s, (const float*)x, ld, rows, cols, ws, counters, out, accumulate, CT);
+  else if (dt == VFM_BF16) hipLaunchKernelGGL(k_colsum_tk<bf16_t>, grid, dim3(256), 0, s, (const bf16_t*)x, ld, rows, cols, ws, counters, out, accumulate, CT);
+  else VFM_FAIL(VFM_E_INVAL, "vfm_colsum_fused: dtype");
+  VFM_LAUNCH_CHECK();
+  return VFM_OK;
+}
+
 __global__ void k_slab_reduce(const float* __restrict__ slabs, int kch, long P, long Q, long rows_used, float alpha,
                               float* __restrict__ dst, long sp, long sq, int accumulate) {
   const long total = rows_used * Q;
@@ -604,6 +681,209 @@
   return VFM_OK;
 }
 
+__device__ __forceinline__ float drop_mult(uint64_t seed, uint64_t ctr, float p, float keep_scale) {
+  const float u = (hash_u32(seed, ctr) >> 8) * (1.0f / 16777216.0f);
+  return u >= p ? keep_scale : 0.f;
+}
+__device__ __forceinline__ float round_h16(float v) { return bf16_to_f32(f32_to_bf16(v)); }
+__device__ __forceinline__ float round_dt(float v, int dt) { return dt == VFM_BF16 ? round_h16(v) : v; }
+template <typename T>
+__device__ __forceinline__ F8 ld8(const T* p) {
+  if constexpr (sizeof(T) == 2) return ld8_bf16(p); else return ld8_f32(p);
+}
+template <typename T>
+__device__ __forceinline__ void st8(T* p, const F8& r) {
+  if constexpr (sizeof(T) == 2) st8_bf16(p, r); else st8_f32(p, r);
+}
+template <typename T>
+__device__ __forceinline__ F8 drop_mult8(uint64_t seed, uint64_t ctr, float p, float keep_scale) {
+  F8 m;
+#pragma unroll
+  for (int e = 0; e < 8; ++e) {
+    m.v[e] = drop_mult(seed, ctr + (uint64_t)e, p, keep_scale);
+    if constexpr (sizeof(T) == 2) m.v[e] = round_h16(m.v[e]);
+  }
+  return m;
+}
+
+template <typename TS, typename TM, typename TD>
+__global__ void k_dropout_apply_x8(const TS* __restrict__ src, long ld_src, TM* __restrict__ mask, long mask_ld, long rpg, TD* __restrict__ dst,
+                                   long ld_dst, long rows, int cols8, float p, float keep_scale, uint64_t seed, uint64_t offset) {
+  const long total = rows * cols8;
+  for (long i = blockIdx.x * (long)blockDim.x + threadIdx.x; i < total; i += (long)gridDim.x * blockDim.x) {
+    const long r = i / cols8;
+    const int c = (int)(i - r * cols8) * 8;
+    const long gr = r / rpg;
+    const F8 m = drop_mult8<TM>(seed, offset + (uint64_t)(gr * ((long)cols8 * 8) + c), p, keep_scale);
+    if (r == gr * rpg) st8(mask + gr * mask_ld + c, m);
+    F8 a = ld8(src + r * ld_src + c);
+#pragma unroll
+    for (int e = 0; e < 8; ++e) a.v[e] *= m.v[e];
+    st8(dst + r * ld_dst + c, a);
+  }
+}
+__global__ void k_dropout_apply(const void* __restrict__ src, int src_dt, long ld_src, void* __restrict__ mask, int mask_dt, long mask_ld, long rpg,
+                                void* __restrict__ dst, int dst_dt, long ld_dst, long rows, long cols, float p, float keep_scale, uint64_t seed,
+                                uint64_t offset) {
+  const long total = rows * cols;
+  for (long i = blockIdx.x * (long)blockDim.x + threadIdx.x; i < total; i += (long)gridDim.x * blockDim.x) {
+    const long r = i / cols, c = i - r * cols, gr = r / rpg;
+    const float m = round_dt(drop_mult(seed, offset + (uint64_t)(gr * cols + c), p, keep_scale), mask_dt);
+    if (r == gr * rpg) st_any(mask, gr * mask_ld + c, mask_dt, m);
+    st_any(dst, r * ld_dst + c, dst_dt, ld_any(src, r * ld_src + c, src_dt) * m);
+  }
+}
+template <typename TS, typename TM, typename TD>
+static void launch_dropout_apply_x8(const void* src, long ld_src, void* mask, long mask_ld, long rpg, void* dst, long ld_dst, long rows, long cols, float p,
+                                    uint64_t seed, uint64_t offset, hipStream_t s) {
+  hipLaunchKernelGGL((k_dropout_apply_x8<TS, TM, TD>), dim3(grid8(rows * cols / 8)), dim3(256), 0, s, (const TS*)src, ld_src, (TM*)mask, mask_ld, rpg,
+                     (TD*)dst, ld_dst, rows, (int)(cols / 8), p, 1.0f / (1.0f - p), seed, offset);
+}
+extern "C" int vfm_dropout_apply(const void* src, int src_dt, long ld_src, void* mask, int mask_dt, long mask_ld, long rows_per_group, void* dst,
+                                 int dst_dt, long ld_dst, long rows, long cols, float p, uint64_t seed, uint64_t offset, void* stream) {
+  VFM_CHECK(p >= 0.f && p < 1.f, VFM_E_INVAL, "vfm_dropout_apply: p");
+  VFM_CHECK(rows_per_group >= 1 && mask_ld >= cols, VFM_E_INVAL, "vfm_dropout_apply: rows_per_group / mask_ld");
+  auto okdt = [](int dt) { return dt == VFM_BF16 || dt == VFM_F32; };
+  VFM_CHECK(okdt(src_dt) && okdt(mask_dt) && okdt(dst_dt), VFM_E_INVAL, "vfm_dropout_apply: dtype");
+  const long total = rows * cols;
+  if (total == 0) return VFM_OK;
+  hipStream_t s = (hipStream_t)stream;
+  if (cols % 8 == 0 && ld_src % 8 == 0 && mask_ld % 8 == 0 && ld_dst % 8 == 0 && al16(src) && al16(mask) && al16(dst)) {
+    const int key = (src_dt == VFM_BF16 ? 4 : 0) | (mask_dt == VFM_BF16 ? 2 : 0) | (dst_dt == VFM_BF16 ? 1 : 0);
+#define DA(TS, TM, TD) launch_dropout_apply_x8<TS, TM, TD>(src, ld_src, mask, mask_ld, rows_per_group, dst, ld_dst, rows, cols, p, seed, offset, s)
+    switch (key) {
+      case 0: DA(float, float, float); break;
+      case 1: DA(float, float, bf16_t); break;
+      case 2: DA(float, bf16_t, float); break;
+      case 3: DA(float, bf16_t, bf16_t); break;
+      case 4: DA(bf16_t, float, float); break;
+      case 5: DA(bf16_t, float, bf16_t); break;
+      case 6: DA(bf16_t, bf16_t, float); break;
+      default: DA(bf16_t, bf16_t, bf16_t); break;
+    }
+#undef DA
+    VFM_LAUNCH_CHECK();
+    return VFM_OK;
+  }
+  const int grid = (int)((total + 255) / 256 > 8192 ? 8192 : (total + 255) / 256);
+  hipLaunchKernelGGL(k_dropout_apply, dim3(grid), dim3(256), 0, s, src, src_dt, ld_src, mask, mask_dt, mask_ld, rows_per_group, dst, dst_dt, ld_dst, rows,
+                     cols, p, 1.0f / (1.0f - p), seed, offset);
+  VFM_LAUNCH_CHECK();
+  return VFM_OK;
+}
+
+template <typename TM>
+__global__ void k_geglu_dropout_fwd_x8(const bf16_t* __restrict__ h, long ld_h, bf16_t* __restrict__ out, long ld_out, TM* __restrict__ mask, long mask_ld,
+                                       long rows, long C, int c8, float p, float keep_scale, uint64_t seed, uint64_t offset) {
+  const long total = rows * c8;
+  for (long i = blockIdx.x * (long)blockDim.x + threadIdx.x; i < total; i += (long)gridDim.x * blockDim.x) {
+    const long r = i / c8;
+    const int c = (int)(i - r * c8) * 8;
+    const F8 m = drop_mult8<TM>(seed, offset + (uint64_t)(r * C + c), p, keep_scale);
+    st8(mask + r * mask_ld + c, m);
+    F8 a = ld8_bf16(h + r * ld_h + c);
+    const F8 g = ld8_bf16(h + r * ld_h + C + c);
+#pragma unroll
+    for (int e = 0; e < 8; ++e) {
+      a.v[e] *= gelu_f(g.v[e]);
+      a.v[e] = round_h16(a.v[e]) * m.v[e];
+    }
+    st8_bf16(out + r * ld_out + c, a);
+  }
+}
+__global__ void k_geglu_dropout_fwd(const void* __restrict__ h, int h_dt, long ld_h, void* __restrict__ out, int out_dt, long ld_out,
+                                    void* __restrict__ mask, int mask_dt, long mask_ld, long rows, long C, float p, float keep_scale, uint64_t seed,
+                                    uint64_t offset) {
+  const long total = rows * C;
+  for (long i = blockIdx.x * (long)blockDim.x + threadIdx.x; i < total; i += (long)gridDim.x * blockDim.x) {
+    const long r = i / C, c = i - r * C;
+    const float m = round_dt(drop_mult(seed, offset + (uint64_t)i, p, keep_scale), mask_dt);
+    st_any(mask, r * mask_ld + c, mask_dt, m);
+    const float a = ld_any(h, r * ld_h + c, h_dt), g = ld_any(h, r * ld_h + C + c, h_dt);
+    st_any(out, r * ld_out + c, out_dt, round_dt(a * gelu_f(g), out_dt) * m);
+  }
+}
+extern "C" int vfm_geglu_dropout_fwd(const void* h, int h_dt, long ld_h, void* out, int out_dt, long ld_out, void* mask, int mask_dt, long mask_ld,
+                                     long rows, long C, float p, uint64_t seed, uint64_t offset, void* stream) {
+  VFM_CHECK(p >= 0.f && p < 1.f && mask_ld >= C, VFM_E_INVAL, "vfm_geglu_dropout_fwd: p / mask_ld");
+  auto okdt = [](int dt) { return dt == VFM_BF16 || dt == VFM_F32; };
+  VFM_CHECK(okdt(h_dt) && okdt(out_dt) && okdt(mask_dt), VFM_E_INVAL, "vfm_geglu_dropout_fwd: dtype");
+  const long total = rows * C;
+  if (total == 0) return VFM_OK;
+  hipStream_t s = (hipStream_t)stream;
+  const float ks = 1.0f / (1.0f - p);
+  if (h_dt == VFM_BF16 && out_dt == VFM_BF16 && C % 8 == 0 && ld_h % 8 == 0 && ld_out % 8 == 0 && mask_ld % 8 == 0 && al16(h) && al16(out) && al16(mask)) {
+    if (mask_dt == VFM_BF16)
+      hipLaunchKernelGGL(k_geglu_dropout_fwd_x8<bf16_t>, dim3(grid8(total / 8)), dim3(256), 0, s, (const bf16_t*)h, ld_h, (bf16_t*)out, ld_out, (bf16_t*)mask,
+                         mask_ld, rows, C, (int)(C / 8), p, ks, seed, offset);
+    else
+      hipLaunchKernelGGL(k_geglu_dropout_fwd_x8<float>, dim3(grid8(total / 8)), dim3(256), 0, s, (const bf16_t*)h, ld_h, (bf16_t*)out, ld_out, (float*)mask,
+                         mask_ld, rows, C, (int)(C / 8), p, ks, seed, offset);
+    VFM_LAUNCH_CHECK();
+    return VFM_OK;
+  }
+  const int grid = (int)((total + 255) / 256 > 8192 ? 8192 : (total + 255) / 256);
+  hipLaunchKernelGGL(k_geglu_dropout_fwd, dim3(grid), dim3(256), 0, s, h, h_dt, ld_h, out, out_dt, ld_out, mask, mask_dt, mask_ld, rows, C, p, ks, seed, offset);
+  VFM_LAUNCH_CHECK();
+  return VFM_OK;
+}
+
+template <typename TM>
+__global__ void k_geglu_dropout_bwd_x8(const bf16_t* __restrict__ h, long ld_h, const bf16_t* __restrict__ dout, long ld_do, const TM* __restrict__ mask,
+                                       long mask_ld, bf16_t* __restrict__ dh, long ld_dh, long rows, long C, int c8) {
+  const long total = rows * c8;
+  for (long i = blockIdx.x * (long)blockDim.x + threadIdx.x; i < total; i += (long)gridDim.x * blockDim.x) {
+    const long r = i / c8;
+    const int c = (int)(i - r * c8) * 8;
+    const F8 a = ld8_bf16(h + r * ld_h + c), g = ld8_bf16(h + r * ld_h + C + c), m = ld8(mask + r * mask_ld + c);
+    F8 d = ld8_bf16(dout + r * ld_do + c);
+    F8 da, dg;
+#pragma unroll
+    for (int e = 0; e < 8; ++e) {
+      d.v[e] = round_h16(d.v[e] * m.v[e]);
+      da.v[e] = d.v[e] * gelu_f(g.v[e]);
+      dg.v[e] = d.v[e] * a.v[e] * gelu_grad_f(g.v[e]);
+    }
+    st8_bf16(dh + r * ld_dh + c, da);
+    st8_bf16(dh + r * ld_dh + C + c, dg);
+  }
+}
+__global__ void k_geglu_dropout_bwd(const void* __restrict__ h, int h_dt, long ld_h, const void* __restrict__ dout, int do_dt, long ld_do,
+                                    const void* __restrict__ mask, int mask_dt, long mask_ld, void* __restrict__ dh, int dh_dt, long ld_dh, long rows,
+                                    long C) {
+  const long total = rows * C;
+  for (long i = blockIdx.x * (long)blockDim.x + threadIdx.x; i < total; i += (long)gridDim.x * blockDim.x) {
+    const long r = i / C, c = i - r * C;
+    const float a = ld_any(h, r * ld_h + c, h_dt), g = ld_any(h, r * ld_h + C + c, h_dt);
+    const float d = round_dt(ld_any(dout, r * ld_do + c, do_dt) * ld_any(mask, r * mask_ld + c, mask_dt), do_dt);
+    st_any(dh, r * ld_dh + c, dh_dt, d * gelu_f(g));
+    st_any(dh, r * ld_dh + C + c, dh_dt, d * a * gelu_grad_f(g));
+  }
+}
+extern "C" int vfm_geglu_dropout_bwd(const void* h, int h_dt, long ld_h, const void* dout, int do_dt, long ld_do, const void* mask, int mask_dt,
+                                     long mask_ld, void* dh, int dh_dt, long ld_dh, long rows, long C, void* stream) {
+  auto okdt = [](int dt) { return dt == VFM_BF16 || dt == VFM_F32; };
+  VFM_CHECK(okdt(h_dt) && okdt(do_dt) && okdt(mask_dt) && okdt(dh_dt) && mask_ld >= C, VFM_E_INVAL, "vfm_geglu_dropout_bwd: dtype / mask_ld");
+  const long total = rows * C;
+  if (total == 0) return VFM_OK;
+  hipStream_t s = (hipStream_t)stream;
+  if (h_dt == VFM_BF16 && do_dt == VFM_BF16 && dh_dt == VFM_BF16 && C % 8 == 0 && ld_h % 8 == 0 && ld_do % 8 == 0 && ld_dh % 8 == 0 && mask_ld % 8 == 0 &&
+      al16(h) && al16(dout) && al16(dh) && al16(mask)) {
+    if (mask_dt == VFM_BF16)
+      hipLaunchKernelGGL(k_geglu_dropout_bwd_x8<bf16_t>, dim3(grid8(total / 8)), dim3(256), 0, s, (const bf16_t*)h, ld_h, (const bf16_t*)dout, ld_do,
+                         (const bf16_t*)mask, mask_ld, (bf16_t*)dh, ld_dh, rows, C, (int)(C / 8));
+    else
+      hipLaunchKernelGGL(k_geglu_dropout_bwd_x8<float>, dim3(grid8(total / 8)), dim3(256), 0, s, (const bf16_t*)h, ld_h, (const bf16_t*)dout, ld_do,
+                         (const float*)mask, mask_ld, (bf16_t*)dh, ld_dh, rows, C, (int)(C / 8));
+    VFM_LAUNCH_CHECK();
+    return VFM_OK;
+  }
+  const int grid = (int)((total + 255) / 256 > 8192 ? 8192 : (total + 255) / 256);
+  hipLaunchKernelGGL(k_geglu_dropout_bwd, dim3(grid), dim3(256), 0, s, h, h_dt, ld_h, dout, do_dt, ld_do, mask, mask_dt, mask_ld, dh, dh_dt, ld_dh, rows, C);
+  VFM_LAUNCH_CHECK();
+  return VFM_OK;
+}
+
 __global__ void k_swiglu_fwd(const void* __restrict__ h, int h_dt, long ld_h, void* __restrict__ out, int out_dt, long ld_out,
                              long rows, long C) {
   const long total = rows * C;
diff --git a/vfmseg_amd/csrc/norm.hip b/vfmseg_amd/csrc/norm.hip
--- a/vfmseg_amd/csrc/norm.hip
+++ b/vfmseg_amd/csrc/norm.hip
@@ -642,6 +642,130 @@
   return VFM_OK;
 }
 
+#define LNTK_THREADS 1024
+#define LNTK_MAX_PARTS 64
+template <typename TD>
+__global__ void __launch_bounds__(LNTK_THREADS) k_ln_bwd_tk(const TD* __restrict__ dy, long ld_dy, const float* __restrict__ x, long ld_x,
+                                                            const float* __restrict__ w, const float* __restrict__ stats,
+                                                            const float* __restrict__ dx_add, long ld_add, float* __restrict__ dx, long ld_dx,
+                                                            float* __restrict__ ws, unsigned* __restrict__ counter, float* __restrict__ dw,
+                                                            float* __restrict__ db, long rows, int C) {
+  constexpr int MAXPL = 4, NW = LNTK_THREADS / 64;
+  extern __shared__ float sh[];
+  const int lane = threadIdx.x & 63, wv = threadIdx.x >> 6;
+  const int C2 = 2 * C, parts = gridDim.x;
+  float pdw[MAXPL], pdb[MAXPL];
+#pragma unroll
+  for (int i = 0; i < MAXPL; ++i) pdw[i] = pdb[i] = 0.f;
+  for (long row = (long)blockIdx.x * NW + wv; row < rows; row += (long)gridDim.x * NW) {
+    const float mean = stats[row * 2], rstd = stats[row * 2 + 1];
+    float g[MAXPL], xh[MAXPL];
+    float s1 = 0.f, s2 = 0.f;
+#pragma unroll
+    for (int i = 0; i < MAXPL; ++i) {
+      const int c = i * 64 + lane;
+      if (c < C) {
+        const float d = ld_f32(dy + row * ld_dy + c);
+        xh[i] = (x[row * ld_x + c] - mean) * rstd;
+        g[i] = d * w[c];
+        s1 += g[i];
+        s2 += g[i] * xh[i];
+        pdw[i] += d * xh[i];
+        pdb[i] += d;
+      } else {
+        g[i] = xh[i] = 0.f;
+      }
+    }
+    s1 = wave_sum(s1) / C;
+    s2 = wave_sum(s2) / C;
+#pragma unroll
+    for (int i = 0; i < MAXPL; ++i) {
+      const int c = i * 64 + lane;
+      if (c < C) {
+        float v = rstd * (g[i] - s1 - xh[i] * s2);
+        asm volatile("" : "+v"(v));
+        dx[row * ld_dx + c] = dx_add ? dx_add[row * ld_add + c] + v : v;
+      }
+    }
+  }
+#pragma unroll
+  for (int i = 0; i < MAXPL; ++i) {
+    const int c = i * 64 + lane;
+    if (c < C) {
+      sh[(wv * 2 + 0) * C + c] = pdw[i];
+      sh[(wv * 2 + 1) * C + c] = pdb[i];
+    }
+  }
+  __syncthreads();
+  if ((int)threadIdx.x < C2) {
+    float a = 0.f;
+#pragma unroll
+    for (int k = 0; k < NW; ++k) a += sh[k * C2 + threadIdx.x];
+    __hip_atomic_store(&ws[(long)blockIdx.x * C2 + threadIdx.x], a, __ATOMIC_RELAXED, __HIP_MEMORY_SCOPE_AGENT);
+  }
+  asm volatile("s_waitcnt vmcnt(0)" ::: "memory");
+  __syncthreads();
+  if (threadIdx.x == 0) {
+    const unsigned t = __hip_atomic_fetch_add(counter, 1u, __ATOMIC_RELAXED, __HIP_MEMORY_SCOPE_AGENT);
+    const bool last = t == (unsigned)(parts - 1);
+    if (last) {
+      __builtin_amdgcn_fence(__ATOMIC_ACQUIRE, "agent");
+      asm volatile("s_waitcnt vmcnt(0)" ::: "memory");
+      __hip_atomic_store(counter, 0u, __ATOMIC_RELAXED, __HIP_MEMORY_SCOPE_AGENT);
+    }
+    sh[NW * C2] = last ? 1.f : 0.f;
+  }
+  __syncthreads();
+  if (sh[NW * C2] == 0.f) return;
+  float acc[2 * MAXPL];
+#pragma unroll
+  for (int s = 0; s < 2 * MAXPL; ++s) {
+    const int col = s * 64 + lane;
+    float v[LNTK_MAX_PARTS / NW];
+#pragma unroll
+    for (int j = 0; j < LNTK_MAX_PARTS / NW; ++j) {
+      const int p = wv + j * NW;
+      v[j] = (col < C2 && p < parts) ? ws[(long)p * C2 + col] : 0.f;
+    }
+    acc[s] = (v[0] + v[1]) + (v[2] + v[3]);
+  }
+#pragma unroll
+  for (int s = 0; s < 2 * MAXPL; ++s) {
+    const int col = s * 64 + lane;
+    if (col < C2) sh[wv * C2 + col] = acc[s];
+  }
+  __syncthreads();
+  if ((int)threadIdx.x < C2) {
+    float a = 0.f;
+#pragma unroll
+    for (int k = 0; k < NW; ++k) a += sh[k * C2 + threadIdx.x];
+    if ((int)threadIdx.x < C) dw[threadIdx.x] += a;
+    else db[threadIdx.x - C] += a;
+  }
+}
+extern "C" int vfm_layernorm_bwd_fused_ok(long C) { return (C > 0 && C <= 256) ? 1 : 0; }
+extern "C" int vfm_layernorm_bwd_fused(const void* dy, int dy_dt, long ld_dy, const float* x, long ld_x, const float* w, const float* stats,
+                                       const float* dx_add, long ld_add, float* dx, long ld_dx, float* dw, float* db, float* ws,
+                                       unsigned* counter, long rows, long C, void* stream) {
+  VFM_CHECK(C > 0 && C <= 256, VFM_E_SHAPE, "vfm_layernorm_bwd_fused: C=%ld is outside the one-launch kernel's coverage (C <= 256)", C);
+  VFM_CHECK(dw && db && ws && counter, VFM_E_INVAL, "vfm_layernorm_bwd_fused: dw, db, ws and counter are required");
+  VFM_CHECK(ld_dy >= C && ld_x >= C && ld_dx >= C && (!dx_add || ld_add >= C), VFM_E_SHAPE, "vfm_layernorm_bwd_fused: leading dimensions");
+  if (rows == 0) return VFM_OK;
+  hipStream_t s = (hipStream_t)stream;
+  int parts = cdiv(rows, 2 * (LNTK_THREADS / 64));
+  if (parts > LNTK_MAX_PARTS) parts = LNTK_MAX_PARTS;
+  const size_t shm = ((size_t)(LNTK_THREADS / 64) * 2 * C + 1) * sizeof(float);
+  if (dy_dt == VFM_BF16)
+    hipLaunchKernelGGL(k_ln_bwd_tk<bf16_t>, dim3(parts), dim3(LNTK_THREADS), shm, s, (const bf16_t*)dy, ld_dy, x, ld_x, w, stats, dx_add, ld_add, dx, ld_dx,
+                       ws, counter, dw, db, rows, (int)C);
+  else if (dy_dt == VFM_F32)
+    hipLaunchKernelGGL(k_ln_bwd_tk<float>, dim3(parts), dim3(LNTK_THREADS), shm, s, (const float*)dy, ld_dy, x, ld_x, w, stats, dx_add, ld_add, dx, ld_dx, ws,
+                       counter, dw, db, rows, (int)C);
+  else VFM_FAIL(VFM_E_INVAL, "vfm_layernorm_bwd_fused: dtype");
+  VFM_LAUNCH_CHECK();
+  return VFM_OK;
+}
+
 template <int MODE, typename TD>
 __global__ void k_chan_moments(const float* __restrict__ x, const TD* __restrict__ dy, const float* __restrict__ w,
                                const float* __restrict__ bb, const float* __restrict__ stats, int G, float eps, int act,
diff --git a/vfmseg_amd/functional.py b/vfmseg_amd/functional.py
--- a/vfmseg_amd/functional.py
+++ b/vfmseg_amd/functional.py
@@ -377,19 +377,21 @@
         C = x.shape[1]
         y = torch.empty(B * P, C, dtype=out_dtype, device=x.device)
         stats = torch.empty(B, groups, 2, dtype=torch.float32, device=x.device)
-        ops.groupnorm_fwd(x, w.detach(), b.detach(), eps, groups, act, y, stats, B, P)
+        fused = ops.heads_fused() and act in (ops.ACT_NONE, ops.ACT_RELU)
+        tile = fused and gn_tile_selected(P, C, groups, B)
+        (ops.groupnorm_tile_fwd if tile else ops.groupnorm_fwd)(x, w.detach(), b.detach(), eps, groups, act, y, stats, B, P)
         ctx.save_for_backward(x, w, b, stats)
-        ctx.cfg = (B, P, groups, act)
+        ctx.cfg = (B, P, groups, act, fused and gn_tile_selected(P, C, groups, B, backward=True))
         return y
 
     @staticmethod
     def backward(ctx, dy):
         x, w, b, stats = ctx.saved_tensors
-        B, P, groups, act = ctx.cfg
+        B, P, groups, act, tile = ctx.cfg
         C = x.shape[1]
         dx = torch.empty_like(x)
         dw, db, ret_w, ret_b = _norm_grad_slots(w, b, C, x.device)
-        ops.groupnorm_bwd(dy.contiguous(), x, w.detach(), b.detach(), stats, groups, act, dx, dw, db, B, P)
+        (ops.groupnorm_tile_bwd if tile else ops.groupnorm_bwd)(dy.contiguous(), x, w.detach(), b.detach(), stats, groups, act, dx, dw, db, B, P)
         return dx, ret_w, ret_b, None, None, None, None, None, None
 
 
@@ -574,6 +576,40 @@
     return LayerNormFn.apply(x, w, b, eps, out_dtype or compute_dtype())
 
 
+class LayerNormResFn(torch.autograd.Function):
+
+    @staticmethod
+    def forward(ctx, x, w, b, eps, out_dtype):
+        x = x.contiguous()
+        M, C = x.shape
+        y = torch.empty(M, C, dtype=out_dtype, device=x.device)
+        stats = torch.empty(M, 2, dtype=torch.float32, device=x.device)
+        ops.layernorm_fwd(x, w.detach(), b.detach(), eps, y, stats)
+        ctx.save_for_backward(x, w, b, stats)
+        ctx.set_materialize_grads(False)
+        return x.view_as(x), y
+
+    @staticmethod
+    def backward(ctx, gx, gy):
+        x, w, b, stats = ctx.saved_tensors
+        if gy is None:
+            return gx, None, None, None, None
+        C = x.shape[1]
+        dx = torch.empty_like(x)
+        dw, db, ret_w, ret_b = _norm_grad_slots(w, b, C, x.device)
+        if gx is not None:
+            assert gx.dtype == torch.float32 and gx.shape == x.shape
+            gx = gx.contiguous()
+        ops.layernorm_bwd_fused(gy.contiguous(), x, w.detach(), stats, dx, dw, db, dx_add=gx)
+        return dx, ret_w, ret_b, None, None
+
+
+def layer_norm_res(x, w, b, eps=1e-5, out_dtype=None):
+    if x.is_cuda and x.dtype == torch.float32 and ops.heads_fused() and ops.layernorm_bwd_fused_ok(x.shape[1]):
+        return LayerNormResFn.apply(x, w, b, eps, out_dtype or compute_dtype())
+    return x, layer_norm(x, w, b, eps, out_dtype)
+
+
 class BatchNormActFn(torch.autograd.Function):
 
     @staticmethod
@@ -691,6 +727,32 @@
         return dh
 
 
+class GegluDropoutFn(torch.autograd.Function):
+
+    @staticmethod
+    def forward(ctx, h, p):
+        M, c2 = h.shape
+        out = torch.empty(M, c2 // 2, dtype=h.dtype, device=h.device)
+        mask = torch.empty(M, c2 // 2, dtype=torch.float32, device=h.device)
+        seed, off = _next_rng(M * (c2 // 2))
+        ops.geglu_dropout_fwd(h, out, mask, p, seed, off)
+        ctx.save_for_backward(h, mask)
+        return out
+
+    @staticmethod
+    def backward(ctx, dout):
+        h, mask = ctx.saved_tensors
+        dh = torch.empty_like(h)
+        ops.geglu_dropout_bwd(h, dout.contiguous(), mask, dh)
+        return dh, None
+
+
+def geglu_dropout(h, p, training):
+    if training and p > 0 and ops.heads_fused():
+        return GegluDropoutFn.apply(h, p)
+    return dropout(GegluFn.apply(h), p, training)
+
+
 class DropoutFn(torch.autograd.Function):
 
     @staticmethod
@@ -699,9 +761,12 @@
         g = (M + rows_per_group - 1) // rows_per_group
         mask = torch.empty(g, C, dtype=torch.float32, device=x.device)
         seed, off = _next_rng(g * C)
-        ops.dropout_mask(mask, p, seed, off)
         y = torch.empty_like(x)
-        ops.mul_mask(x, mask, y, rows_per_group)
+        if rows_per_group == 1 and ops.heads_fused():
+            ops.dropout_apply(x, mask, y, p, seed, off)
+        else:
+            ops.dropout_mask(mask, p, seed, off)
+            ops.mul_mask(x, mask, y, rows_per_group)
         ctx.save_for_backward(mask)
         ctx.rpg = rows_per_group
         return y
diff --git a/vfmseg_amd/heads.py b/vfmseg_amd/heads.py
--- a/vfmseg_amd/heads.py
+++ b/vfmseg_amd/heads.py
@@ -293,20 +293,19 @@
         a1, a2, ff = self.attn1, self.attn2, self.ff
         H, d = a1.heads, a1.dim_head
         lin = ["linear"]
-        h = Fh.layer_norm(x, self.norm1.weight, self.norm1.bias, self.norm1.eps, cd)
+        x, h = Fh.layer_norm_res(x, self.norm1.weight, self.norm1.bias, self.norm1.eps, cd)
         qkv = Fh.linear(h, [a1.to_q.weight, a1.to_k.weight, a1.to_v.weight], lin * 3, out_dtype=cd)
         o = Fh.SelfAttnFn.apply(qkv, B, N, H, d)
         x = Fh.linear(o, a1.to_out[0].weight, "linear", bias=a1.to_out[0].bias, residual=x, out_dtype=torch.float32,
                       drop_p=a1.p if training else 0.0)
-        h = Fh.layer_norm(x, self.norm2.weight, self.norm2.bias, self.norm2.eps, cd)
+        x, h = Fh.layer_norm_res(x, self.norm2.weight, self.norm2.bias, self.norm2.eps, cd)
         q = Fh.linear(h, a2.to_q.weight, "linear", out_dtype=cd)
         kv = Fh.linear(ctx, [a2.to_k.weight, a2.to_v.weight], lin * 2, out_dtype=cd)
         o = Fh.CrossAttnFn.apply(q, kv, B, N, Nk, H, d)
         x = Fh.linear(o, a2.to_out[0].weight, "linear", bias=a2.to_out[0].bias, residual=x, out_dtype=torch.float32,
                       drop_p=a2.p if training else 0.0)
-        h = Fh.layer_norm(x, self.norm3.weight, self.norm3.bias, self.norm3.eps, cd)
-        g = Fh.GegluFn.apply(Fh.linear(h, ff.net[0].proj.weight, "linear", bias=ff.net[0].proj.bias, out_dtype=cd))
-        g = Fh.dropout(g, ff.p, training)
+        x, h = Fh.layer_norm_res(x, self.norm3.weight, self.norm3.bias, self.norm3.eps, cd)
+        g = Fh.geglu_dropout(Fh.linear(h, ff.net[0].proj.weight, "linear", bias=ff.net[0].proj.bias, out_dtype=cd), ff.p, training)
         return Fh.linear(g, ff.net[2].weight, "linear", bias=ff.net[2].bias, residual=x, out_dtype=torch.float32)
 
 
diff --git a/vfmseg_amd/lib.py b/vfmseg_amd/lib.py
--- a/vfmseg_amd/lib.py
+++ b/vfmseg_amd/lib.py
@@ -8,7 +8,7 @@
 LIB_PATH_F16 = os.path.join(_HERE, "csrc", "libvfmseg_hip_f16.so")
 
 F32, BF16, U8, I64, SPLIT3 = 0, 1, 2, 3, 4
-ABI_VERSION = 6
+ABI_VERSION = 7
 EP_NONE, EP_GELU, EP_RELU, EP_MUL_GELU_GRAD, EP_MUL, EP_QGELU, EP_MUL_QGELU_GRAD, EP_GELU_DGELU = 0, 1, 2, 3, 4, 5, 6, 7
 ACT_NONE, ACT_GELU, ACT_RELU, ACT_QGELU = 0, 1, 2, 3
 
@@ -98,6 +98,7 @@
     "vfm_axpby": [vp, cf, vp, cf, cl, vp],
     "vfm_scale_by_device_scalar": [vp, vp, cl, vp],
     "vfm_colsum": [vp, ci, cl, cl, cl, vp, ci, vp, vp],
+    "vfm_colsum_fused": [vp, ci, cl, cl, cl, vp, ci, vp, vp, cl, vp],
     "vfm_preprocess_u8": [vp, ci, ci, vp, ci, ci, C.POINTER(C.c_float), C.POINTER(C.c_float), ci, cf, vp],
     "vfm_lora_pack": [vp, ci, cl, ci, vp],
     "vfm_slab_reduce": [vp, ci, cl, cl, cl, cf, vp, cl, cl, ci, vp],
@@ -105,6 +106,9 @@
     "vfm_mul_mask": [vp, ci, cl, vp, ci, cl, cl, vp, ci, cl, cl, cl, vp],
     "vfm_geglu_fwd": [vp, ci, cl, vp, ci, cl, cl, cl, vp],
     "vfm_geglu_bwd": [vp, ci, cl, vp, ci, cl, vp, ci, cl, cl, cl, vp],
+    "vfm_dropout_apply": [vp, ci, cl, vp, ci, cl, cl, vp, ci, cl, cl, cl, cf, u64, u64, vp],
+    "vfm_geglu_dropout_fwd": [vp, ci, cl, vp, ci, cl, vp, ci, cl, cl, cl, cf, u64, u64, vp],
+    "vfm_geglu_dropout_bwd": [vp, ci, cl, vp, ci, cl, vp, ci, cl, vp, ci, cl, cl, cl, vp],
     "vfm_swiglu_fwd": [vp, ci, cl, vp, ci, cl, cl, cl, vp],
     "vfm_swiglu_bwd": [vp, ci, cl, vp, ci, cl, vp, ci, cl, cl, cl, vp],
     "vfm_rope": [vp, ci, cl, cl, ci, ci, ci, vp, vp, ci, vp],
@@ -116,6 +120,8 @@
     "vfm_layernorm_dropout_fwd": [vp, cl, vp, vp, cf, vp, cl, vp, vp, cl, vp, cl, cf, u64, u64, cl, cl, vp],
     "vfm_layernorm_bwd_scaled": [vp, ci, cl, vp, cl, vp, vp, vp, cl, ci, vp, cl, vp, cl, cl, vp],
     "vfm_layernorm_bwd": [vp, ci, cl, vp, cl, vp, vp, vp, cl, ci, vp, vp, vp, cl, cl, vp],
+    "vfm_layernorm_bwd_fused_ok": [cl],
+    "vfm_layernorm_bwd_fused": [vp, ci, cl, vp, cl, vp, vp, vp, cl, vp, cl, vp, vp, vp, vp, cl, cl, vp],
     "vfm_groupnorm_fwd": [vp, vp, vp, cf, ci, ci, vp, ci, vp, vp, cl, cl, cl, vp],
     "vfm_groupnorm_bwd": [vp, ci, vp, vp, vp, vp, ci, ci, vp, vp, vp, vp, cl, cl, cl, vp],
     "vfm_groupnorm_tile_ok": [cl, cl, ci],
diff --git a/vfmseg_amd/ops.py b/vfmseg_amd/ops.py
--- a/vfmseg_amd/ops.py
+++ b/vfmseg_amd/ops.py
@@ -25,13 +25,21 @@
         REGION.pop()
 
 
-def workspace(nfloats, device, tag="default"):
+def workspace(nfloats, device, tag="default", zero=False):
     key = (str(device), tag, L.stream())
     t = _ws_cache.get(key)
     if t is None or t.numel() < nfloats:
-        t = torch.empty(max(int(nfloats), 1 << 16), dtype=torch.float32, device=device)
+        t = (torch.zeros if zero else torch.empty)(max(int(nfloats), 1 << 16), dtype=torch.float32, device=device)
         _ws_cache[key] = t
     return t
+
+
+def tickets(n, device):
+    return workspace(n, device, tag="tickets", zero=True)
+
+
+def heads_fused():
+    return os.environ.get("VFMSEG_HEADS_FUSED", "1") != "0"
 
 
 def ld_pad(cols, dtype):
@@ -129,10 +137,23 @@
     return y
 
 
+def _colsum_parts(rows, cols):
+    ct = 64
+    while ct > 8 and ct // 2 >= cols:
+        ct //= 2
+    per = (256 // ct) * 8
+    return min(64, max(1, (rows + per - 1) // per))
+
+
 def colsum(x, out, accumulate=False):
     lib = L.load()
     rows, cols = x.shape
     ws = workspace(64 * cols, x.device)
+    if heads_fused() and (_colsum_parts(rows, cols) == 1 or os.environ.get("VFMSEG_COLSUM_TICKET", "0") == "1"):
+        nt = (cols + 7) // 8
+        L.check(lib.vfm_colsum_fused(L.ptr(x), L.dt_of(x), _ld(x), rows, cols, L.ptr(out), int(accumulate), L.ptr(ws),
+                                     L.ptr(tickets(nt, x.device)), nt, L.stream()), "vfm_colsum_fused")
+        return out
     L.check(lib.vfm_colsum(L.ptr(x), L.dt_of(x), _ld(x), rows, cols, L.ptr(out), int(accumulate), L.ptr(ws), L.stream()),
             "vfm_colsum")
     return out
@@ -151,6 +172,32 @@
     L.check(lib.vfm_mul_mask(L.ptr(src), L.dt_of(src), _ld(src), L.ptr(mask), L.dt_of(mask), _ld(mask), rows_per_group,
                              L.ptr(dst), L.dt_of(dst), _ld(dst), src.shape[0], src.shape[1], L.stream()), "vfm_mul_mask")
     return dst
+
+
+def dropout_apply(src, mask, dst, p, seed, offset=0, rows_per_group=1):
+    lib = L.load()
+    assert mask.is_contiguous() and mask.shape[1] == src.shape[1]
+    L.check(lib.vfm_dropout_apply(L.ptr(src), L.dt_of(src), _ld(src), L.ptr(mask), L.dt_of(mask), _ld(mask), rows_per_group, L.ptr(dst),
+                                  L.dt_of(dst), _ld(dst), src.shape[0], src.shape[1], float(p), int(seed), int(offset), L.stream()),
+            "vfm_dropout_apply")
+    return dst
+
+
+def geglu_dropout_fwd(h, out, mask, p, seed, offset=0):
+    lib = L.load()
+    rows, c2 = h.shape
+    assert mask.is_contiguous() and mask.shape == (rows, c2 // 2)
+    L.check(lib.vfm_geglu_dropout_fwd(L.ptr(h), L.dt_of(h), _ld(h), L.ptr(out), L.dt_of(out), _ld(out), L.ptr(mask), L.dt_of(mask),
+                                      _ld(mask), rows, c2 // 2, float(p), int(seed), int(offset), L.stream()), "vfm_geglu_dropout_fwd")
+    return out
+
+
+def geglu_dropout_bwd(h, dout, mask, dh):
+    lib = L.load()
+    rows, c2 = h.shape
+    L.check(lib.vfm_geglu_dropout_bwd(L.ptr(h), L.dt_of(h), _ld(h), L.ptr(dout), L.dt_of(dout), _ld(dout), L.ptr(mask), L.dt_of(mask),
+                                      _ld(mask), L.ptr(dh), L.dt_of(dh), _ld(dh), rows, c2 // 2, L.stream()), "vfm_geglu_dropout_bwd")
+    return dh
 
 
 def geglu_fwd(h, out):
@@ -264,6 +311,20 @@
     L.check(lib.vfm_layernorm_bwd(L.ptr(dy), L.dt_of(dy), _ld(dy), L.ptr(x), _ld(x), L.ptr(w), L.ptr(stats), L.ptr(dx),
                                   _ld(dx), int(accumulate_dx), L.ptr(dw), L.ptr(db), L.ptr(ws), rows, c, L.stream()),
             "vfm_layernorm_bwd")
+    return dx
+
+
+def layernorm_bwd_fused_ok(C):
+    return bool(L.load().vfm_layernorm_bwd_fused_ok(int(C)))
+
+
+def layernorm_bwd_fused(dy, x, w, stats, dx, dw, db, dx_add=None):
+    lib = L.load()
+    rows, c = x.shape
+    ws = workspace(64 * 2 * c, x.device)
+    L.check(lib.vfm_layernorm_bwd_fused(L.ptr(dy), L.dt_of(dy), _ld(dy), L.ptr(x), _ld(x), L.ptr(w), L.ptr(stats), L.ptr(dx_add),
+                                        _ld(dx_add) if dx_add is not None else 0, L.ptr(dx), _ld(dx), L.ptr(dw), L.ptr(db), L.ptr(ws),
+                                        L.ptr(tickets(1, x.device)), rows, c, L.stream()), "vfm_layernorm_bwd_fused")
     return dx
 
 
```
